# collinlongoria/blok

Hardware: AMD Instinct MI355X
Metric: Mrays/sec, primary first-hit rays at 4K over a 1024^3 SVO (higher is better)
Workload: dtype f32; 1 GPU; 1024^3 synthetic SVO (G(N,seed) terrain shell + 64 spheres, 2829976 voxels, 9299813 reference SvoNodes, 15132 sub-chunks), 3840x2160 primary rays, camera pose A, first-hit records 16 B/ray; hits_per_frame=2276630, framebuffer_pixels_hit=2276630, outputs=16-B first-hit records (kept on the tracing GPU) + RGBA8 framebuffer on rank 0, frames_in_flight=3, settle_frames=32, walk_waves_that_gave_up_waiting=0, beam_tile=32, full=False

## Files before the change

blok_amd/_ffi.py:

```python
from __future__ import annotations

import ctypes as C
import os
from pathlib import Path

import numpy as np

PKG_DIR = Path(__file__).resolve().parent
HOST_LIB = PKG_DIR / "libblok_host.so"
HIP_LIB = Path(os.environ.get("BLOK_HIP_LIB", PKG_DIR / "libblok_hip.so"))


class BlokLibraryError(RuntimeError):
    pass


class BlokError(RuntimeError):
    def __init__(self, status: int, message: str):
        super().__init__(f"blok status {status}: {message}")
        self.status = status


SVO_NODE = np.dtype([("child_mask", "<u4"), ("first_child", "<u4"), ("material_id", "<u4"),
                     ("occupancy", "<f4")])
# ... 237 lines not shown
    "blok_shapes_voxels": (C.c_int, [C.c_void_p, C.c_void_p, C.POINTER(C.c_int32), C.c_uint32, C.c_uint32, C.c_uint32, C.c_void_p, C.c_uint32, C.POINTER(C.c_uint64)]),
    "blok_lod_reduce": (C.c_int, [C.c_void_p, C.c_void_p, C.POINTER(C.c_int32), C.c_uint32, C.c_uint32, C.c_uint32, C.POINTER(C.c_int32), C.POINTER(C.c_int32),
                                  C.c_uint32, C.c_uint32, C.c_void_p, C.c_uint64, C.c_void_p]),
    "blok_terrain_reduce": (C.c_int, [C.c_void_p, C.POINTER(C.c_int32), C.POINTER(C.c_int32), C.c_uint32, C.c_uint32, C.c_void_p, C.c_uint64, C.c_void_p]),
    "blok_automaton_check": (C.c_int, [C.c_void_p, C.c_char_p, C.c_size_t]),
    "blok_automaton_voxels": (C.c_int, [C.c_void_p, C.c_void_p, C.POINTER(C.c_int32), C.c_uint32, C.c_uint32, C.c_uint32, C.POINTER(C.c_int32), C.POINTER(C.c_int32),
                                        C.c_void_p, C.c_void_p, C.c_void_p]),
    "blok_affine_from_instance": (C.c_int, [C.c_void_p, C.c_uint32, C.c_void_p]),
    "blok_affine_from_matrix": (C.c_int, [C.POINTER(C.c_double), C.c_void_p]),
    "blok_pose_from_instance": (C.c_int, [C.c_void_p, C.c_float, C.c_void_p]),
    "blok_pose_from_matrix": (C.c_int, [C.POINTER(C.c_double), C.POINTER(C.c_double), C.c_uint32, C.c_void_p]),
    "blok_affine_from_pose": (C.c_int, [C.c_void_p, C.c_float, C.c_uint32, C.c_void_p]),
    "blok_pose_motion_record": (C.c_int, [C.c_void_p, C.c_void_p, C.c_int, C.c_void_p]),
    "blok_affine_stamp_voxels": (C.c_int, [C.c_void_p, C.c_void_p, C.POINTER(C.c_int32), C.c_uint32, C.c_uint32, C.c_uint32, C.c_void_p, C.c_void_p, C.c_size_t,
                                           C.c_void_p, C.POINTER(C.c_int32), C.POINTER(C.c_int32), C.c_int, C.c_float, C.POINTER(C.c_uint64)]),
    "blok_scene_generate": (C.c_int, [C.c_void_p, C.c_uint32, C.c_uint32, C.POINTER(C.c_uint64)]),
    "blok_scene_generate_dense": (C.c_int, [C.c_uint32, C.c_uint32, C.c_void_p, C.POINTER(C.c_uint64)]),
    "blok_scene_materials": (C.c_int, [C.c_uint32, C.c_void_p]),
    "blok_scene_camera": (C.c_int, [C.c_uint32, C.c_uint32, C.c_int, C.c_uint32, C.c_uint32, C.c_void_p]),
}

HIP_SYMBOLS = {
    "blok_hip_create": (C.c_int, [C.POINTER(C.c_void_p), C.c_int, C.c_uint32, C.c_uint32]),
    "blok_hip_resize": (C.c_int, [C.c_void_p, C.c_uint32, C.c_uint32]),
    "blok_hip_destroy": (None, [C.c_void_p]),
    "blok_hip_last_error": (C.c_char_p, [C.c_void_p]),
    "blok_hip_release_stream": (C.c_int, [C.c_void_p, C.c_void_p]),
    "blok_hip_upload_world": (C.c_int, [C.c_void_p, C.c_void_p, C.c_size_t, C.c_void_p, C.c_size_t,
                                        C.c_void_p, C.c_size_t]),
    "blok_hip_upload_dense": (C.c_int, [C.c_void_p, C.c_void_p, C.c_uint32, C.c_uint32, C.c_uint32,
                                        C.POINTER(C.c_int32), C.c_void_p, C.c_size_t]),
    "blok_hip_set_host_build": (C.c_int, [C.c_void_p, C.c_int]),
    "blok_hip_world_built_on_device": (C.c_int, [C.c_void_p]),
    "blok_hip_download_tree": (C.c_int, [C.c_void_p, C.c_void_p, C.c_size_t, C.c_void_p, C.c_size_t]),
    "blok_hip_world_stats": (C.c_int, [C.c_void_p, C.POINTER(WorldStats)]),
    "blok_hip_trace_primary": (C.c_int, [C.c_void_p, C.c_void_p, C.c_uint32, C.c_uint32, C.c_uint32,
                                         C.c_uint32, C.c_void_p]),
    "blok_hip_trace_primary_device": (C.c_int, [C.c_void_p, C.c_void_p, C.c_uint32, C.c_uint32,
                                                C.c_uint32, C.c_uint32, C.c_void_p, C.c_void_p, C.c_void_p]),
    "blok_hip_tiles_for_rank": (C.c_uint32, [C.c_uint32, C.c_uint32, C.c_uint32, C.c_uint32, C.c_uint32]),
    "blok_hip_trace_tiles_device": (C.c_int, [C.c_void_p, C.c_void_p, C.c_uint32, C.c_uint32, C.c_uint32,
                                              C.c_void_p, C.c_void_p, C.c_void_p]),
    "blok_hip_untile_device": (C.c_int, [C.c_void_p, C.c_void_p, C.c_uint32, C.c_uint32, C.c_uint32, C.c_uint32,
                                         C.c_void_p, C.c_void_p]),
    "blok_hip_trace_paths_device": (C.c_int, [C.c_void_p, C.c_void_p] + [C.c_uint32] * 7 + [C.POINTER(GBuffer), C.c_void_p]),
    "blok_hip_trace_paths": (C.c_int, [C.c_void_p, C.c_void_p] + [C.c_uint32] * 7 + [C.POINTER(GBuffer)]),
    "blok_hip_trace_paths_ref_device": (C.c_int, [C.c_void_p, C.c_void_p] + [C.c_uint32] * 7 + [C.POINTER(C.c_float), C.POINTER(GBufferRef), C.c_void_p]),
    "blok_hip_denoise_ref_device": (C.c_int, [C.c_void_p, C.POINTER(GBufferRef), C.POINTER(C.c_float), C.c_uint32, C.c_void_p, C.c_void_p, C.c_void_p]),
    "blok_hip_tonemap_device": (C.c_int, [C.c_void_p, C.c_void_p, C.c_uint32, C.c_float, C.c_float, C.c_int, C.c_void_p, C.c_void_p]),
    "blok_hip_tonemap": (C.c_int, [C.c_void_p, C.c_void_p, C.c_uint32, C.c_float, C.c_float, C.c_int, C.c_void_p]),
    "blok_hip_trace_rays": (C.c_int, [C.c_void_p, C.c_void_p, C.c_size_t, C.c_void_p]),
    "blok_hip_shade_rgba8": (C.c_int, [C.c_void_p, C.c_void_p, C.c_uint32, C.c_uint32, C.c_uint32,
                                       C.c_uint32, C.c_void_p]),
    "blok_hip_draw_frame_accumulate": (C.c_int, [C.c_void_p, C.c_void_p, C.c_uint32, C.c_uint32, C.c_void_p, C.POINTER(C.c_uint32)]),
    "blok_hip_accum_download": (C.c_int, [C.c_void_p, C.c_void_p]),
    "blok_hip_reset_accum": (C.c_int, [C.c_void_p]),
    "blok_hip_set_beam": (C.c_int, [C.c_void_p, C.c_uint32]),
    "blok_hip_set_fused": (C.c_int, [C.c_void_p, C.c_int]),
    "blok_hip_set_dense_dda": (C.c_int, [C.c_void_p, C.c_int]),
    "blok_hip_set_voxel_size": (C.c_int, [C.c_void_p, C.c_float]),
    "blok_hip_multi_create": (C.c_int, [C.POINTER(C.c_void_p), C.POINTER(C.c_int), C.c_uint32, C.c_uint32, C.c_uint32, C.c_uint32, C.c_int]),
    "blok_hip_multi_destroy": (None, [C.c_void_p]),
    "blok_hip_multi_last_error": (C.c_char_p, [C.c_void_p]),
    "blok_hip_multi_device_count": (C.c_uint32, [C.c_void_p]),
    "blok_hip_multi_transport": (C.c_char_p, [C.c_void_p]),
    "blok_hip_multi_context": (C.c_void_p, [C.c_void_p, C.c_uint32]),
    "blok_hip_multi_upload_world": (C.c_int, [C.c_void_p, C.c_void_p, C.c_size_t, C.c_void_p, C.c_size_t, C.c_void_p, C.c_size_t]),
    "blok_hip_multi_draw_frame_device": (C.c_int, [C.c_void_p, C.c_void_p, C.POINTER(C.c_void_p)]),
    "blok_hip_multi_synchronize": (C.c_int, [C.c_void_p]),
    "blok_hip_multi_draw_frame": (C.c_int, [C.c_void_p, C.c_void_p, C.c_void_p]),
    "blok_hip_multi_set_exchange": (C.c_int, [C.c_void_p, C.c_int]),
    "blok_hip_multi_exchange": (C.c_char_p, [C.c_void_p]),
    "blok_hip_multi_debug_deny_peer_access": (C.c_int, [C.c_void_p, C.c_int]),
    "blok_hip_multi_draw_frames_device": (C.c_int, [C.c_void_p, C.c_void_p, C.c_uint32, C.POINTER(C.c_void_p)]),
    "blok_hip_multi_draw_frames": (C.c_int, [C.c_void_p, C.c_void_p, C.c_uint32, C.c_void_p]),
    "blok_hip_multi_download_hits": (C.c_int, [C.c_void_p, C.c_uint32, C.c_void_p, C.c_size_t]),
    "blok_hip_set_beam_budget": (C.c_int, [C.c_void_p, C.c_uint32]),
    "blok_hip_beam_cache_download": (C.c_int, [C.c_void_p, C.c_void_p, C.c_void_p, C.c_void_p, C.c_size_t]),
    "blok_hip_set_miss_writer": (C.c_int, [C.c_void_p, C.c_int]),
    "blok_hip_set_beam_cache": (C.c_int, [C.c_void_p, C.c_int]),
    "blok_hip_beam_cache_counters": (C.c_int, [C.c_void_p, C.POINTER(C.c_uint64), C.POINTER(C.c_uint64)]),
    "blok_hip_beam_cache_download_starts": (C.c_int, [C.c_void_p, C.c_void_p, C.c_void_p, C.c_size_t, C.c_void_p, C.c_size_t]),
    "blok_hip_beam_cache_start_counters": (C.c_int, [C.c_void_p, C.POINTER(C.c_uint64), C.POINTER(C.c_uint64)]),
    "blok_hip_set_packed_fill": (C.c_int, [C.c_void_p, C.c_uint32]),
    "blok_hip_packed_fill_counters": (C.c_int, [C.c_void_p, C.POINTER(C.c_uint64), C.POINTER(C.c_uint64)]),
    "blok_hip_beam_cache_refines": (C.c_int, [C.c_void_p, C.POINTER(C.c_uint64)]),
    "blok_hip_set_beam_refine_after": (C.c_int, [C.c_void_p, C.c_uint32]),
    "blok_hip_beam_cache_download_fine": (C.c_int, [C.c_void_p, C.c_void_p, C.c_void_p, C.c_void_p, C.c_size_t]),
    "blok_hip_pack_area": (C.c_uint32, []),
    "blok_hip_set_beam_list_after": (C.c_int, [C.c_void_p, C.c_uint32]),
    "blok_hip_beam_cache_list_builds": (C.c_int, [C.c_void_p, C.POINTER(C.c_uint64)]),
    "blok_hip_beam_cache_download_list": (C.c_int, [C.c_void_p, C.c_void_p, C.c_void_p, C.c_void_p, C.c_void_p, C.c_size_t, C.c_void_p, C.c_size_t, C.c_void_p, C.c_size_t]),
    "blok_hip_last_launch_kind": (C.c_int, [C.c_void_p]),
    "blok_hip_set_volume_layout": (C.c_int, [C.c_void_p, C.c_int]),
    "blok_hip_set_list_classes": (C.c_int, [C.c_void_p, C.c_int]),
    "blok_hip_set_joint_prefix_limit": (C.c_int, [C.c_void_p, C.c_uint32]),
    "blok_hip_set_tile_ordering": (C.c_int, [C.c_void_p, C.c_int]),
    "blok_hip_set_rank_tile_ordering": (C.c_int, [C.c_void_p, C.c_int]),
    "blok_hip_set_moving_order": (C.c_int, [C.c_void_p, C.c_int]),
    "blok_hip_last_fallback_tiles": (C.c_int64, [C.c_void_p]),
    "blok_hip_debug_force_order_shift": (C.c_int, [C.c_void_p, C.c_int, C.c_uint32, C.c_uint32]),
    "blok_hip_debug_class_order": (C.c_int, [C.c_void_p, C.c_void_p, C.c_uint32, C.c_uint32, C.c_uint32, C.c_void_p, C.c_uint32, C.c_void_p, C.c_void_p, C.POINTER(C.c_uint32), C.c_void_p]),
    "blok_hip_last_order_use": (C.c_int, [C.c_void_p, C.POINTER(C.c_int32), C.POINTER(C.c_int32)]),
    "blok_hip_beam_prepass": (C.c_int, [C.c_void_p, C.c_void_p] + [C.c_uint32] * 4 + [C.c_void_p, C.c_void_p, C.c_size_t]),
    "blok_hip_trace_wave_tiles_device": (C.c_int, [C.c_void_p, C.c_void_p] + [C.c_uint32] * 4 + [C.c_void_p, C.c_void_p, C.c_size_t, C.c_void_p, C.c_void_p, C.c_void_p]),
    "blok_hip_set_debug_wave_clocks": (C.c_int, [C.c_void_p, C.c_void_p]),
    "blok_hip_set_taa_jitter": (C.c_int, [C.c_void_p, C.POINTER(C.c_float)]),
    "blok_hip_set_rt_taa_jitter": (C.c_int, [C.c_void_p, C.c_int]),
    "blok_hip_compact_words": (C.c_size_t, [C.c_uint32, C.c_uint32]),
    "blok_hip_trace_tile_frames_device": (C.c_int, [C.c_void_p, C.c_void_p, C.c_uint32, C.c_uint32, C.c_uint32, C.c_uint32, C.c_uint32,
                                                    C.c_void_p, C.c_void_p, C.c_void_p]),
    "blok_hip_untile_frames_device": (C.c_int, [C.c_void_p, C.c_void_p, C.c_uint32, C.c_uint32, C.c_uint32, C.c_uint32, C.c_uint32, C.c_uint32,
                                                C.c_void_p, C.c_void_p]),
    "blok_hip_compact_tile_frames_device": (C.c_int, [C.c_void_p, C.c_void_p, C.c_uint32, C.c_uint32, C.c_uint32, C.c_uint32, C.c_void_p,
                                                      C.c_void_p]),
    "blok_hip_scatter_tile_frames_device": (C.c_int, [C.c_void_p, C.c_void_p, C.c_uint32, C.c_size_t, C.c_uint32, C.c_uint32, C.c_uint32,
                                                      C.c_void_p, C.c_void_p, C.c_void_p]),
    "blok_hip_exchange_code_bits": (C.c_uint32, [C.c_void_p]),
    "blok_hip_compact_code_words": (C.c_size_t, [C.c_uint32, C.c_uint32]),
    "blok_hip_compact_hit_tile_frames_device": (C.c_int, [C.c_void_p, C.c_void_p, C.c_uint32, C.c_uint32, C.c_uint32, C.c_uint32, C.c_void_p,
                                                          C.c_void_p]),
    "blok_hip_scatter_code_tile_frames_device": (C.c_int, [C.c_void_p, C.c_void_p, C.c_uint32, C.c_size_t, C.c_uint32, C.c_uint32, C.c_uint32,
                                                           C.c_void_p, C.c_void_p, C.c_void_p]),
    "blok_hip_compact_tiles_device": (C.c_int, [C.c_void_p, C.c_void_p, C.c_uint32, C.c_uint32, C.c_void_p, C.c_void_p]),
    "blok_hip_scatter_tiles_device": (C.c_int, [C.c_void_p, C.c_void_p, C.c_uint32, C.c_size_t, C.c_uint32, C.c_uint32, C.c_void_p, C.c_void_p]),
    "blok_hip_frame_queue_stalls": (C.c_int, [C.c_void_p, C.POINTER(C.c_uint32)]),
    "blok_hip_set_sun_map": (C.c_int, [C.c_void_p, C.c_int]),
    "blok_hip_sun_map_download": (C.c_int, [C.c_void_p, C.c_void_p, C.c_void_p, C.c_size_t]),
    "blok_hip_set_ray_batching": (C.c_int, [C.c_void_p, C.c_int]),
    "blok_hip_set_path_start": (C.c_int, [C.c_void_p, C.c_int, C.c_int]),
    "blok_denoise_settings_default": (None, [C.c_void_p]),
    "blok_hip_denoise_device": (C.c_int, [C.c_void_p, C.c_void_p, C.c_void_p, C.POINTER(C.c_float), C.c_uint32, C.c_void_p,
                                          C.c_void_p, C.c_void_p]),
    "blok_hip_denoise_state": (C.c_int, [C.c_void_p] * 6),
    "blok_hip_taa_device": (C.c_int, [C.c_void_p, C.c_void_p, C.c_void_p, C.c_float, C.c_float, C.c_uint32, C.c_void_p, C.c_void_p]),
    "blok_hip_sharpen_device": (C.c_int, [C.c_void_p, C.c_void_p, C.c_float, C.c_void_p, C.c_void_p]),
    "blok_hip_post_reset": (C.c_int, [C.c_void_p]),
    "blok_camera_view_proj": (None, [C.c_void_p, C.POINTER(C.c_float)]),
    "blok_hip_draw_frame_rt": (C.c_int, [C.c_void_p, C.c_void_p, C.c_uint32, C.c_uint32, C.c_void_p, C.c_void_p, C.POINTER(C.c_uint32)]),
    "blok_hip_volume_create": (C.c_int, [C.c_void_p, C.POINTER(C.c_int32), C.c_uint32, C.c_uint32, C.c_uint32, C.c_uint32, C.c_float]),
    "blok_hip_volume_destroy": (C.c_int, [C.c_void_p]),
    "blok_hip_volume_upload": (C.c_int, [C.c_void_p, C.c_void_p, C.c_void_p]),
    "blok_hip_volume_download": (C.c_int, [C.c_void_p, C.c_void_p, C.c_void_p]),
    "blok_hip_volume_set_voxels": (C.c_int, [C.c_void_p, C.c_void_p, C.c_void_p, C.c_void_p, C.c_size_t]),
    "blok_hip_volume_apply_brush": (C.c_int, [C.c_void_p, C.POINTER(C.c_float), C.c_float, C.c_float, C.c_int]),
    "blok_hip_volume_rebuild": (C.c_int, [C.c_void_p, C.c_void_p, C.c_size_t]),
    "blok_hip_volume_voxelize_mesh": (C.c_int, [C.c_void_p, C.c_void_p, C.c_size_t, C.c_void_p, C.c_size_t, C.c_void_p, C.c_uint32, C.c_float,
                                               C.c_int, C.POINTER(C.c_uint64)]),
    "blok_hip_volume_generate_terrain": (C.c_int, [C.c_void_p, C.c_void_p, C.POINTER(C.c_int32), C.POINTER(C.c_int32), C.POINTER(C.c_uint64)]),
    "blok_hip_volume_extract_quads": (C.c_int, [C.c_void_p, C.POINTER(C.c_int32), C.POINTER(C.c_int32), C.c_uint32, C.POINTER(C.c_uint64),
                                                C.POINTER(C.c_uint64)]),
    "blok_hip_volume_quads_download": (C.c_int, [C.c_void_p, C.c_void_p, C.c_uint64, C.c_uint64]),
    "blok_hip_lights_from_quads": (C.c_int, [C.c_void_p, C.c_uint32, C.c_void_p]),
    "blok_hip_set_lights": (C.c_int, [C.c_void_p, C.c_void_p, C.c_uint32, C.c_void_p]),
    "blok_hip_lights_info": (C.c_int, [C.c_void_p, C.c_void_p]),
    "blok_hip_lights_download": (C.c_int, [C.c_void_p, C.c_void_p, C.c_uint64, C.c_uint64]),
    "blok_hip_volume_stamp_models": (C.c_int, [C.c_void_p, C.c_void_p, C.c_uint32, C.c_int, C.c_float, C.POINTER(C.c_uint64)]),
    "blok_hip_volume_stamp_affine": (C.c_int, [C.c_void_p, C.c_void_p, C.c_uint32, C.POINTER(C.c_int32), C.POINTER(C.c_int32), C.c_int, C.c_float,
                                               C.POINTER(C.c_uint64)]),
    "blok_hip_volume_capture_model": (C.c_int, [C.c_void_p, C.POINTER(C.c_int32), C.POINTER(C.c_int32), C.c_uint32, C.POINTER(C.c_uint32),
                                                C.POINTER(C.c_uint64)]),
    "blok_hip_volume_label_components": (C.c_int, [C.c_void_p, C.POINTER(C.c_int32), C.POINTER(C.c_int32), C.c_uint32, C.POINTER(C.c_uint64),
                                                   C.POINTER(C.c_uint64)]),
    "blok_hip_volume_components_download": (C.c_int, [C.c_void_p, C.c_void_p, C.c_uint64, C.c_uint64]),
    "blok_hip_volume_labels_download": (C.c_int, [C.c_void_p, C.c_void_p, C.c_uint64, C.c_uint64]),
    "blok_hip_volume_capture_component": (C.c_int, [C.c_void_p, C.c_uint32, C.c_uint32, C.POINTER(C.c_uint32), C.POINTER(C.c_int32),
# ... 141 lines not shown
```

blok_amd/csrc/hip/api.hip:

```cpp
#include "api_internal.h"
#include "../common/lights_core.h"
#include <cstdlib>

namespace blok_api {


thread_local std::string g_create_error;

int set_error(blok_hip_ctx* ctx, int status, const std::string& msg) {
    if (ctx) ctx->error = msg; else g_create_error = msg;
    return status;
}


void free_world(blok_hip_ctx* ctx) {
    ctx->own_nodes.reset(); ctx->own_tree_materials.reset();
    ctx->d_nodes = nullptr; ctx->d_tree_materials = nullptr; ctx->tree_owned_by_volume = false;
    ctx->d_materials.reset(); ctx->d_sun_map.reset(); ctx->d_dense_tiled.reset(); ctx->d_dense_bits.reset();
    ctx->has_sun_map = false; ctx->has_dense = false;
    ctx->n_materials = 0; ctx->has_world = false; ctx->built_on_device = false; ctx->stats = blok_world_stats{};
    ctx->world_voxel_size = 1.0f;
    clear_lights(ctx);
}

// ... 155 lines not shown
    a.levels = ctx->stats.levels;
    a.voxel_size = ctx->world_voxel_size; a.inv_voxel_size = 1.0f / ctx->world_voxel_size;
    if (cam) a.cam = *cam;
    a.frame_w = ctx->width; a.frame_h = ctx->height;
    a.jitter_clip[0] = (2.0f * ctx->jitter_px[0]) / static_cast<float>(ctx->width);
    a.jitter_clip[1] = (2.0f * ctx->jitter_px[1]) / static_cast<float>(ctx->height);
    a.mat_table = ctx->d_materials;
    a.n_materials = static_cast<uint32_t>(ctx->n_materials);
    a.tmin = BLOK_RAY_TMIN; a.tmax = BLOK_RAY_TMAX;
    a.beam_budget = ctx->beam_budget;
    a.debug_clocks = ctx->debug_clocks;
    return a;
}

int beam_buffer(blok_hip_ctx* ctx, hipStream_t stream, size_t n, float** out) {
    auto& slot = ctx->beam_buffers[stream];
    BLOK_HIP_TRY(ctx, slot.beam.reserve(n, blok::FreeAfter::work_on(stream)));
    *out = slot.beam;
    return BLOK_OK;
}

int prepare_queue(blok_hip_ctx* ctx, blok::RayMode mode, const blok::TraceArgs& args, hipStream_t stream, uint32_t n_beams,
                  blok::FrameQueue* queue, uint32_t* n_blocks) {
    const size_t per_beam = static_cast<size_t>(args.beam_tile / blok::kWaveW) * (args.beam_tile / blok::kWaveH);
    const uint32_t parts = ctx->frame_parts;
    const size_t part_capacity = static_cast<size_t>((n_beams + parts - 1u) / parts) * per_beam;
    const size_t need = part_capacity * parts;
    auto& slot = ctx->beam_buffers[stream];
    bool fresh = false;
    BLOK_HIP_TRY(ctx, slot.ctl.reserve(blok::kFrameCtlWords, blok::FreeAfter::nothing(), &fresh));
    if (fresh) BLOK_HIP_TRY_FILL(ctx, slot.ctl, hipMemsetAsync(slot.ctl, 0, blok::kFrameCtlWords * sizeof(uint32_t), stream));
    BLOK_HIP_TRY(ctx, slot.entries.reserve(need, blok::FreeAfter::work_on(stream), &fresh));
    if (fresh) BLOK_HIP_TRY_FILL(ctx, slot.entries, hipMemsetAsync(slot.entries, 0xFF, need * sizeof(unsigned long long), stream));
    queue->ctl = slot.ctl; queue->entries = slot.entries; queue->n_beam = n_beams; queue->part_capacity = static_cast<uint32_t>(part_capacity);
    queue->n_parts = parts; queue->chunk = ctx->frame_chunk;
    const int m = mode == blok::RayMode::Rect ? 0 : 1;
    const uint32_t lv = args.levels < 16u ? args.levels : 15u;
    if (!ctx->frame_blocks_per_cu[m][lv]) {
        const int n = blok::frame_blocks_per_cu(mode, args);
        if (n <= 0) return set_error(ctx, BLOK_ERR_HIP, "frame kernel does not fit a compute unit");
        ctx->frame_blocks_per_cu[m][lv] = n;
    }
    const size_t resident = static_cast<size_t>(ctx->cu_count) * ctx->frame_blocks_per_cu[m][lv];
    const size_t waves = std::min(resident, std::max<size_t>(static_cast<size_t>(n_beams) * per_beam, n_beams));
    *n_blocks = static_cast<uint32_t>((waves + parts - 1u) / parts * parts);
    return BLOK_OK;
}

int prepare_beam(blok_hip_ctx* ctx, blok::RayMode mode, blok::TraceArgs& args, hipStream_t stream, uint32_t tiles_of_rank, uint32_t* n_beams) {
    *n_beams = 0;
    if (mode == blok::RayMode::Rays || !ctx->beam_tile) return BLOK_OK;
    args.beam_tile = ctx->beam_tile;
    if (mode == blok::RayMode::Tiles && args.tile % args.beam_tile) args.beam_tile = 16;
    if (args.beam_tile % blok::kWaveW || args.beam_tile % blok::kWaveH) { args.beam_tile = 0; return BLOK_OK; }
    args.beam_bx = (args.w + args.beam_tile - 1u) / args.beam_tile;
    *n_beams = blok::beam_tiles(mode, args, tiles_of_rank);
    return beam_buffer(ctx, stream, *n_beams, &args.beam);
}

bool rect_inside(const blok_hip_ctx* ctx, uint32_t x0, uint32_t y0, uint32_t w, uint32_t h) {
    return w && h && x0 < ctx->width && y0 < ctx->height && w <= ctx->width - x0 && h <= ctx->height - y0;
}

int check_trace(blok_hip_ctx* ctx, const blok_camera* cam) {
    if (!ctx) return BLOK_ERR_INVALID_ARG;
    if (!cam) return set_error(ctx, BLOK_ERR_INVALID_ARG, "camera is null");
    {
        const float* f = reinterpret_cast<const float*>(cam);
        for (size_t i = 0; i < sizeof(blok_camera) / sizeof(float); ++i)
            if (!std::isfinite(f[i])) return set_error(ctx, BLOK_ERR_INVALID_ARG, "camera has a non-finite component");
        if (!(cam->tan_half_fov > 0.0f) || !(cam->aspect > 0.0f)) return set_error(ctx, BLOK_ERR_INVALID_ARG, "camera needs tan_half_fov > 0 and aspect > 0");
    }
    if (!ctx->has_world) return set_error(ctx, BLOK_ERR_NO_WORLD, "no world uploaded");
    BLOK_HIP_TRY(ctx, hipSetDevice(ctx->device));
    return BLOK_OK;
}

}

using namespace blok_api;

extern "C" {

uint32_t blok_hip_abi_version(void) { return (1u << 16) | 26u; }

const char* blok_hip_last_error(const blok_hip_ctx* ctx) { return ctx ? ctx->error.c_str() : g_create_error.c_str(); }

int blok_hip_create(blok_hip_ctx** out_ctx, int device_ordinal, uint32_t width, uint32_t height) {
    if (!out_ctx) return BLOK_ERR_INVALID_ARG;
    *out_ctx = nullptr;
    if (!width || !height) return set_error(nullptr, BLOK_ERR_INVALID_ARG, "zero-sized frame");
    int count = 0;
    hipError_t e = hipGetDeviceCount(&count);
    if (e != hipSuccess || count <= 0)
        return set_error(nullptr, BLOK_ERR_NO_DEVICE, std::string("no HIP device: ") + hipGetErrorString(e));
    if (device_ordinal < 0 || device_ordinal >= count)
        return set_error(nullptr, BLOK_ERR_INVALID_ARG, "device ordinal out of range");
    hipDeviceProp_t prop{};
    e = hipGetDeviceProperties(&prop, device_ordinal);
    if (e != hipSuccess) return set_error(nullptr, BLOK_ERR_NO_DEVICE, std::string("hipGetDeviceProperties: ") + hipGetErrorString(e));
    if (std::strncmp(prop.gcnArchName, "gfx950", 6) != 0)
        return set_error(nullptr, BLOK_ERR_NO_DEVICE, std::string("device is ") + prop.gcnArchName + ", this backend is built for gfx950 only");
    e = hipSetDevice(device_ordinal);
    if (e != hipSuccess) return set_error(nullptr, BLOK_ERR_NO_DEVICE, std::string("hipSetDevice: ") + hipGetErrorString(e));
    auto* ctx = new (std::nothrow) blok_hip_ctx();
    if (!ctx) return set_error(nullptr, BLOK_ERR_OOM, "host allocation failed");
    ctx->device = device_ordinal; ctx->width = width; ctx->height = height;
    ctx->cu_count = prop.multiProcessorCount;
    if (const char* e = std::getenv("BLOK_FRAME_PARTS")) { const long v = std::atol(e); if (v >= 1 && v <= long(blok::kFrameParts)) ctx->frame_parts = uint32_t(v); }
    if (const char* e = std::getenv("BLOK_FRAME_CHUNK")) { const long v = std::atol(e); if (v >= 1 && v <= 64) ctx->frame_chunk = uint32_t(v); }    if (ctx->ev_begin.create(hipEventDefault) != hipSuccess || ctx->ev_end.create(hipEventDefault) != hipSuccess) {
        delete ctx;
        return set_error(nullptr, BLOK_ERR_HIP, "hipEventCreate failed");
    }
    if (order_buffers(ctx, 0u, nullptr) != BLOK_OK || beam_cache_buffers(ctx) != BLOK_OK || hipDeviceSynchronize() != hipSuccess) {
        const std::string why = ctx->error;
        blok_hip_destroy(ctx);
        return set_error(nullptr, BLOK_ERR_OOM, "scheduling buffers: " + why);
    }
    *out_ctx = ctx;
    return BLOK_OK;
}

int blok_hip_resize(blok_hip_ctx* ctx, uint32_t width, uint32_t height) {
    if (!ctx) return BLOK_ERR_INVALID_ARG;
    if (!width || !height) return set_error(ctx, BLOK_ERR_INVALID_ARG, "zero-sized frame");
    ctx->width = width; ctx->height = height;
    BLOK_HIP_TRY(ctx, hipSetDevice(ctx->device));
    const int rc = order_buffers(ctx, 0u, nullptr);
    if (rc != BLOK_OK) return rc;
    const int rc_cache = beam_cache_buffers(ctx);
    if (rc_cache != BLOK_OK) return rc_cache;
    BLOK_HIP_TRY(ctx, hipDeviceSynchronize());
    return BLOK_OK;
}

int blok_hip_release_stream(blok_hip_ctx* ctx, void* hip_stream) {
    if (!ctx) return BLOK_ERR_INVALID_ARG;
    hipStream_t stream = static_cast<hipStream_t>(hip_stream);
    BLOK_HIP_TRY(ctx, hipSetDevice(ctx->device));
    BLOK_HIP_TRY(ctx, hipDeviceSynchronize());
    auto it = ctx->beam_buffers.find(stream);
    if (it != ctx->beam_buffers.end()) ctx->beam_buffers.erase(it);
    forget_device_activity(ctx, true, stream);
    settle_beam_cache(ctx);
    return BLOK_OK;
}

void blok_hip_destroy(blok_hip_ctx* ctx) {
    if (!ctx) return;
    (void)hipSetDevice(ctx->device);
    if (ctx->has_volume) blok::gpu_volume_destroy(&ctx->volume);
    free_volume_snapshots(ctx);
    forget_device_activity(ctx);
    delete ctx;
}

int blok_hip_upload_world(blok_hip_ctx* ctx, const blok_svo_node* nodes, size_t n_nodes,
                          const blok_sub_chunk* sub_chunks, size_t n_sub_chunks,
                          const blok_material* materials, size_t n_materials) {
    if (!ctx) return BLOK_ERR_INVALID_ARG;
    if ((n_nodes && !nodes) || (n_sub_chunks && !sub_chunks) || (n_materials && !materials))
        return set_error(ctx, BLOK_ERR_INVALID_ARG, "null array with non-zero count");
    BLOK_HIP_TRY(ctx, hipSetDevice(ctx->device));
    const float vs = ctx->voxel_size;
    std::vector<blok_sub_chunk> scaled;
    if (vs != 1.0f) {
        scaled.assign(sub_chunks, sub_chunks + n_sub_chunks);
// ... 639 lines not shown
```

blok_amd/csrc/hip/api_debug.hip:

```cpp
#include "api_internal.h"
#include <cstdlib>
#include <cstdio>

using namespace blok_api;

extern "C" {

int blok_hip_set_host_build(blok_hip_ctx* ctx, int enabled) {
    if (!ctx) return BLOK_ERR_INVALID_ARG;
    ctx->force_host_build = enabled != 0;
    return BLOK_OK;
}

int blok_hip_world_built_on_device(const blok_hip_ctx* ctx) { return ctx && ctx->has_world && ctx->built_on_device ? 1 : 0; }

int blok_hip_download_tree(const blok_hip_ctx* ctx, void* nodes_out, size_t node_capacity, uint32_t* materials_out,
                           size_t material_capacity) {
    if (!ctx || !ctx->has_world) return BLOK_ERR_NO_WORLD;
    if ((nodes_out && node_capacity < ctx->stats.n_tree_nodes) || (materials_out && material_capacity < ctx->stats.n_voxels))
        return BLOK_ERR_INVALID_ARG;
    if (nodes_out && hipMemcpy(nodes_out, ctx->d_nodes, ctx->stats.n_tree_nodes * sizeof(blok::TreeNode), hipMemcpyDeviceToHost) != hipSuccess)
        return BLOK_ERR_HIP;
    if (materials_out && ctx->stats.n_voxels &&
        hipMemcpy(materials_out, ctx->d_tree_materials, ctx->stats.n_voxels * sizeof(uint32_t), hipMemcpyDeviceToHost) != hipSuccess)
// ... 209 lines not shown
    *out_stalled_waves = 0;
    BLOK_HIP_TRY(ctx, hipSetDevice(ctx->device));
    BLOK_HIP_TRY(ctx, hipDeviceSynchronize());
    for (auto& kv : ctx->beam_buffers) {
        if (kv.second.gave_up) {
            uint32_t n = 0;
            BLOK_HIP_TRY(ctx, hipMemcpy(&n, kv.second.gave_up, sizeof(n), hipMemcpyDeviceToHost));
            *out_stalled_waves += n;
        }
        if (!kv.second.ctl) continue;
        for (uint32_t part = 0; part < blok::kFrameParts; ++part) {
            uint32_t n = 0;
            BLOK_HIP_TRY(ctx, hipMemcpy(&n, kv.second.ctl + part * blok::kFramePartWords + blok::kFrameStalledWord, sizeof(n), hipMemcpyDeviceToHost));
            *out_stalled_waves += n;
        }
    }
    return BLOK_OK;
}

int blok_hip_last_launch_kind(const blok_hip_ctx* ctx) { return ctx ? ctx->last_launch_kind : -1; }

int blok_hip_set_tile_ordering(blok_hip_ctx* ctx, int resort_every_n_frames) {
    if (!ctx) return BLOK_ERR_INVALID_ARG;
    if (resort_every_n_frames < 0) return set_error(ctx, BLOK_ERR_INVALID_ARG, "tile ordering: interval must be >= 0");
    ctx->order.enabled = resort_every_n_frames != 0;
    if (resort_every_n_frames) ctx->order.interval = ctx->order.interval_now = static_cast<uint32_t>(resort_every_n_frames);
    return BLOK_OK;
}

int blok_hip_set_rank_tile_ordering(blok_hip_ctx* ctx, int enabled) {
    if (!ctx) return BLOK_ERR_INVALID_ARG;
    ctx->order.rank_tiles = enabled != 0;
    return BLOK_OK;
}

int blok_hip_debug_force_order_shift(blok_hip_ctx* ctx, int enabled, uint32_t shift_x, uint32_t shift_y) {
    if (!ctx) return BLOK_ERR_INVALID_ARG;
    ctx->order.debug_shift = enabled != 0; ctx->order.debug_sx = shift_x; ctx->order.debug_sy = shift_y;
    return BLOK_OK;
}

int64_t blok_hip_last_fallback_tiles(const blok_hip_ctx* ctx) {
    if (!ctx || !ctx->order.h_fallback) return -1;
    return static_cast<int64_t>(*static_cast<volatile uint32_t*>(ctx->order.h_fallback));
}

int blok_hip_set_moving_order(blok_hip_ctx* ctx, int enabled) {
    if (!ctx) return BLOK_ERR_INVALID_ARG;
    ctx->order.moving = enabled != 0;
    return BLOK_OK;
}

int blok_hip_last_order_use(const blok_hip_ctx* ctx, int32_t* out_shift_x, int32_t* out_shift_y) {
    if (!ctx) return -1;
    if (out_shift_x) *out_shift_x = static_cast<int32_t>(ctx->order.last_sx);
    if (out_shift_y) *out_shift_y = static_cast<int32_t>(ctx->order.last_sy);
    return ctx->order.last_use;
}

int blok_hip_set_joint_prefix_limit(blok_hip_ctx* ctx, uint32_t max_walk_waves) {
    if (!ctx) return BLOK_ERR_INVALID_ARG;
    ctx->order.prefix_limit = max_walk_waves;
    return BLOK_OK;
}

int blok_hip_set_list_classes(blok_hip_ctx* ctx, int enabled) {
    if (!ctx) return BLOK_ERR_INVALID_ARG;
    ctx->list_classes = enabled != 0;
    return BLOK_OK;
}

int blok_hip_set_miss_writer(blok_hip_ctx* ctx, int in_walk) {
    if (!ctx) return BLOK_ERR_INVALID_ARG;
    ctx->miss_in_walk = in_walk != 0;
    return BLOK_OK;
}

int blok_hip_set_beam_cache(blok_hip_ctx* ctx, int mode) {
    if (!ctx) return BLOK_ERR_INVALID_ARG;
    ctx->beam_cache.enabled = mode != 0;
    ctx->beam_cache.refine = mode >= 2;
    ctx->beam_cache.packed = mode >= 3;
    ctx->beam_cache.policy.own_starts = mode >= 4;
    blok::beam_cache_clear(ctx->beam_cache.policy);
    if (!ctx->beam_cache.packed) return BLOK_OK;
    BLOK_HIP_TRY(ctx, hipSetDevice(ctx->device));
    return beam_list_buffers(ctx);
}

int blok_hip_set_beam_list_after(blok_hip_ctx* ctx, uint32_t hits) {
    if (!ctx) return BLOK_ERR_INVALID_ARG;
    ctx->beam_cache.policy.list_after = hits ? hits : blok::kBeamListAfter;
    return BLOK_OK;
}

uint32_t blok_hip_pack_area(void) { return blok::kPackArea; }

int blok_hip_beam_cache_list_builds(const blok_hip_ctx* ctx, uint64_t* out_builds) {
    if (!ctx) return BLOK_ERR_INVALID_ARG;
    if (out_builds) *out_builds = ctx->beam_cache.list_builds;
    return BLOK_OK;
}

int blok_hip_beam_cache_download_list(blok_hip_ctx* ctx, int* out_state, uint32_t* out_n_areas, uint32_t* out_n_groups, uint32_t* out_list_host, size_t list_capacity,
                                      uint32_t* out_table_host, size_t table_capacity, uint8_t* out_trips_host, size_t trips_capacity) {
    if (!ctx) return BLOK_ERR_INVALID_ARG;
    const auto& B = ctx->beam_cache;
    if (out_state) *out_state = B.last_list;
    if (out_n_areas) *out_n_areas = 0u;
    if (out_n_groups) *out_n_groups = 0u;
    if (!B.last_list) return BLOK_OK;
    if (B.last_slot < 0 || static_cast<uint32_t>(B.last_slot) >= blok::kBeamCacheSlots || !B.slots[B.last_slot].d_list)
        return set_error(ctx, BLOK_ERR_INVALID_ARG, "beam cache: the latest launch's slot is gone (a resize)");
    const auto& sl = B.slots[B.last_slot];
    const uint32_t n_areas = sl.n_words / blok::kPackGroups;
    const size_t entries = static_cast<size_t>(n_areas) * blok::kPackStretch, pixels = static_cast<size_t>(B.last_w) * B.last_h;
    if (entries > B.list_capacity || sl.n_words > B.words_capacity || pixels > B.d_trips.capacity()) return set_error(ctx, BLOK_ERR_INVALID_ARG, "beam cache: the list's buffers are gone (a resize)");
    if ((out_list_host && list_capacity < entries) || (out_table_host && table_capacity < sl.n_words) || (out_trips_host && trips_capacity < pixels))
        return set_error(ctx, BLOK_ERR_INVALID_ARG, "beam cache: output smaller than the list, the table or the rectangle");
    if (out_n_areas) *out_n_areas = n_areas;
    if (!out_n_groups && !out_list_host && !out_table_host && !out_trips_host) return BLOK_OK;
    BLOK_HIP_TRY(ctx, hipSetDevice(ctx->device));
    BLOK_HIP_TRY(ctx, hipDeviceSynchronize());
    if (out_n_groups) *out_n_groups = B.last_list == 2 ? sl.n_groups : std::min(B.h_groups[B.last_slot], sl.n_words);
    if (out_list_host) BLOK_HIP_TRY(ctx, hipMemcpy(out_list_host, sl.d_list, entries * sizeof(uint32_t), hipMemcpyDeviceToHost));
    if (out_table_host) BLOK_HIP_TRY(ctx, hipMemcpy(out_table_host, sl.d_table, sl.n_words * sizeof(uint32_t), hipMemcpyDeviceToHost));
    if (out_trips_host) BLOK_HIP_TRY(ctx, hipMemcpy(out_trips_host, B.d_trips, pixels, hipMemcpyDeviceToHost));
    return BLOK_OK;
}

int blok_hip_beam_cache_download_starts(blok_hip_ctx* ctx, int* out_state, float* out_starts_host, size_t starts_capacity, uint8_t* out_restarts_host, size_t restarts_capacity) {
    if (!ctx) return BLOK_ERR_INVALID_ARG;
    const auto& B = ctx->beam_cache;
    if (out_state) *out_state = B.last_starts;
    if (!out_starts_host && !out_restarts_host) return BLOK_OK;
    if (!B.last_list || B.last_slot < 0 || static_cast<uint32_t>(B.last_slot) >= blok::kBeamCacheSlots || !B.policy.starts[B.last_slot] || !B.slots[B.last_slot].d_start)
        return set_error(ctx, BLOK_ERR_INVALID_ARG, "beam cache: the latest launch's slot has no list with starts");
    const auto& sl = B.slots[B.last_slot];
    const size_t entries = static_cast<size_t>(sl.n_words / blok::kPackGroups) * blok::kPackStretch, pixels = static_cast<size_t>(B.last_w) * B.last_h;
    if (entries > sl.d_start.capacity() || pixels > B.d_restarts.capacity()) return set_error(ctx, BLOK_ERR_INVALID_ARG, "beam cache: the starts' buffers are gone (a resize)");
    if ((out_starts_host && starts_capacity < entries) || (out_restarts_host && restarts_capacity < pixels))
        return set_error(ctx, BLOK_ERR_INVALID_ARG, "beam cache: output smaller than the list or the rectangle");
    BLOK_HIP_TRY(ctx, hipSetDevice(ctx->device));
    BLOK_HIP_TRY(ctx, hipDeviceSynchronize());
    if (out_starts_host) BLOK_HIP_TRY(ctx, hipMemcpy(out_starts_host, sl.d_start, entries * sizeof(float), hipMemcpyDeviceToHost));
    if (out_restarts_host) BLOK_HIP_TRY(ctx, hipMemcpy(out_restarts_host, B.d_restarts, pixels, hipMemcpyDeviceToHost));
    return BLOK_OK;
}

int blok_hip_beam_cache_start_counters(const blok_hip_ctx* ctx, uint64_t* out_from_starts, uint64_t* out_other_key) {
    if (!ctx) return BLOK_ERR_INVALID_ARG;
    if (out_from_starts) *out_from_starts = ctx->beam_cache.start_hits;
    if (out_other_key) *out_other_key = ctx->beam_cache.start_other_key;
    return BLOK_OK;
}

int blok_hip_set_packed_fill(blok_hip_ctx* ctx, uint32_t units_per_wave) {
    if (!ctx) return BLOK_ERR_INVALID_ARG;
    ctx->beam_cache.packed_fill = units_per_wave;
    return BLOK_OK;
}

int blok_hip_packed_fill_counters(const blok_hip_ctx* ctx, uint64_t* out_one_launch_frames, uint64_t* out_fill_only_workgroups) {
    if (!ctx) return BLOK_ERR_INVALID_ARG;
    if (out_one_launch_frames) *out_one_launch_frames = ctx->beam_cache.one_launch_frames;
    if (out_fill_only_workgroups) *out_fill_only_workgroups = ctx->beam_cache.fill_only_workgroups;
    return BLOK_OK;
}

int blok_hip_beam_cache_counters(const blok_hip_ctx* ctx, uint64_t* out_hits, uint64_t* out_fills) {
    if (!ctx) return BLOK_ERR_INVALID_ARG;
    if (out_hits) *out_hits = ctx->beam_cache.hits;
    if (out_fills) *out_fills = ctx->beam_cache.fills;
    return BLOK_OK;
}

int blok_hip_set_beam_refine_after(blok_hip_ctx* ctx, uint32_t hits) {
    if (!ctx) return BLOK_ERR_INVALID_ARG;
    ctx->beam_cache.policy.refine_after = hits ? hits : blok::kBeamRefineAfter;
    return BLOK_OK;
}

int blok_hip_beam_cache_refines(const blok_hip_ctx* ctx, uint64_t* out_refines) {
    if (!ctx) return BLOK_ERR_INVALID_ARG;
    if (out_refines) *out_refines = ctx->beam_cache.refines;
    return BLOK_OK;
}

int blok_hip_beam_cache_download(blok_hip_ctx* ctx, int* out_action, uint32_t* out_n_beams, float* out_t0_host, size_t capacity) {
    if (!ctx) return BLOK_ERR_INVALID_ARG;
    const auto& B = ctx->beam_cache;
    if (out_action) *out_action = B.last_action;
    if (out_n_beams) *out_n_beams = B.last_action ? B.last_n_beams : 0u;
    if (!out_t0_host || !B.last_action) return BLOK_OK;
    if (B.last_slot < 0 || static_cast<uint32_t>(B.last_slot) >= blok::kBeamCacheSlots || !B.slots[B.last_slot].d_beam || B.last_n_beams > B.capacity)
        return set_error(ctx, BLOK_ERR_INVALID_ARG, "beam cache: the latest launch's slot is gone (a resize)");
    if (capacity < B.last_n_beams) return set_error(ctx, BLOK_ERR_INVALID_ARG, "beam cache: output smaller than the launch's beam tiles");
    BLOK_HIP_TRY(ctx, hipSetDevice(ctx->device));
    BLOK_HIP_TRY(ctx, hipDeviceSynchronize());
    BLOK_HIP_TRY(ctx, hipMemcpy(out_t0_host, B.slots[B.last_slot].d_beam, B.last_n_beams * sizeof(float), hipMemcpyDeviceToHost));
    return BLOK_OK;
}

int blok_hip_beam_cache_download_fine(blok_hip_ctx* ctx, int* out_state, uint32_t* out_n_tiles, float* out_t0_host, size_t capacity) {
    if (!ctx) return BLOK_ERR_INVALID_ARG;
    const auto& B = ctx->beam_cache;
    if (out_state) *out_state = B.last_fine;
    if (out_n_tiles) *out_n_tiles = B.last_n_fine;
    if (!out_t0_host || !B.last_fine) return BLOK_OK;
    if (B.last_slot < 0 || static_cast<uint32_t>(B.last_slot) >= blok::kBeamCacheSlots || !B.slots[B.last_slot].d_fine || B.last_n_fine > B.capacity)
        return set_error(ctx, BLOK_ERR_INVALID_ARG, "beam cache: the latest launch's slot is gone (a resize)");
    if (capacity < B.last_n_fine) return set_error(ctx, BLOK_ERR_INVALID_ARG, "beam cache: output smaller than the launch's wave tiles");
    BLOK_HIP_TRY(ctx, hipSetDevice(ctx->device));
    BLOK_HIP_TRY(ctx, hipDeviceSynchronize());
    BLOK_HIP_TRY(ctx, hipMemcpy(out_t0_host, B.slots[B.last_slot].d_fine, B.last_n_fine * sizeof(float), hipMemcpyDeviceToHost));
    return BLOK_OK;
}

int blok_hip_set_beam_budget(blok_hip_ctx* ctx, uint32_t max_node_visits) {
    if (!ctx) return BLOK_ERR_INVALID_ARG;
    ctx->beam_budget = max_node_visits;
    return BLOK_OK;
}

}
```

blok_amd/csrc/hip/api_internal.h:

```cpp
#ifndef BLOK_API_INTERNAL_H
#define BLOK_API_INTERNAL_H
#include <hip/hip_runtime.h>

#include <cmath>
#include <map>
#include <mutex>
#include <unordered_map>
#include <utility>
#include <cstdio>
#include <cstring>
#include <new>
#include <string>
#include <vector>

#include "blok_hip.h"
#include "blok_hip_debug.h"
#include "device_buffer.h"
#include "gpu_build.h"
#include <hip/hip_fp16.h>
#include "post_kernels.h"
#include "post_core.h"
#include "reference_world.h"
#include "trace_kernels.h"
#include "dense_kernels.h"
// ... 46 lines not shown
        bool has_motion = false;
        blok::DeviceArray<float> rt_planes[2], rt_denoised, rt_resolved;
        blok::DeviceArray<uint16_t> rt_normal_roughness_h, rt_motion_h;
        blok::DeviceArray<uint32_t> rt_albedo_metallic_u8;
        blok::DeviceArray<uint32_t> rt_ldr, rt_final;
        uint32_t rt_frame = 0;
        blok_camera rt_prev_cam{};
        blok::DeviceArray<uint32_t> rt_ids;
        uint32_t rt_prev_n = 0;
        uint32_t rt_prev_n_poses = 0;
    } post;
    blok::DeviceArray<blok_instance> rt_instances, rt_prev_instances;
    blok::DeviceArray<blok_pose> rt_poses;
    blok::DeviceArray<blok_pose> rt_prev_poses;
    blok::GpuVolume volume;
    bool has_volume = false;
    bool volume_keyed_layout = true;
    blok::GpuQuads quads;
    blok::GpuComponents components;
    blok::GpuBricks bricks;
    blok::GpuDistance distance;
    blok::GpuFlood flood;
    blok::GpuColumns columns;
    blok::GpuScatter scatter;
    blok::GpuLod lod;
    struct Lights {
        blok::DeviceArray<blok_light> table;
        blok::DeviceArray<uint32_t> owned;
        uint32_t n = 0, n_owned = 0;
        uint64_t n_faces = 0;
        float area_world = 0.0f;
    } lights;
    std::vector<uint32_t> material_glows;
    std::vector<unsigned char> volume_materials;
    blok::DeviceArray<float> d_sun_map;
    bool sun_map_enabled = true, has_sun_map = false;
    uint32_t sun_loose_edits = 0; int32_t sun_loose_lo[3] = {0, 0, 0}, sun_loose_hi[3] = {0, 0, 0};
    bool sun_tighten_pending = false; uint32_t sun_tighten_u0 = 0, sun_tighten_u1 = 0, sun_tighten_v0 = 0, sun_tighten_v1 = 0;
    blok::Event sun_event; bool sun_event_pending = false;
    uint32_t ray_batching = 3;
    uint32_t tail_cap = 24, tail_cap_parked = 32;
    bool pose_tlas = true;
    bool path_resume = false, path_fine_beam = true;
    blok::SunMapArgs sun{};
    uint32_t beam_tile = 32;
    uint32_t beam_budget = 0;
    bool miss_in_walk = true;
    struct StreamScratch {
        blok::DeviceArray<float> beam;
        blok::DeviceArray<uint32_t> ctl; blok::DeviceArray<unsigned long long> entries;
        blok::DeviceArray<unsigned long long> slots; uint32_t serial = 0;
        blok::DeviceArray<uint32_t> gave_up;
        blok::DeviceArray<unsigned long long> list_entries; size_t list_capacity = 0;
        blok::DeviceArray<unsigned long long> list_ctl;
        uint32_t list_serial = 0;
        blok::PinnedArray<uint32_t> list_hint; bool list_hint_valid = false; uint32_t list_hint_key = 0;
        blok::DeviceArray<uint32_t> tile_map;
        blok::DeviceBytes tail_pool;
        blok::DeviceArray<uint32_t> inst_bins;
        blok::DeviceArray<blok_hit> inst_hits;
        blok::DeviceArray<uint32_t> pose_bins;
        blok::DeviceBytes pose_tlas;
        blok::DeviceArray<blok_pose_motion> pose_motion;
        blok::DeviceBytes tlas;
    };
    std::unordered_map<hipStream_t, StreamScratch> beam_buffers;
    struct BeamCache {
        bool enabled = true;
        bool refine = true;
        blok::BeamCachePolicy policy{};
        struct Produced {
            blok::Event done;
            hipStream_t producer = nullptr;
            bool settled = true;
            static constexpr uint32_t kWaited = 8;
            hipStream_t waited[kWaited] = {}; uint32_t n_waited = 0;
        };
        struct Slot {
            blok::DeviceArray<float> d_beam, d_fine;
            Produced filled, refined;
            bool used = false;
            blok::DeviceArray<uint32_t> d_list, d_table;
            blok::DeviceArray<float> d_start;
            uint32_t n_words = 0, n_groups = 0;
        } slots[blok::kBeamCacheSlots];
        bool packed = true;
        blok::DeviceArray<uint8_t> d_trips;
        blok::DeviceArray<float> d_ray_start;
        blok::DeviceArray<uint8_t> d_restarts;
        blok::DeviceArray<uint32_t> d_words;
        blok::DeviceBytes d_sort_temp; size_t sort_temp_bytes = 0;
        blok::PinnedArray<uint32_t> h_groups;
        blok::Event list_done;
        size_t list_capacity = 0, words_capacity = 0;
        uint64_t list_builds = 0;
        uint64_t start_hits = 0, start_other_key = 0;
        uint32_t packed_fill = BLOK_PACKED_FILL;
        uint64_t one_launch_frames = 0, fill_only_workgroups = 0;
        int last_starts = 0;
        int last_list = 0;
        uint32_t last_w = 0, last_h = 0;
        size_t capacity = 0;
        uint64_t hits = 0, fills = 0, refines = 0;
        int last_action = 0, last_slot = -1; uint32_t last_n_beams = 0;
        int last_fine = 0; uint32_t last_n_fine = 0;
    } beam_cache;
    struct TileOrder {
        bool enabled = true;
        bool rank_tiles = true;
        uint32_t interval = 8, interval_now = 8;
        blok::DeviceArray<uint32_t> d_cost, d_iota;
        blok::DeviceArray<uint32_t> d_keys_in, d_keys;
        blok::DeviceBytes d_temp;
        size_t temp_bytes = 0, capacity = 0;
        static constexpr int kSlots = 4;
        struct Slot {
            blok::DeviceArray<uint32_t> d_order, d_rank_of;
            bool valid = false, dilated = false;
            uint32_t live = 0, radius = 0;
            blok_camera cam{};
            float inv_depth[2] = {};
            uint32_t frames_since_sort = 0, interval_now = 8;
            uint64_t last_use = 0;
        } slots[kSlots];
        blok::PinnedArray<uint32_t> h_live;
        blok::PinnedArray<float> h_depth;
        uint32_t key[7] = {};
        int current = -1, target = 0;
        bool pending = false;
        bool orphan = false;
        uint32_t still_frames = 0, prefix_limit = 0;
        uint64_t launch_serial = 0, hold_serial = 0;
        blok_camera last_cam{};
        blok_camera recent[4] = {}; uint32_t n_recent = 0, revisit_streak = 0;
        blok_camera pending_cam{}; bool pending_dilated = false; uint32_t pending_radius = 0, pending_interval = 8;
        blok::Event done;
        bool moving = true;
        blok::DeviceBytes d_class_scratch;
        bool have_residual = false; float last_residual = 0.0f;
        bool debug_shift = false; uint32_t debug_sx = 0, debug_sy = 0;
        blok::DeviceArray<uint32_t> d_fallback;
        blok::PinnedArray<uint32_t> h_fallback;
        uint32_t last_fallback = 0;
        bool alone_before = false;
        int last_use = 0; uint32_t last_sx = 0, last_sy = 0;
        int chosen = -1;
    } order;
    blok::DeviceArray<uint32_t> d_list_cost; uint32_t list_cost_key[6] = {};
    blok_camera list_prev_cam{}; bool list_has_prev_cam = false;
    bool list_classes = true;
    uint32_t* debug_clocks = nullptr;
    int launch_form = blok::kFormAuto;
    int last_launch_kind = -1;
    uint32_t frame_parts = 32, frame_chunk = 1;
    int cu_count = 0;
    int frame_blocks_per_cu[2][16] = {};
    float jitter_px[2] = {0.0f, 0.0f};
    bool rt_taa_jitter = true;
    struct Models {
        struct Arrays {
            blok::DeviceArray<uint4> nodes; blok::DeviceArray<uint32_t> materials;
            uint32_t n_nodes = 0, n_materials = 0;
            int32_t box_lo[3] = {0, 0, 0}, box_hi[3] = {0, 0, 0};
        };
        std::vector<blok::ModelDesc> desc;
        std::vector<Arrays> own;
        blok::DeviceArray<blok::ModelDesc> d_desc;
        float uploaded_voxel_size = 1.0f;
        uint32_t stack_levels = 1;
    } models;
    blok::Event ev_begin, ev_end;
    bool timing = false, timed = false;
// ... 112 lines not shown
```

blok_amd/csrc/hip/api_launch.hip:

```cpp
#include "api_internal.h"
#include "beam.h"
#include <cstdlib>

namespace blok_api {

namespace {
struct StreamMarks { blok::Event last, held; bool fresh = false; };
struct DeviceActivity {
    std::mutex lock;
    std::map<std::pair<const blok_hip_ctx*, hipStream_t>, StreamMarks> marks;
};
DeviceActivity& device_activity(int device) {
    static std::mutex table_lock;
    static auto& table = *new std::map<int, DeviceActivity>;
    std::lock_guard<std::mutex> g(table_lock);
    return table[device];
}
}

static bool device_busy_elsewhere(const blok_hip_ctx* ctx, hipStream_t stream) {
    DeviceActivity& act = device_activity(ctx->device);
    std::lock_guard<std::mutex> g(act.lock);
    bool busy = false;
    for (auto& kv : act.marks) {
// ... 227 lines not shown
}

int live_list(blok_hip_ctx* ctx, blok::TraceArgs& args, hipStream_t stream, uint32_t n_searches, uint32_t per_search) {
    auto& slot = ctx->beam_buffers[stream];
    const size_t seg_capacity = static_cast<size_t>((n_searches + blok::kListSegments - 1u) / blok::kListSegments) * per_search;
    bool fresh = false;
    BLOK_HIP_TRY(ctx, slot.list_ctl.reserve(blok::kListSegments * blok::kListCtlWords, blok::FreeAfter::nothing(), &fresh));
    if (fresh) {
        BLOK_HIP_TRY_FILL(ctx, slot.list_ctl, hipMemsetAsync(slot.list_ctl, 0, blok::kListSegments * blok::kListCtlWords * sizeof(unsigned long long), stream));
        BLOK_HIP_TRY_FILL(ctx, slot.list_ctl, slot.list_hint.reserve(blok::kListSegments * blok::kListClasses, blok::FreeAfter::nothing()));
        std::memset(slot.list_hint, 0, blok::kListSegments * blok::kListClasses * sizeof(uint32_t));
        slot.list_hint_valid = false;
    }
    const bool wrapped = slot.list_serial + 1u >= (1u << blok::kListSerialBits);
    if (slot.list_capacity < seg_capacity || wrapped) {
        bool grown = false;
        if (slot.list_capacity < seg_capacity) {
            slot.list_capacity = 0;
            BLOK_HIP_TRY(ctx, slot.list_entries.reserve(seg_capacity * blok::kListSegments * blok::kListClasses, blok::FreeAfter::work_on(stream), &grown));
            slot.list_capacity = seg_capacity;
        }
        const hipError_t emptied = hipMemsetAsync(slot.list_entries, 0, slot.list_capacity * blok::kListSegments * blok::kListClasses * sizeof(unsigned long long), stream);
        if (emptied != hipSuccess && grown) { slot.list_entries.reset(); slot.list_capacity = 0; }
        BLOK_HIP_TRY(ctx, emptied);
        if (wrapped) slot.list_serial = 0;
    }
    slot.list_serial += 1u;
    args.list.entries = slot.list_entries; args.list.ctl = slot.list_ctl; args.list.hint = slot.list_hint;
    args.list.seg_capacity = static_cast<uint32_t>(slot.list_capacity);
    args.list.serial = slot.list_serial; args.list.n_searches = n_searches;
    return gave_up_counter(ctx, stream, &args.joint_gave_up);
}

static bool list_hint(const blok_hip_ctx* ctx, hipStream_t stream, uint32_t geometry_key, uint32_t per_class[blok::kListClasses]) {
    auto it = ctx->beam_buffers.find(stream);
    if (it == ctx->beam_buffers.end() || !it->second.list_hint || !it->second.list_hint_valid || it->second.list_hint_key != geometry_key) return false;
    for (uint32_t c = 0; c < blok::kListClasses; ++c) {
        per_class[c] = 0;
        for (uint32_t k = 0; k < blok::kListSegments; ++k) per_class[c] = std::max(per_class[c], it->second.list_hint[k * blok::kListClasses + c]);
    }
    return true;
}

static int list_costs(blok_hip_ctx* ctx, blok::TraceArgs& args, uint32_t wave_tiles, hipStream_t stream) {
    const uint32_t key[6] = {args.x0, args.y0, args.w, args.h, ctx->width, ctx->height};
    bool fresh = false;
    BLOK_HIP_TRY(ctx, ctx->d_list_cost.reserve(wave_tiles, blok::FreeAfter::device(), &fresh));
    if (fresh || std::memcmp(key, ctx->list_cost_key, sizeof(key)) != 0) {
        BLOK_HIP_TRY(ctx, hipMemsetAsync(ctx->d_list_cost, 0, ctx->d_list_cost.capacity() * sizeof(uint32_t), stream));
        std::memcpy(ctx->list_cost_key, key, sizeof(key));
        ctx->list_has_prev_cam = false;
    }
    args.list.cost = ctx->d_list_cost;
    args.list.has_prev = ctx->list_has_prev_cam ? 1u : 0u;
    args.list.prev_cam = ctx->list_prev_cam;
    ctx->list_prev_cam = args.cam; ctx->list_has_prev_cam = true;
    return BLOK_OK;
}

int beam_cache_buffers(blok_hip_ctx* ctx) {
    auto& B = ctx->beam_cache;
    const size_t want = static_cast<size_t>((ctx->width + 7u) / 8u) * ((ctx->height + 7u) / 8u);
    if (B.capacity >= want) return beam_list_buffers(ctx);
    BLOK_HIP_TRY(ctx, hipDeviceSynchronize());
    B.capacity = 0;
    blok::beam_cache_clear(B.policy);
    for (auto& sl : B.slots) {
        sl = blok_hip_ctx::BeamCache::Slot{};
        BLOK_HIP_TRY(ctx, sl.d_beam.reserve(want, blok::FreeAfter::nothing()));
        BLOK_HIP_TRY(ctx, sl.d_fine.reserve(want, blok::FreeAfter::nothing()));
        BLOK_HIP_TRY(ctx, sl.filled.done.create());
        BLOK_HIP_TRY(ctx, sl.refined.done.create());
    }
    B.capacity = want;
    B.list_capacity = 0;
    return beam_list_buffers(ctx);
}

int beam_list_buffers(blok_hip_ctx* ctx) {
    auto& B = ctx->beam_cache;
    if (!B.packed) return BLOK_OK;
    const size_t areas = static_cast<size_t>((ctx->width + blok::kPackArea - 1u) / blok::kPackArea) * ((ctx->height + blok::kPackArea - 1u) / blok::kPackArea);
    const size_t entries = areas * blok::kPackStretch, words = areas * blok::kPackGroups, pixels = static_cast<size_t>(ctx->width) * ctx->height;
    const bool own = B.policy.own_starts;
    if (B.list_capacity >= entries && B.words_capacity >= words && B.d_trips.capacity() >= pixels &&
        (!own || (B.d_ray_start.capacity() >= pixels && B.d_restarts.capacity() >= pixels && B.slots[0].d_start.capacity() >= entries))) return BLOK_OK;
    BLOK_HIP_TRY(ctx, hipDeviceSynchronize());
    B.list_capacity = 0; B.words_capacity = 0;
    blok::beam_cache_clear(B.policy);
    blok::beam_list_settle(B.policy);
    const blok::FreeAfter waited = blok::FreeAfter::nothing();
    for (auto& sl : B.slots) {
        BLOK_HIP_TRY(ctx, sl.d_list.reserve(entries, waited));
        BLOK_HIP_TRY(ctx, sl.d_table.reserve(words, waited));
        if (own) BLOK_HIP_TRY(ctx, sl.d_start.reserve(entries, waited));
        sl.n_groups = 0;
    }
    BLOK_HIP_TRY(ctx, B.d_trips.reserve(pixels, waited));
    if (own) { BLOK_HIP_TRY(ctx, B.d_ray_start.reserve(pixels, waited)); BLOK_HIP_TRY(ctx, B.d_restarts.reserve(pixels, waited)); }
    BLOK_HIP_TRY(ctx, B.d_words.reserve(words, waited));
    B.sort_temp_bytes = blok::pack_table_temp_bytes(static_cast<uint32_t>(words));
    BLOK_HIP_TRY(ctx, B.d_sort_temp.reserve(B.sort_temp_bytes ? B.sort_temp_bytes : 16, waited));
    BLOK_HIP_TRY(ctx, B.h_groups.reserve(blok::kBeamCacheSlots, waited));
    BLOK_HIP_TRY(ctx, B.list_done.create());
    B.list_capacity = entries; B.words_capacity = words;
    return BLOK_OK;
}

void settle_beam_cache(blok_hip_ctx* ctx) {
    for (auto& sl : ctx->beam_cache.slots)
        for (auto* p : {&sl.filled, &sl.refined}) { p->settled = true; p->n_waited = 0; }
}

static blok::BeamKey beam_key(const blok_hip_ctx* ctx, blok::RayMode mode, const blok::TraceArgs& args) {
    blok::BeamKey k{};
    static_assert(sizeof(k.cam) == sizeof(blok_camera), "beam_cache.h: BeamKey::cam is blok_camera, byte for byte");
    std::memcpy(k.cam, &args.cam, sizeof(blok_camera));
    k.x0 = args.x0; k.y0 = args.y0; k.w = args.w; k.h = args.h;
    k.frame_w = args.frame_w; k.frame_h = args.frame_h;
    k.beam_tile = args.beam_tile; k.beam_budget = args.beam_budget;
    k.tuning = blok::kBeamCoarsen1 | (blok::kBeamCoarsen2 << 8) | (static_cast<uint32_t>(BLOK_BEAM_STOP_LEVEL) << 16);
    k.ray_mode = static_cast<uint32_t>(mode);
    k.levels = args.levels;
    for (int a = 0; a < 3; ++a) k.origin[a] = args.origin[a];
    std::memcpy(&k.voxel_bits, &args.voxel_size, sizeof(uint32_t));
    const uint64_t nodes = reinterpret_cast<uintptr_t>(args.nodes);
    k.nodes_lo = static_cast<uint32_t>(nodes); k.nodes_hi = static_cast<uint32_t>(nodes >> 32);
    k.world_version = ctx->world_version; k.tree_version = ctx->tree_version;
    return k;
}

static int wait_for_producer(blok_hip_ctx* ctx, blok_hip_ctx::BeamCache::Produced& p, hipStream_t stream) {
    if (p.settled || stream == p.producer) return BLOK_OK;
    for (uint32_t k = 0; k < p.n_waited; ++k) if (p.waited[k] == stream) return BLOK_OK;
    if (hipEventQuery(p.done) == hipSuccess) { p.settled = true; p.n_waited = 0; return BLOK_OK; }
    (void)hipGetLastError();
    BLOK_HIP_TRY(ctx, hipStreamWaitEvent(stream, p.done, 0));
    if (p.n_waited < blok_hip_ctx::BeamCache::Produced::kWaited) p.waited[p.n_waited++] = stream;
    return BLOK_OK;
}

static int beam_cache_before_launch(blok_hip_ctx* ctx, blok::RayMode mode, blok::TraceArgs& args, hipStream_t stream, blok::BeamCachePlan* plan, blok::BeamRefinePlan* fine,
                                    blok::BeamListPlan* listed, blok::BeamStartsPlan* starts) {
    auto& B = ctx->beam_cache;
    *plan = blok::plan_beam_cache(B.policy, beam_key(ctx, mode, args));
    *fine = blok::plan_beam_refine(B.policy, *plan, B.refine && blok::beam_refine_applies(args) && blok::beam_refine_tiles(args) <= B.capacity);
    bool build_finished = false;
    if (B.policy.building >= 0) { build_finished = hipEventQuery(B.list_done) == hipSuccess; (void)hipGetLastError(); }
    *listed = blok::plan_beam_list(B.policy, *plan, *fine, B.packed && blok::pack_applies(args) && static_cast<size_t>(blok::pack_areas(args)) * blok::kPackStretch <= B.list_capacity &&
                                   static_cast<size_t>(args.w) * args.h <= B.d_trips.capacity(), build_finished);
    if (listed->adopted >= 0) { auto& got = B.slots[listed->adopted]; got.n_groups = std::min(B.h_groups[listed->adopted], got.n_words); }
    blok::BeamStartKey start_key;
    static_assert(sizeof(args.jitter_clip) == sizeof(start_key.jitter_clip), "beam_cache.h: BeamStartKey::jitter_clip is TraceArgs::jitter_clip, bit for bit");
    std::memcpy(start_key.jitter_clip, args.jitter_clip, sizeof(start_key.jitter_clip));
    std::memcpy(&start_key.tmin, &args.tmin, sizeof(uint32_t)); std::memcpy(&start_key.tmax, &args.tmax, sizeof(uint32_t));
    *starts = blok::plan_beam_starts(B.policy, *plan, *listed, start_key);
    if (plan->action == blok::BeamAction::Search) return BLOK_OK;
    auto& sl = B.slots[plan->slot];
    if (plan->action == blok::BeamAction::Hit) {
        { const int rc = wait_for_producer(ctx, sl.filled, stream); if (rc != BLOK_OK) return rc; }
        if (fine->use_fine) { const int rc = wait_for_producer(ctx, sl.refined, stream); if (rc != BLOK_OK) return rc; }
        B.hits += 1u;
    } else {
        if (sl.used) {
            hold_markers(ctx);
            const int rc = wait_for_held_markers(ctx, stream);
            if (rc != BLOK_OK) return rc;
        }
        sl.used = true;
        sl.filled.settled = false; sl.filled.producer = stream; sl.filled.n_waited = 0;
        B.fills += 1u;
    }
    args.beam = sl.d_beam; args.beam_slots = nullptr; args.beam_serial = 0u;
    return BLOK_OK;
}

int launch_timed(blok_hip_ctx* ctx, blok::RayMode mode, blok::TraceArgs args, uint32_t blocks, hipStream_t stream,
                 uint32_t tiles_of_rank, const blok::TileFrames* frames) {
    uint32_t n_beams = 0;
    if (blocks) { const int rc = prepare_beam(ctx, mode, args, stream, tiles_of_rank, &n_beams); if (rc != BLOK_OK) return rc; }
    const uint32_t n_frames = frames ? frames->n_frames : 1u;
    if (frames && n_beams) { const int rc = beam_buffer(ctx, stream, static_cast<size_t>(n_beams) * n_frames, &args.beam); if (rc != BLOK_OK) return rc; }
    blok::LaunchFacts facts{};
    facts.form = ctx->launch_form;
    facts.has_beam = n_beams != 0;
    facts.one_wave_blocks = blok::kBlock == 64;
    facts.wave_tiles = blocks * n_frames;
    const uint32_t geometry_key = blocks * 31u + n_beams * n_frames;
    facts.have_hint = list_hint(ctx, stream, geometry_key, facts.hint);
    bool busy = false;
    bool capturing = false;
    if (stream) {
        hipStreamCaptureStatus status = hipStreamCaptureStatusNone;
        if (hipStreamIsCapturing(stream, &status) == hipSuccess) capturing = status != hipStreamCaptureStatusNone;
        else (void)hipGetLastError();
    }
    if (capturing) facts.form = blok::kFormTwoLaunches;
    else busy = facts.has_beam && (ctx->launch_form == blok::kFormAuto || (ctx->order.enabled && ctx->order.moving)) && device_busy_elsewhere(ctx, stream);
    facts.device_busy = busy && ctx->launch_form == blok::kFormAuto;
    blok::LaunchPlan plan = blok::plan_launch(facts);
    if (frames && (plan.kind == blok::LaunchKind::Queues || plan.kind == blok::LaunchKind::Joint)) plan.kind = blok::LaunchKind::TwoLaunches;
    ctx->last_launch_kind = static_cast<int>(plan.kind);

    blok::FrameQueue queue{};
    uint32_t frame_blocks = 0;
    blok::TileFrames fr{};
    if (frames) { fr = *frames; fr.blocks_per_frame = blocks; fr.beams_per_frame = n_beams; }
    if (plan.kind == blok::LaunchKind::Joint) { const int rc = joint_slots(ctx, args, stream, n_beams); if (rc != BLOK_OK) return rc; }
    if (plan.kind == blok::LaunchKind::Queues) { const int rc = prepare_queue(ctx, mode, args, stream, n_beams, &queue, &frame_blocks); if (rc != BLOK_OK) return rc; }
    if (plan.kind == blok::LaunchKind::ListJoint || plan.kind == blok::LaunchKind::ListTwoLaunches) {
        const uint32_t per_search = (args.beam_tile / blok::kWaveW) * (args.beam_tile / blok::kWaveH);
        const int rc = live_list(ctx, args, stream, n_beams * n_frames, per_search);
        if (rc != BLOK_OK) return rc;
        for (uint32_t c = 0; c < blok::kListClasses; ++c) args.list.walkers[c] = plan.walkers_per_class[c];
        if (mode == blok::RayMode::Rect && ctx->list_classes) { const int rc2 = list_costs(ctx, args, blocks, stream); if (rc2 != BLOK_OK) return rc2; }
        auto& slot = ctx->beam_buffers[stream];
        slot.list_hint_valid = true; slot.list_hint_key = geometry_key;
    }
    const bool static_form = plan.kind == blok::LaunchKind::TwoLaunches || plan.kind == blok::LaunchKind::Joint;
    const bool rect = mode == blok::RayMode::Rect;
    const bool orderable = !capturing && ctx->order.enabled && static_form && ((rect && !frames) || (mode == blok::RayMode::Tiles && ctx->order.rank_tiles)) && n_beams &&
                           blocks >= blok::kOrderMinTiles && BLOK_XCD_MAP == 0 && blok::kBlock == 64;
    bool uniform_view = true;
    if (frames) for (uint32_t f = 1; f < frames->n_frames; ++f) uniform_view = uniform_view && camera_near(ctx, frames->cam[0], frames->cam[f]);
    blok::OrderPlan order_plan{};
    if (orderable) { const int rc = order_before_launch(ctx, args, blocks, stream, !busy, rect, uniform_view, &order_plan); if (rc != BLOK_OK) return rc; }
    else ctx->order.last_use = 0;
    uint32_t walk_blocks = blocks;
    if (args.order && args.rank_of && plan.may_use_prefix && args.launched <= blocks) {
        if (ctx->order.prefix_limit && args.launched > ctx->order.prefix_limit) args.launched = ctx->order.prefix_limit;
        walk_blocks = args.launched;
        if (ctx->timing) {
            ctx->order.last_fallback = *static_cast<volatile uint32_t*>(ctx->order.h_fallback.get());
            BLOK_HIP_TRY(ctx, hipMemsetAsync(ctx->order.d_fallback, 0, sizeof(uint32_t), stream));
            args.fallback_tiles = ctx->order.d_fallback;
        }
        if (args.order_sx || args.order_sy) {
            const uint32_t tiles_x = (args.w + blok::kTileW - 1u) / blok::kTileW, tiles_y = (args.h + blok::kTileH - 1u) / blok::kTileH;
            const bool left = args.order_sx * 2u <= tiles_x, top = args.order_sy * 2u <= tiles_y;
            const float res = ctx->order.have_residual && ctx->order.last_residual >= 0.0f ? std::min(ctx->order.last_residual, 8.0f) : 0.0f;
            const uint32_t extra = static_cast<uint32_t>(std::ceil(res));
            args.strip_nx = left ? args.order_sx : tiles_x - args.order_sx; if (args.strip_nx) args.strip_nx = std::min(args.strip_nx + extra, tiles_x);
            args.strip_ny = top ? args.order_sy : tiles_y - args.order_sy; if (args.strip_ny) args.strip_ny = std::min(args.strip_ny + extra, tiles_y);
            args.strip_x0 = left ? 0u : tiles_x - args.strip_nx;
            args.strip_y0 = top ? 0u : tiles_y - args.strip_ny;
            args.n_strip = args.strip_nx * tiles_y + (tiles_x - args.strip_nx) * args.strip_ny;
            walk_blocks += args.n_strip;
        }
    } else { args.rank_of = nullptr; args.launched = 0u; }
    if (ctx->timing && !capturing) BLOK_HIP_TRY(ctx, hipEventRecord(ctx->ev_begin, stream));
    args.miss_in_walk = static_form && !args.rank_of && ctx->miss_in_walk ? 1u : 0u;
    blok::BeamCachePlan cached{blok::BeamAction::Search, -1};
    blok::BeamRefinePlan finer{false, false};
    blok::BeamListPlan listed{false, false, -1};
    blok::BeamStartsPlan starts{false, blok::BeamStarts::None};
    if (ctx->beam_cache.enabled && rect && !frames && !capturing && static_form && ctx->launch_form == blok::kFormAuto && n_beams && n_beams <= ctx->beam_cache.capacity) {
        const int rc = beam_cache_before_launch(ctx, mode, args, stream, &cached, &finer, &listed, &starts);
        if (rc != BLOK_OK) {
            if (finer.refine_now) blok::beam_refine_commit(ctx->beam_cache.policy, cached.slot, false);
            if (listed.count_now) blok::beam_list_commit(ctx->beam_cache.policy, cached.slot, false);
            return rc;
        }
        if (cached.action == blok::BeamAction::Fill && plan.kind == blok::LaunchKind::Joint) { plan.kind = blok::LaunchKind::TwoLaunches; ctx->last_launch_kind = static_cast<int>(plan.kind); }
    }
    ctx->beam_cache.last_action = cached.action == blok::BeamAction::Hit ? 2 : cached.action == blok::BeamAction::Fill ? 1 : 0;
    ctx->beam_cache.last_slot = cached.slot; ctx->beam_cache.last_n_beams = n_beams;
    ctx->beam_cache.last_fine = finer.use_fine ? 2 : finer.refine_now ? 1 : 0;
    ctx->beam_cache.last_n_fine = ctx->beam_cache.last_fine ? blok::beam_refine_tiles(args) : 0u;
    ctx->beam_cache.last_list = listed.use_list ? 2 : listed.count_now ? 1 : 0;
    ctx->beam_cache.last_starts = starts.use == blok::BeamStarts::OtherKey ? 2 : (starts.use == blok::BeamStarts::Use || starts.count_own) ? 1 : 0;
    if (starts.use == blok::BeamStarts::Use) ctx->beam_cache.start_hits += 1u;
    if (starts.use == blok::BeamStarts::OtherKey) ctx->beam_cache.start_other_key += 1u;
    ctx->beam_cache.last_w = args.w; ctx->beam_cache.last_h = args.h;
    if (cached.action == blok::BeamAction::Hit && (listed.use_list || listed.count_now)) {
        auto& B = ctx->beam_cache;
        auto& sl = B.slots[cached.slot];
        blok::TraceArgs fill = args;
        fill.order = nullptr; fill.rank_of = nullptr; fill.launched = 0u; fill.order_sx = fill.order_sy = 0u; fill.n_strip = 0u; fill.fallback_tiles = nullptr;
        fill.miss_in_walk = 0u;
        const bool one_launch = listed.use_list && sl.n_groups > 0u && B.packed_fill > 0u;
        if (!one_launch) blok::launch_beam_fill(mode, fill, n_beams, sl.d_fine, stream);
        if (one_launch) {
            const uint32_t tail = starts.use == blok::BeamStarts::Use ? blok::launch_packed_frame_own(fill, sl.d_start, sl.d_fine, sl.d_list, sl.d_table, sl.n_groups, B.packed_fill, stream)
                                                                      : blok::launch_packed_frame(fill, sl.d_fine, sl.d_list, sl.d_table, sl.n_groups, B.packed_fill, stream);
            B.one_launch_frames += 1u; B.fill_only_workgroups += tail;
        } else if (listed.use_list && starts.use == blok::BeamStarts::Use) blok::launch_packed_walk_own(fill, sl.d_start, sl.d_list, sl.d_table, sl.n_groups, stream);
        else if (listed.use_list) blok::launch_packed_walk(fill, sl.d_fine, sl.d_list, sl.d_table, sl.n_groups, stream);
        else if (starts.count_own) {
            blok::TraceArgs walk = fill;
            walk.beam = sl.d_fine; walk.beam_tile = blok::kWaveW; walk.beam_bx = (args.w + blok::kWaveW - 1u) / blok::kWaveW;
            blok::launch_trace_count_own(walk, blocks, B.d_trips, B.d_ray_start, B.d_restarts, stream);
            sl.n_words = blok::pack_areas(args) * blok::kPackGroups; sl.n_groups = 0u;
            blok::launch_pack_build_own(fill, sl.d_fine, B.d_restarts, B.d_ray_start, sl.d_list, B.d_words, sl.d_start, stream);
        } else {
            blok::TraceArgs walk = fill;
            walk.beam = sl.d_fine; walk.beam_tile = blok::kWaveW; walk.beam_bx = (args.w + blok::kWaveW - 1u) / blok::kWaveW;
            blok::launch_trace_count(walk, blocks, B.d_trips, stream);
            sl.n_words = blok::pack_areas(args) * blok::kPackGroups; sl.n_groups = 0u;
            blok::launch_pack_build(fill, sl.d_fine, B.d_trips, sl.d_list, B.d_words, stream);
        }
    } else if (cached.action == blok::BeamAction::Hit) {
        float* const d_fine = ctx->beam_cache.slots[cached.slot].d_fine;
        if (!args.miss_in_walk) blok::launch_beam_fill(mode, args, n_beams, finer.use_fine ? d_fine : nullptr, stream);
        if (finer.use_fine) {
            blok::TraceArgs walk = args;
            walk.beam = d_fine; walk.beam_tile = blok::kWaveW; walk.beam_bx = (args.w + blok::kWaveW - 1u) / blok::kWaveW;
            blok::launch_trace(mode, walk, walk_blocks, stream);
        } else blok::launch_trace(mode, args, walk_blocks, stream);
        if (finer.refine_now) blok::launch_beam_refine(args, d_fine, stream);
    } else
    switch (plan.kind) {
        case blok::LaunchKind::Walk:
            if (frames) blok::launch_tile_frames(args, fr, stream); else blok::launch_trace(mode, args, blocks, stream);
            break;
        case blok::LaunchKind::TwoLaunches:
            if (frames) blok::launch_tile_frames(args, fr, stream, walk_blocks);
            else { blok::launch_beam(mode, args, n_beams, stream); blok::launch_trace(mode, args, walk_blocks, stream); }
            break;
        case blok::LaunchKind::Queues: blok::launch_frame(mode, args, queue, frame_blocks, stream); break;
        case blok::LaunchKind::Joint: blok::launch_joint(mode, args, n_beams, walk_blocks, stream); break;
        case blok::LaunchKind::ListJoint: blok::launch_list_joint(mode, args, frames ? &fr : nullptr, n_beams * n_frames, plan.walkers, stream); break;
        case blok::LaunchKind::ListTwoLaunches:
            if (frames) blok::launch_beam_frames(args, fr, stream); else blok::launch_beam(mode, args, n_beams, stream);
            blok::launch_list_walk(mode, args, frames ? &fr : nullptr, plan.walkers, stream);
            break;
    }
    const hipError_t launch_error = hipGetLastError();
    if (launch_error != hipSuccess && cached.action == blok::BeamAction::Fill) ctx->beam_cache.policy.valid[cached.slot] = false;
    if (finer.refine_now) {
        auto& made = ctx->beam_cache.slots[cached.slot].refined;
        const hipError_t marked = launch_error == hipSuccess ? hipEventRecord(made.done, stream) : launch_error;
        blok::beam_refine_commit(ctx->beam_cache.policy, cached.slot, marked == hipSuccess);
        if (marked == hipSuccess) { made.settled = false; made.producer = stream; made.n_waited = 0; ctx->beam_cache.refines += 1u; }
        else if (launch_error == hipSuccess) BLOK_HIP_TRY(ctx, marked);
    }
    if (listed.count_now) {
        auto& B = ctx->beam_cache;
        auto& sl = B.slots[cached.slot];
        hipError_t built = launch_error;
        if (built == hipSuccess) built = blok::launch_pack_table_sort(B.d_words, sl.d_table, B.d_sort_temp, B.sort_temp_bytes, sl.n_words, B.h_groups + cached.slot, stream);
        if (built == hipSuccess) built = hipEventRecord(B.list_done, stream);
        blok::beam_list_commit(B.policy, cached.slot, built == hipSuccess);
        if (built == hipSuccess) B.list_builds += 1u;
        else if (launch_error == hipSuccess) BLOK_HIP_TRY(ctx, built);
    }
    BLOK_HIP_TRY(ctx, launch_error);
    if (cached.action == blok::BeamAction::Fill) BLOK_HIP_TRY(ctx, hipEventRecord(ctx->beam_cache.slots[cached.slot].filled.done, stream));
    if (ctx->timing && !capturing) { BLOK_HIP_TRY(ctx, hipEventRecord(ctx->ev_end, stream)); ctx->timed = true; }
    if (args.fallback_tiles) BLOK_HIP_TRY(ctx, hipMemcpyAsync(ctx->order.h_fallback, ctx->order.d_fallback, sizeof(uint32_t), hipMemcpyDeviceToHost, stream));
    if (listed.use_list) order_plan.start_sort = false;
    if (orderable) { const int rc = order_after_launch(ctx, args, blocks, n_beams, stream, order_plan); if (rc != BLOK_OK) return rc; }
    if (facts.has_beam && !capturing) return note_frame_launch(ctx, stream);
    return BLOK_OK;
}

}
```

blok_amd/csrc/hip/beam_cache.h:

```cpp
#ifndef BLOK_BEAM_CACHE_H
#define BLOK_BEAM_CACHE_H
#include <stdint.h>
#include <string.h>

namespace blok {

struct BeamKey {
    uint32_t cam[14];
    uint32_t x0, y0, w, h;
    uint32_t frame_w, frame_h;
    uint32_t beam_tile, beam_budget, tuning;
    uint32_t ray_mode;
    uint32_t levels;
    int32_t origin[3];
    uint32_t voxel_bits;
    uint32_t nodes_lo, nodes_hi;
    uint32_t world_version, tree_version;
};
static_assert(sizeof(BeamKey) == 33 * sizeof(uint32_t), "BeamKey is compared with memcmp: no padding");

inline bool beam_key_equal(const BeamKey& a, const BeamKey& b) { return memcmp(&a, &b, sizeof(BeamKey)) == 0; }

constexpr int kBeamCacheSlots = 4;

enum class BeamAction : int {
    Search = 0,
    Fill = 1,
    Hit = 2,
};
struct BeamCachePlan { BeamAction action; int slot; };

enum class BeamRefine : uint8_t {
    None = 0,
    Now = 1,
    Done = 2,
};
constexpr uint32_t kBeamRefineAfter = 16;
struct BeamRefinePlan { bool refine_now, use_fine; };

enum class BeamList : uint8_t {
    None = 0,
    Now = 1,
    Building = 2,
    Ready = 3,
};
constexpr uint32_t kBeamListAfter = 16;
struct BeamListPlan { bool count_now, use_list; int adopted; };

struct BeamStartKey { uint32_t jitter_clip[2], tmin, tmax; };
static_assert(sizeof(BeamStartKey) == 4 * sizeof(uint32_t), "BeamStartKey is compared with memcmp: no padding");
inline bool beam_start_key_equal(const BeamStartKey& a, const BeamStartKey& b) { return memcmp(&a, &b, sizeof(BeamStartKey)) == 0; }
enum class BeamStarts : int {
    None = 0,
    Use = 1,
    OtherKey = 2,
};
struct BeamStartsPlan { bool count_own; BeamStarts use; };

struct BeamCachePolicy {
    BeamKey key[kBeamCacheSlots];
    bool valid[kBeamCacheSlots];
    uint64_t last_use[kBeamCacheSlots];
    BeamKey last;
    bool have_last;
    uint64_t serial;
    BeamRefine refine[kBeamCacheSlots];
    uint32_t hits_since_fill[kBeamCacheSlots];
    uint32_t refine_after = kBeamRefineAfter;
    BeamList list[kBeamCacheSlots];
    uint32_t fine_hits[kBeamCacheSlots];
    uint32_t list_after = kBeamListAfter;
    bool own_starts = true;
    bool starts[kBeamCacheSlots];
    BeamStartKey start_key[kBeamCacheSlots];
    int building = -1;
    bool building_stale = false;
};

inline void beam_list_drop(BeamCachePolicy& s, int slot) {
    s.list[slot] = BeamList::None; s.fine_hits[slot] = 0u; s.starts[slot] = false;
    if (s.building == slot) s.building_stale = true;
}

inline void beam_cache_clear(BeamCachePolicy& s) {
    for (int k = 0; k < kBeamCacheSlots; ++k) { s.valid[k] = false; s.last_use[k] = 0u; s.refine[k] = BeamRefine::None; s.hits_since_fill[k] = 0u; beam_list_drop(s, k); }
    s.have_last = false;
}

inline void beam_list_settle(BeamCachePolicy& s) {
    if (s.building >= 0 && s.building < kBeamCacheSlots && s.list[s.building] == BeamList::Building) s.list[s.building] = BeamList::None;
    s.building = -1; s.building_stale = false;
}

inline BeamCachePlan plan_beam_cache(BeamCachePolicy& s, const BeamKey& k) {
    s.serial += 1u;
    const bool again = s.have_last && beam_key_equal(s.last, k);
    s.last = k; s.have_last = true;
    for (int i = 0; i < kBeamCacheSlots; ++i)
        if (s.valid[i] && beam_key_equal(s.key[i], k)) {
            s.last_use[i] = s.serial;
            if (s.hits_since_fill[i] != UINT32_MAX) s.hits_since_fill[i] += 1u;
            return {BeamAction::Hit, i};
        }
    if (!again) return {BeamAction::Search, -1};
    int target = -1;
    for (int i = 0; i < kBeamCacheSlots && target < 0; ++i) if (!s.valid[i]) target = i;
    if (target < 0) { target = 0; for (int i = 1; i < kBeamCacheSlots; ++i) if (s.last_use[i] < s.last_use[target]) target = i; }
    s.key[target] = k; s.valid[target] = true; s.last_use[target] = s.serial;
    s.refine[target] = BeamRefine::None; s.hits_since_fill[target] = 0u;
    beam_list_drop(s, target);
    return {BeamAction::Fill, target};
}

inline BeamRefinePlan plan_beam_refine(BeamCachePolicy& s, const BeamCachePlan& p, bool eligible) {
    if (p.action != BeamAction::Hit || p.slot < 0 || p.slot >= kBeamCacheSlots || !eligible) return {false, false};
    if (s.refine[p.slot] == BeamRefine::Done) return {false, true};
    if (s.refine[p.slot] == BeamRefine::None && s.hits_since_fill[p.slot] >= (s.refine_after ? s.refine_after : 1u)) {
        s.refine[p.slot] = BeamRefine::Now;
        return {true, false};
    }
    return {false, false};
}

inline void beam_refine_commit(BeamCachePolicy& s, int slot, bool issued) {
    if (slot < 0 || slot >= kBeamCacheSlots || s.refine[slot] != BeamRefine::Now) return;
    s.refine[slot] = issued ? BeamRefine::Done : BeamRefine::None;
    if (!issued) s.hits_since_fill[slot] = 0u;
}

inline BeamListPlan plan_beam_list(BeamCachePolicy& s, const BeamCachePlan& p, const BeamRefinePlan& f, bool eligible, bool build_finished) {
    BeamListPlan out{false, false, -1};
    if (s.building >= 0 && build_finished) {
        if (!s.building_stale && s.building < kBeamCacheSlots && s.list[s.building] == BeamList::Building) { s.list[s.building] = BeamList::Ready; out.adopted = s.building; }
        s.building = -1; s.building_stale = false;
    }
    if (p.action != BeamAction::Hit || p.slot < 0 || p.slot >= kBeamCacheSlots || !f.use_fine || !eligible) return out;
    if (s.list[p.slot] == BeamList::Ready) { out.use_list = true; return out; }
    if (s.list[p.slot] != BeamList::None) return out;
    if (s.fine_hits[p.slot] != UINT32_MAX) s.fine_hits[p.slot] += 1u;
    if (s.building < 0 && s.fine_hits[p.slot] >= (s.list_after ? s.list_after : 1u)) { s.list[p.slot] = BeamList::Now; out.count_now = true; }
    return out;
}

inline BeamStartsPlan plan_beam_starts(BeamCachePolicy& s, const BeamCachePlan& p, const BeamListPlan& l, const BeamStartKey& k) {
    if (p.action != BeamAction::Hit || p.slot < 0 || p.slot >= kBeamCacheSlots) return {false, BeamStarts::None};
    if (l.count_now) {
        s.starts[p.slot] = s.own_starts;
        if (s.own_starts) s.start_key[p.slot] = k;
        return {s.own_starts, BeamStarts::None};
    }
    if (!l.use_list || !s.starts[p.slot]) return {false, BeamStarts::None};
    return {false, beam_start_key_equal(s.start_key[p.slot], k) ? BeamStarts::Use : BeamStarts::OtherKey};
}

inline void beam_list_commit(BeamCachePolicy& s, int slot, bool issued) {
    if (slot < 0 || slot >= kBeamCacheSlots || s.list[slot] != BeamList::Now) return;
    s.list[slot] = issued ? BeamList::Building : BeamList::None;
    if (issued) { s.building = slot; s.building_stale = false; }
    else { s.fine_hits[slot] = 0u; s.starts[slot] = false; }
}

}
#endif
```

blok_amd/csrc/hip/trace_core.h:

```cpp
#ifndef BLOK_TRACE_CORE_H
#define BLOK_TRACE_CORE_H

#include "trace_kernels.h"

#ifdef BLOK_TRACE_HOST_HARNESS
#define BLOK_DEV inline
#else
#define BLOK_DEV __device__ __forceinline__
#endif

#ifndef BLOK_STAT
#define BLOK_STAT(event, level)
#endif

#if defined(__clang__)
#pragma clang fp contract(off)
#endif

namespace blok {

BLOK_DEV float rn_add(float a, float b) { return a + b; }
BLOK_DEV float rn_sub(float a, float b) { return a - b; }
BLOK_DEV float rn_mul(float a, float b) { return a * b; }
BLOK_DEV float rn_div(float a, float b) { return a / b; }
// ... 313 lines not shown
        s.fx = __uint_as_float(__float_as_uint(fx) & keep); s.fy = __uint_as_float(__float_as_uint(fy) & keep); s.fz = __uint_as_float(__float_as_uint(fz) & keep);
        s.tFx = plane_t(R.ax, s.fx + s.size); s.tFy = plane_t(R.ay, s.fy + s.size); s.tFz = plane_t(R.az, s.fz + s.size);
    }
    if (climbed) {
        BLOK_STAT(2, lvl);
        const float tExit = fminf(fminf(s.tFx, s.tFy), s.tFz);
        s.tCur = tExit;
        if (!(tExit < r.tmax)) { s.walking = false; return true; }
        const bool sx = s.tFx == tExit;
        const bool sy = !sx && s.tFy == tExit;
        const float stepped = as_written((sx ? s.fx : (sy ? s.fy : s.fz)) + s.size);
        s.fx = sx ? stepped : s.fx; s.fy = sy ? stepped : s.fy; s.fz = (sx || sy) ? s.fz : stepped;
        const uint32_t up = static_cast<uint32_t>(__builtin_ctz(__float_as_uint(stepped))) >> 1;
        if (up != lvl) {
            BLOK_STAT(3, lvl);
            if (up >= L) { s.walking = false; return true; }
            lvl = up;
            s.size = cell_size(lvl);
            const uint32_t keep = ~((1u << (2 * up)) - 1u);
            s.fx = __uint_as_float(__float_as_uint(s.fx) & keep); s.fy = __uint_as_float(__float_as_uint(s.fy) & keep); s.fz = __uint_as_float(__float_as_uint(s.fz) & keep);
            const uint4 c = stk[(lvl - 1) * kBlock];
            node.lo = c.x; node.hi = c.y; node.base = c.z;
        }
        s.tFx = plane_t(R.ax, s.fx + s.size); s.tFy = plane_t(R.ay, s.fy + s.size); s.tFz = plane_t(R.az, s.fz + s.size);
    }
    s.lvl = lvl; s.node = node;
    return true;
}

#ifndef BLOK_TRACE_HOST_HARNESS
BLOK_DEV bool walk_enter_wave(const TraceArgs& A, const RayIn& r, const WalkRay& R, uint4* stk, WalkState& s) {
    const uint32_t L = A.levels;
    const int W = 1 << (2 * L);
    const float tS = r.tmin;
    const bool negx = !(R.ax.inv > 0.0f), negy = !(R.ay.inv > 0.0f), negz = !(R.az.inv > 0.0f);
    float fx, fy, fz, tFx, tFy, tFz;
    bool ok = resume_axis(R.ax, negx, __builtin_fmaf(r.dx, tS, r.ox), A.inv_voxel_size, A.origin[0], W, tS, fx, tFx);
    ok = resume_axis(R.ay, negy, __builtin_fmaf(r.dy, tS, r.oy), A.inv_voxel_size, A.origin[1], W, tS, fy, tFy) && ok;
    ok = resume_axis(R.az, negz, __builtin_fmaf(r.dz, tS, r.oz), A.inv_voxel_size, A.origin[2], W, tS, fz, tFz) && ok;
    ok = ok && tS < r.tmax;
    if (__ballot(!ok) != 0ull) return false;
    const uint32_t qx = __float_as_uint(fx) & 0x7FFFFFu, qy = __float_as_uint(fy) & 0x7FFFFFu, qz = __float_as_uint(fz) & 0x7FFFFFu;
    const uint32_t ux = negx ? static_cast<uint32_t>(W - 1) - qx : qx, uy = negy ? static_cast<uint32_t>(W - 1) - qy : qy, uz = negz ? static_cast<uint32_t>(W - 1) - qz : qz;
    const uint32_t ux0 = __builtin_amdgcn_readfirstlane(ux), uy0 = __builtin_amdgcn_readfirstlane(uy), uz0 = __builtin_amdgcn_readfirstlane(uz);
    const uint32_t diff = (ux ^ ux0) | (uy ^ uy0) | (uz ^ uz0);
    const uint32_t mine = diff ? (static_cast<uint32_t>(31 - __clz(static_cast<int>(diff))) >> 1) + 1u : 0u;
    uint32_t m = 0u;
    for (uint32_t k = 0; k < L; ++k) if (__ballot(mine > k) != 0ull) m = k + 1u;
    if (m >= L) return false;
    typedef uint32_t Words4 __attribute__((ext_vector_type(4)));
    auto uniform_node = [&](uint32_t index, uint32_t& lo, uint32_t& hi, uint32_t& base) {
        const Words4 v = reinterpret_cast<const __attribute__((address_space(4))) Words4*>(reinterpret_cast<uintptr_t>(A.nodes))[__builtin_amdgcn_readfirstlane(index)];
        lo = v.x; hi = v.y; base = v.z;
    };
    uint32_t n_lo, n_hi, n_base;
    uniform_node(0u, n_lo, n_hi, n_base);
    uint32_t lvl = L - 1u;
    for (;;) {
        if (lvl < m) break;
        const uint32_t shift = 2u * lvl;
        const uint32_t bit = ((ux0 >> shift) & 3u) | (((uy0 >> shift) & 3u) << 2) | (((uz0 >> shift) & 3u) << 4);
        const uint32_t word = bit < 32u ? n_lo : n_hi;
        if (!((word >> (bit & 31u)) & 1u) || lvl == 0u) break;
        BLOK_STAT(1, lvl);
        stk[(lvl - 1u) * kBlock] = make_uint4(n_lo, n_hi, n_base, 0u);
        const uint32_t below_lo = bit < 32u ? (n_lo & ((1u << bit) - 1u)) : n_lo;
        const uint32_t below_hi = bit < 32u ? 0u : (n_hi & ((1u << (bit & 31u)) - 1u));
        const uint32_t child = n_base + static_cast<uint32_t>(__builtin_popcount(below_lo)) + static_cast<uint32_t>(__builtin_popcount(below_hi));
        uniform_node(child, n_lo, n_hi, n_base);
        lvl -= 1u;
    }
    s.found = false; s.bit = 0u; s.tCur = tS; s.walking = true;
    s.lvl = lvl; s.size = cell_size(lvl);
    s.node.lo = n_lo; s.node.hi = n_hi; s.node.base = n_base;
    if (lvl != 0u) {
        const uint32_t keep = ~((1u << (2 * lvl)) - 1u);
        s.fx = __uint_as_float(__float_as_uint(fx) & keep); s.fy = __uint_as_float(__float_as_uint(fy) & keep); s.fz = __uint_as_float(__float_as_uint(fz) & keep);
        s.tFx = plane_t(R.ax, s.fx + s.size); s.tFy = plane_t(R.ay, s.fy + s.size); s.tFz = plane_t(R.az, s.fz + s.size);
    } else { s.fx = fx; s.fy = fy; s.fz = fz; s.tFx = tFx; s.tFy = tFy; s.tFz = tFz; }
    return true;
}
#endif

BLOK_DEV HitInfo walk(const TraceArgs& A, const RayIn& r, uint4* stk) {
    BLOK_STAT(4, 0);
    HitInfo out;
    out.found = false; out.t = -1.0f; out.material = 0u; out.face = 0xFFu; out.vx = out.vy = out.vz = 0;
    out.brick.lo = out.brick.hi = out.brick.base = 0u;
    const WalkRay R = walk_ray(A, r.ox, r.oy, r.oz, safe_inv(r.dx), safe_inv(r.dy), safe_inv(r.dz));
    WalkState s;
    walk_enter(A, R, r.tmin, r.tmax, s);
    walk_loop(A, R, r.tmax, s, stk);
    if (s.found) out = walk_hit(A, r, R, s);
    return out;
}

template <bool kCount = false, bool kOwn = false>
BLOK_DEV HitInfo walk_wave(const TraceArgs& A, const RayIn& r, uint4* stk, [[maybe_unused]] uint32_t* n_trips = nullptr, [[maybe_unused]] float* own_start = nullptr,
                           [[maybe_unused]] uint32_t* own_trips = nullptr) {
#ifdef BLOK_TRACE_HOST_HARNESS
    return walk(A, r, stk);
#else
    HitInfo out;
    out.found = false; out.t = -1.0f; out.material = 0u; out.face = 0xFFu; out.vx = out.vy = out.vz = 0;
    out.brick.lo = out.brick.hi = out.brick.base = 0u;
    const WalkRay R = walk_ray(A, r.ox, r.oy, r.oz, safe_inv(r.dx), safe_inv(r.dy), safe_inv(r.dz));
    WalkState s;
    if (!walk_enter_wave(A, r, R, stk, s)) walk_enter(A, R, r.tmin, r.tmax, s);
    if constexpr (kCount) {
        const uint32_t shared = A.levels - 1u - s.lvl;
        if constexpr (kOwn) { *own_start = r.tmin; *own_trips = 0u; walk_loop<false, true, true>(A, R, r.tmax, s, stk, 0u, n_trips, own_start, own_trips); }
        else walk_loop<false, true>(A, R, r.tmax, s, stk, 0u, n_trips);
        *n_trips += shared;
    } else walk_loop(A, R, r.tmax, s, stk);
    if (s.found) out = walk_hit(A, r, R, s);
    return out;
#endif
}

template <bool kWave = false, bool kCount = false, bool kOwn = false>
BLOK_DEV void trace_one(const TraceArgs& A, const RayIn& r, uint4* stk, const Sink& dst, [[maybe_unused]] uint8_t* trips_out = nullptr, [[maybe_unused]] float* start_out = nullptr,
                        [[maybe_unused]] uint8_t* restart_out = nullptr) {
    [[maybe_unused]] uint32_t n_trips = 0u, own_trips = 0u;
    [[maybe_unused]] float own_start = 0.0f;
    static_assert(kWave || !kCount, "trips are counted for the primary rays of a wave tile");
    static_assert(kCount || !kOwn, "the restart parameters are left by the count launch");
    const HitInfo h = kOwn ? walk_wave<kCount, kOwn>(A, r, stk, &n_trips, &own_start, &own_trips) : kCount ? walk_wave<kCount>(A, r, stk, &n_trips) : (kWave ? walk_wave(A, r, stk) : walk(A, r, stk));
    if constexpr (kCount) *trips_out = static_cast<uint8_t>(n_trips < 255u ? n_trips : 255u);
    if constexpr (kOwn) { *start_out = own_start; *restart_out = static_cast<uint8_t>(own_trips); }
    if (!h.found) { write_miss(dst); return; }
    uint4 rec;
    rec.x = __float_as_uint(h.t);
    rec.y = h.material;
    rec.z = (static_cast<uint32_t>(h.vx) & 0xFFFFu) | (static_cast<uint32_t>(h.vy) << 16);
    rec.w = (static_cast<uint32_t>(h.vz) & 0xFFFFu) | (h.face << 16) | (1u << 24);
    if (dst.hit) *reinterpret_cast<uint4*>(dst.hit) = rec;
    if (dst.rgba) *dst.rgba = shade_rgba(A.mat_table, A.n_materials, h.material, h.face);
}

BLOK_DEV void camera_plane_uv(const TraceArgs& A, float pcx, float pcy, float& u, float& v) {
    const blok_camera& c = A.cam;
    const float qx = rn_div(pcx, static_cast<float>(A.frame_w));
    const float qy = rn_div(pcy, static_cast<float>(A.frame_h));
    u = rn_mul(rn_mul(rn_add(rn_sub(rn_mul(2.0f, qx), 1.0f), A.jitter_clip[0]), c.tan_half_fov), c.aspect);
    v = rn_mul(rn_sub(rn_sub(1.0f, rn_mul(2.0f, qy)), A.jitter_clip[1]), c.tan_half_fov);
}

BLOK_DEV RayIn primary_ray(const TraceArgs& A, uint32_t x, uint32_t y) {
    const blok_camera& c = A.cam;
    float u, v;
    camera_plane_uv(A, rn_add(static_cast<float>(x), 0.5f), rn_add(static_cast<float>(y), 0.5f), u, v);
    const float dx = rn_add(rn_add(c.fwd[0], rn_mul(c.right[0], u)), rn_mul(c.up[0], v));
    const float dy = rn_add(rn_add(c.fwd[1], rn_mul(c.right[1], u)), rn_mul(c.up[1], v));
    const float dz = rn_add(rn_add(c.fwd[2], rn_mul(c.right[2], u)), rn_mul(c.up[2], v));
    const float len = rn_sqrt(rn_add(rn_add(rn_mul(dx, dx), rn_mul(dy, dy)), rn_mul(dz, dz)));
    RayIn r;
    r.ox = c.pos[0]; r.oy = c.pos[1]; r.oz = c.pos[2];
    r.dx = rn_div(dx, len); r.dy = rn_div(dy, len); r.dz = rn_div(dz, len);
    r.tmin = A.tmin; r.tmax = A.tmax;
    return r;
}

}
#endif
```

blok_amd/csrc/hip/trace_kernels.h:

```cpp
#ifndef BLOK_TRACE_KERNELS_H
#define BLOK_TRACE_KERNELS_H

#ifdef BLOK_TRACE_HOST_HARNESS
#include "host_harness_shims.h"
#else
#include <hip/hip_runtime.h>
#endif
#include <stdint.h>

#include "blok_hip.h"
#include "tree.h"

namespace blok {

#ifndef BLOK_BLOCK_THREADS
#define BLOK_BLOCK_THREADS 64
#endif
constexpr int kBlock = BLOK_BLOCK_THREADS;
#ifndef BLOK_WAVE_W
#define BLOK_WAVE_W 8
#endif
constexpr uint32_t kWaveW = BLOK_WAVE_W, kWaveH = 64u / kWaveW;
constexpr uint32_t kTileW = kBlock >= 128 ? 2u * kWaveW : kWaveW;
constexpr uint32_t kTileH = kBlock >= 256 ? 2u * kWaveH : kWaveH;
// ... 101 lines not shown

struct UntileArgs {
    const void* gathered;
    void* frame;
    uint32_t frame_w, frame_h, tile, n_ranks, tiles_per_rank_max, tiles_x, elem_bytes;
    size_t gathered_frame_stride;
};

struct CompactArgs {
    const uint32_t* tiles;
    uint32_t* out;
    uint32_t tile, n_tiles, n_frames;
    size_t tiles_frame_stride;
};
struct CompactHitArgs {
    const blok_hit* hits;
    uint32_t* out;
    uint32_t tile, n_tiles, n_frames, n_materials;
    size_t hits_frame_stride;
};
struct ScatterArgs {
    const uint32_t* gathered;
    const uint32_t* const* rank_ptrs;
    uint32_t* frame;
    uint32_t* tile_map;
    uint8_t* tile_state;
    uint32_t frame_w, frame_h, tile, n_ranks, tiles_x, tiles_total, max_records, n_frames;
    size_t rank_stride;
    uint32_t record_words;
    const blok_material* mat_table;
    uint32_t n_materials;
};
void launch_compact_hit_tiles(const CompactHitArgs& args, hipStream_t stream);
void launch_compact_tiles(const CompactArgs& args, hipStream_t stream);
void launch_scatter_tiles(const ScatterArgs& args, bool codes, hipStream_t stream);
uint32_t sky_rgba();

struct SunMapArgs {
    TraceArgs trace;
    float u[3], v[3], s[3];
    float u0, v0, texel;
    uint32_t nu, nv;
    float* map;
    uint32_t iu0, iv0, sub_nu, sub_nv;
};
void launch_sun_map(const SunMapArgs& args, hipStream_t stream);
void launch_sun_map_raise(const SunMapArgs& args, float far_depth, hipStream_t stream);

struct PathArgs;
struct TonemapArgs;
struct AccumArgs;
void launch_accumulate(const AccumArgs& args, hipStream_t stream);
void launch_tonemap(const TonemapArgs& args, hipStream_t stream);
void launch_paths(const PathArgs& args, uint32_t n_blocks, hipStream_t stream);
struct TlasScene;
void launch_paths_instanced(const PathArgs& args, const TlasScene& scene, uint32_t stack_slots, uint32_t n_blocks, hipStream_t stream);
struct PoseScene;
struct LightScene;
void launch_paths_posed(const PathArgs& args, const TlasScene& scene, const PoseScene& poses, uint32_t stack_slots, uint32_t n_blocks, hipStream_t stream);
void launch_paths_lit(const PathArgs& args, const TlasScene& scene, const PoseScene& poses, const LightScene& lit, uint32_t stack_slots, uint32_t n_blocks,
                      hipStream_t stream);
void launch_trace(RayMode mode, const TraceArgs& args, uint32_t n_blocks, hipStream_t stream);
void launch_joint(RayMode mode, const TraceArgs& args, uint32_t n_beam_tiles, uint32_t n_blocks, hipStream_t stream);
constexpr uint32_t kJointPollBudget = 512u;
void launch_list_joint(RayMode mode, const TraceArgs& args, const TileFrames* frames, uint32_t n_beam_tiles, uint32_t n_walkers, hipStream_t stream);
void launch_list_walk(RayMode mode, const TraceArgs& args, const TileFrames* frames, uint32_t n_walkers, hipStream_t stream);
uint32_t beam_tiles(RayMode mode, const TraceArgs& args, uint32_t tiles_of_rank);
void launch_beam(RayMode mode, const TraceArgs& args, uint32_t n_beam_tiles, hipStream_t stream);
void launch_beam_fill(RayMode mode, const TraceArgs& args, uint32_t n_beam_tiles, const float* fine, hipStream_t stream);
uint32_t beam_refine_tiles(const TraceArgs& args);
bool beam_refine_applies(const TraceArgs& args);
void launch_beam_refine(const TraceArgs& args, float* fine, hipStream_t stream);
#ifndef BLOK_PACK_AREA
#define BLOK_PACK_AREA 32
#endif
static_assert(BLOK_PACK_AREA == 16 || BLOK_PACK_AREA == 32 || BLOK_PACK_AREA == 64, "whole wave tiles, and a stretch a workgroup can sort");
constexpr uint32_t kPackArea = BLOK_PACK_AREA, kPackStretch = kPackArea * kPackArea, kPackGroups = kPackStretch / 64u, kPackPad = 0xFFFFFFFFu;
constexpr uint32_t kPackKeyShift = 20u;
uint32_t pack_areas(const TraceArgs& args);
bool pack_applies(const TraceArgs& args);
void launch_trace_count(const TraceArgs& args, uint32_t n_blocks, uint8_t* trips, hipStream_t stream);
void launch_pack_build(const TraceArgs& args, const float* fine, const uint8_t* trips, uint32_t* list, uint32_t* words, hipStream_t stream);
void launch_packed_walk(const TraceArgs& args, const float* fine, const uint32_t* list, const uint32_t* table, uint32_t n_groups, hipStream_t stream);
void launch_trace_count_own(const TraceArgs& args, uint32_t n_blocks, uint8_t* trips, float* starts, uint8_t* restarts, hipStream_t stream);
void launch_pack_build_own(const TraceArgs& args, const float* fine, const uint8_t* restarts, const float* starts, uint32_t* list, uint32_t* words, float* slot_start, hipStream_t stream);
void launch_packed_walk_own(const TraceArgs& args, const float* slot_start, const uint32_t* list, const uint32_t* table, uint32_t n_groups, hipStream_t stream);
#ifndef BLOK_PACKED_FILL
#define BLOK_PACKED_FILL 4
#endif
uint32_t launch_packed_frame(const TraceArgs& args, const float* fine, const uint32_t* list, const uint32_t* table, uint32_t n_groups, uint32_t units_per_wave, hipStream_t stream);
uint32_t launch_packed_frame_own(const TraceArgs& args, const float* slot_start, const float* fine, const uint32_t* list, const uint32_t* table, uint32_t n_groups, uint32_t units_per_wave,
                                 hipStream_t stream);
void launch_untile(const UntileArgs& args, uint32_t n_frames, hipStream_t stream);
void launch_tile_frames(const TraceArgs& args, const TileFrames& frames, hipStream_t stream, uint32_t walk_blocks_per_frame = 0);
void launch_beam_frames(const TraceArgs& args, const TileFrames& frames, hipStream_t stream);
void launch_frame(RayMode mode, const TraceArgs& args, const FrameQueue& queue, uint32_t n_blocks, hipStream_t stream);
int frame_blocks_per_cu(RayMode mode, const TraceArgs& args);

}
#endif
```

blok_amd/csrc/hip/trace_kernels.hip:

```cpp
#include "trace_kernels.h"
#include "trace_core.h"
#include "path_core.h"
#include "beam.h"
#include "fill_units.h"

namespace blok {

namespace {

__device__ __forceinline__ bool block_to_tile(uint32_t b, uint32_t grid, uint32_t bx_count, uint32_t by_count,
                                              uint32_t& bx, uint32_t& by) {
#if BLOK_XCD_MAP == 0
    (void)grid;
    bx = b % bx_count; by = b / bx_count;
    return by < by_count;
#else
    const uint32_t vb = (b & 7u) * (grid >> 3) + (b >> 3);
#if BLOK_XCD_MAP == 1
    bx = vb % bx_count; by = vb / bx_count;
    return by < by_count;
#else
    const uint32_t super_x = (bx_count + kSuper - 1u) / kSuper;
    const uint32_t st = vb / (kSuper * kSuper), in = vb % (kSuper * kSuper);
    uint32_t mx = in & 0x55u, my = (in >> 1) & 0x55u;
// ... 60 lines not shown
        const float px = (u + 1.0f) * 0.5f * static_cast<float>(A.frame_w) - static_cast<float>(A.x0), py = (1.0f - v) * 0.5f * static_cast<float>(A.frame_h) - static_cast<float>(A.y0);
        if (!(px >= 0.0f && py >= 0.0f && px < static_cast<float>(A.w) && py < static_cast<float>(A.h))) return kListUnknownClass;
        was = min(static_cast<uint32_t>(py) / kTileH, by_count - 1u) * bx_count + min(static_cast<uint32_t>(px) / kTileW, bx_count - 1u);
    }
    const uint32_t c = Q.cost[was];
    if (c == 0u) return kListUnknownClass;
    return c >= kListCostClass3 ? 3u : (c >= kListCostClass2 ? 2u : (c >= kListCostClass1 ? 1u : 0u));
}

template <RayMode MODE>
__device__ __forceinline__ void list_publish(const TraceArgs& A, const uint32_t search, const uint32_t task_base, const uint32_t b, const float t0, const uint32_t lane) {
    const LiveList& Q = A.list;
    const uint32_t seg = search & (kListSegments - 1u);
    const uint32_t subs_x = A.beam_tile / kWaveW, subs_y = A.beam_tile / kWaveH;
    bool valid = false;
    uint32_t task = 0, cls = kListUnknownClass;
    if (t0 < kBeamNone && lane < subs_x * subs_y) {
        const uint32_t sx = lane % subs_x, sy = lane / subs_x;
        if constexpr (MODE == RayMode::Rect) {
            const uint32_t bx_count = (A.w + kTileW - 1u) / kTileW, by_count = (A.h + kTileH - 1u) / kTileH;
            const uint32_t bx = (b % A.beam_bx) * subs_x + sx, by = (b / A.beam_bx) * subs_y + sy;
            valid = bx < bx_count && by < by_count;
            task = by * bx_count + bx;
            if (valid) cls = list_class_rect(A, bx, by, bx_count, by_count, t0);
        } else {
            const uint32_t per_side = A.tile / kTileW, bps = A.tile / A.beam_tile;
            const uint32_t local_tile = b / (bps * bps), rem = b % (bps * bps);
            task = local_tile * per_side * (A.tile / kTileH) + ((rem / bps) * subs_y + sy) * per_side + (rem % bps) * subs_x + sx;
            valid = true;
        }
    }
    unsigned long long* const ctl = Q.ctl + seg * kListCtlWords;
    for (uint32_t c = 0; c < kListClasses; ++c) {
        const unsigned long long m = __ballot(valid && cls == c);
        if (m == 0ull) continue;
        const uint32_t n = static_cast<uint32_t>(__builtin_popcountll(m));
        const uint32_t pos = static_cast<uint32_t>(wave_fetch_add64(ctl + kListTally + c, n));
        if (valid && cls == c) {
            const uint32_t slot = pos + __builtin_amdgcn_mbcnt_hi(static_cast<uint32_t>(m >> 32), __builtin_amdgcn_mbcnt_lo(static_cast<uint32_t>(m), 0u));
            if (slot < Q.seg_capacity) list_st(Q.entries + (static_cast<size_t>(seg) * kListClasses + c) * Q.seg_capacity + slot, list_entry(Q.serial, task_base + task, t0));
        }
    }
    const uint32_t done = static_cast<uint32_t>(wave_fetch_add64(ctl + kListDone, 1ull));
    const uint32_t in_seg = (Q.n_searches + kListSegments - 1u - seg) / kListSegments;
    if (done + 1u == in_seg && lane < kListClasses) {
        const uint32_t total = min(static_cast<uint32_t>(list_ld(ctl + kListTally + lane)), Q.seg_capacity);
        list_st(ctl + kListFinal + lane, (static_cast<unsigned long long>(Q.serial) << 32) | total);
        list_st(ctl + kListTally + lane, 0ull);
        if (lane == 0) list_st(ctl + kListDone, 0ull);
        if (Q.hint) Q.hint[seg * kListClasses + lane] = total;
    }
}

__device__ __forceinline__ bool list_await(unsigned long long* slot, unsigned long long* final_word, unsigned long long* gave_up_word, const uint32_t serial, const uint32_t k,
                                           uint32_t* gave_up, uint32_t& task, float& t0) {
    for (uint32_t polls = 0; polls < kListPollBudget; ++polls) {
        const unsigned long long v = list_ld(slot);
        const uint32_t lo = __builtin_amdgcn_readfirstlane(static_cast<uint32_t>(v)), hi = __builtin_amdgcn_readfirstlane(static_cast<uint32_t>(v >> 32));
        if ((hi >> 12) == serial) {
            task = ((hi & 0xFFFu) << 9) | (lo >> 23);
            t0 = __uint_as_float((lo & 0x7FFFFFu) << 8);
            return true;
        }
#ifndef BLOK_LIST_FINAL_EVERY
#define BLOK_LIST_FINAL_EVERY 8
#endif
#ifndef BLOK_LIST_SLEEP
#define BLOK_LIST_SLEEP 32
#endif
        if ((polls & (BLOK_LIST_FINAL_EVERY - 1u)) == 0u) {
            const unsigned long long f = list_ld(final_word);
            const uint32_t flo = __builtin_amdgcn_readfirstlane(static_cast<uint32_t>(f)), fhi = __builtin_amdgcn_readfirstlane(static_cast<uint32_t>(f >> 32));
            if (fhi == serial && k >= flo) return false;
        }
        __builtin_amdgcn_s_sleep(BLOK_LIST_SLEEP);
    }
    list_st(gave_up_word, serial);
    if (gave_up && threadIdx.x == 0) (void)__hip_atomic_fetch_add(gave_up, 1u, __ATOMIC_RELAXED, __HIP_MEMORY_SCOPE_AGENT);
    return false;
}

template <RayMode MODE, bool kListed = false, bool kCount = false, bool kOwn = false>
__device__ __forceinline__ void trace_block(const TraceArgs& A, const uint32_t block, const uint32_t grid, uint4* lds_stack, const float listed_t0 = 0.0f,
                                            [[maybe_unused]] uint8_t* trips = nullptr, [[maybe_unused]] float* starts = nullptr, [[maybe_unused]] uint8_t* restarts = nullptr) {
    const uint32_t tid = threadIdx.x;
    uint4* stk = lds_stack + tid;

    if constexpr (MODE == RayMode::Rays) {
        const uint32_t i = block * kBlock + tid;
        if (i >= A.n_rays) return;
        const blok_ray ray = A.rays[i];
        RayIn r{ray.org[0], ray.org[1], ray.org[2], ray.dir[0], ray.dir[1], ray.dir[2], ray.tmin, ray.tmax};
        trace_one(A, r, stk, Sink{A.out ? A.out + i : nullptr, A.out_rgba ? A.out_rgba + i : nullptr});
        return;
    } else {
        const uint32_t wave = tid >> 6, lane = tid & 63u;
        const uint32_t lx = (wave & 1u) * kWaveW + (lane % kWaveW);
        const uint32_t ly = (wave >> 1) * kWaveH + (lane / kWaveW);
        const uint32_t wave_x = __builtin_amdgcn_readfirstlane((wave & 1u) * kWaveW), wave_y = __builtin_amdgcn_readfirstlane((wave >> 1) * kWaveH);
        uint32_t x, y;
        [[maybe_unused]] uint64_t clock0 = 0;
        [[maybe_unused]] uint32_t* cost_slot = nullptr;
        float t0 = 0.0f;
        size_t out_index;
        bool inside;
        if constexpr (MODE == RayMode::Rect) {
            const uint32_t bx_count = (A.w + kTileW - 1u) / kTileW, by_count = (A.h + kTileH - 1u) / kTileH;
            uint32_t bx, by;
            if constexpr (kListed) { bx = block % bx_count; by = block / bx_count; if (by >= by_count) return; }
            else {
                if (A.n_strip && block < A.n_strip) {
                    const uint32_t in_columns = A.strip_nx * by_count;
                    if (block < in_columns) { bx = A.strip_x0 + block % A.strip_nx; by = block / A.strip_nx; }
                    else { const uint32_t k = block - in_columns, w = bx_count - A.strip_nx; bx = k % w; if (bx >= A.strip_x0) bx += A.strip_nx; by = A.strip_y0 + k / w; }
                    if (bx >= bx_count || by >= by_count) return;
                } else {
                    const uint32_t entry = block - A.n_strip;
                    const uint32_t tile = A.order ? A.order[entry] : entry;
                    if (!block_to_tile(tile, grid, bx_count, by_count, bx, by)) return;
                    if (A.order) {
                        bx += A.order_sx; if (bx >= bx_count) bx -= bx_count;
                        by += A.order_sy; if (by >= by_count) by -= by_count;
                        if (A.n_strip && (bx - A.strip_x0 < A.strip_nx || by - A.strip_y0 < A.strip_ny)) return;
                    }
                }
                cost_slot = A.cost_out ? A.cost_out + (by * bx_count + bx) : nullptr;
            }
            if constexpr (kListed) t0 = listed_t0;
            else if (A.beam) {
                const uint32_t beam_index = ((by * kTileH + wave_y) / A.beam_tile) * A.beam_bx + (bx * kTileW + wave_x) / A.beam_tile;
                t0 = A.beam_slots ? await_beam(A.beam_slots + beam_index, A.beam_serial, A.joint_gave_up) : A.beam[beam_index];
                if (t0 >= kBeamNone) {
                    if (cost_slot && tid == 0) *cost_slot = 0u;
                    if (A.miss_in_walk) {
                        const uint32_t mx = bx * kTileW + lx, my = by * kTileH + ly;
                        const size_t at = static_cast<size_t>(my) * A.w + mx;
                        if (mx < A.w && my < A.h) write_miss(Sink{A.out ? A.out + at : nullptr, A.out_rgba ? A.out_rgba + at : nullptr});
                    }
                    return;
                }
            }
            const uint32_t rx = bx * kTileW + lx, ry = by * kTileH + ly;
            inside = rx < A.w && ry < A.h;
            x = A.x0 + rx; y = A.y0 + ry;
            out_index = static_cast<size_t>(ry) * A.w + rx;
        } else {
            const uint32_t per_side = A.tile / kTileW;
            const uint32_t per_tile = per_side * (A.tile / kTileH);
            const uint32_t wave_tile = (!kListed && A.order) ? A.order[block] : block;
            if constexpr (!kListed) cost_slot = A.cost_out ? A.cost_out + wave_tile : nullptr;
            const uint32_t local_tile = wave_tile / per_tile, sub = wave_tile % per_tile;
            const uint32_t global_tile = A.rank + local_tile * A.n_ranks;
            const uint32_t tx = global_tile % A.tiles_x, ty = global_tile / A.tiles_x;
            const uint32_t ix = (sub % per_side) * kTileW + lx, iy = (sub / per_side) * kTileH + ly;
            x = tx * A.tile + ix; y = ty * A.tile + iy;
            out_index = static_cast<size_t>(local_tile) * A.tile * A.tile + static_cast<size_t>(iy) * A.tile + ix;
            inside = x < A.frame_w && y < A.frame_h;
            if (global_tile >= A.tiles_total) {
                write_miss(Sink{A.out ? A.out + out_index : nullptr, A.out_rgba ? A.out_rgba + out_index : nullptr});
                if (cost_slot && tid == 0) *cost_slot = 0u;
                return;
            }
            if constexpr (kListed) t0 = listed_t0;
            else if (A.beam) {
                const uint32_t beams_per_side = A.tile / A.beam_tile;
                const uint32_t beam_index = (local_tile * beams_per_side + ((sub / per_side) * kTileH + wave_y) / A.beam_tile) * beams_per_side +
                                            ((sub % per_side) * kTileW + wave_x) / A.beam_tile;
                t0 = A.beam_slots ? await_beam(A.beam_slots + beam_index, A.beam_serial, A.joint_gave_up) : A.beam[beam_index];
                if (t0 >= kBeamNone) {
                    if (cost_slot && tid == 0) *cost_slot = 0u;
                    if (A.miss_in_walk) write_miss(Sink{A.out ? A.out + out_index : nullptr, A.out_rgba ? A.out_rgba + out_index : nullptr});
                    return;
                }
            }
        }
        const Sink sink{A.out ? A.out + out_index : nullptr, A.out_rgba ? A.out_rgba + out_index : nullptr};
        if (!inside) {
            if constexpr (MODE == RayMode::Tiles) {
                write_miss(sink);
                if (cost_slot && tid == 0) *cost_slot = 256u;
            }
            return;
        }
        if constexpr (MODE == RayMode::Rect) {
            if constexpr (kListed) cost_slot = A.debug_clocks ? A.debug_clocks + block : nullptr;
        }
        if (cost_slot && tid == 0) clock0 = __builtin_amdgcn_s_memtime();
        RayIn r = primary_ray(A, x, y);
        r.tmin = fmaxf(r.tmin, t0);
#ifndef BLOK_WAVE_START
#define BLOK_WAVE_START 1
#endif
        if constexpr (kOwn) trace_one<true, true, true>(A, r, stk, sink, trips + out_index, starts + out_index, restarts + out_index);
        else if constexpr (kCount) trace_one<true, true>(A, r, stk, sink, trips + out_index);
        else trace_one<BLOK_WAVE_START != 0>(A, r, stk, sink);
        if (cost_slot && tid == 0) *cost_slot = max(static_cast<uint32_t>(__builtin_amdgcn_s_memtime() - clock0), 256u);
    }
}

template <RayMode MODE>
__global__ __launch_bounds__(kBlock) void trace_kernel(const TraceArgs A) {
    extern __shared__ uint4 lds_stack[];
    trace_block<MODE>(A, blockIdx.x, gridDim.x, lds_stack);
}

__global__ __launch_bounds__(kBlock) void trace_count_kernel(const TraceArgs A, uint8_t* trips) {
    extern __shared__ uint4 lds_stack[];
    trace_block<RayMode::Rect, false, true>(A, blockIdx.x, gridDim.x, lds_stack, 0.0f, trips);
}

__global__ __launch_bounds__(kBlock) void trace_count_own_kernel(const TraceArgs A, uint8_t* trips, float* starts, uint8_t* restarts) {
    extern __shared__ uint4 lds_stack[];
    trace_block<RayMode::Rect, false, true, true>(A, blockIdx.x, gridDim.x, lds_stack, 0.0f, trips, starts, restarts);
}

__device__ __forceinline__ TraceArgs frame_args(const TraceArgs& A, const TileFrames& F, const uint32_t f) {
    TraceArgs L = A;
    L.cam = F.cam[f];
    if (L.out) L.out += f * F.frame_stride;
    if (L.out_rgba) L.out_rgba += f * F.frame_stride;
    if (L.beam) L.beam += static_cast<size_t>(f) * F.beams_per_frame;
    return L;
}

__global__ __launch_bounds__(kBlock) void trace_frames_kernel(const TraceArgs A, const TileFrames F) {
    extern __shared__ uint4 lds_stack[];
    const uint32_t f = blockIdx.x / F.blocks_per_frame;
    if (f >= F.n_frames) return;
    const TraceArgs L = frame_args(A, F, f);
    trace_block<RayMode::Tiles>(L, blockIdx.x - f * F.blocks_per_frame, F.blocks_per_frame, lds_stack);
}

__device__ __forceinline__ const TraceArgs& kernel_args() {
    return *(const TraceArgs*)__builtin_amdgcn_kernarg_segment_ptr();
}

template <RayMode MODE, bool kKept = false>
__device__ __forceinline__ void beam_block(const TraceArgs& A, const uint32_t b, const uint32_t n_beam_tiles, [[maybe_unused]] uint4* lds_stack = nullptr,
                                           const uint32_t list_search = 0u, const uint32_t list_task_base = 0u, [[maybe_unused]] const float* fine = nullptr) {
    const uint32_t lane = threadIdx.x;
    if (b >= n_beam_tiles) return;
    const uint32_t B = A.beam_tile;
    uint32_t px, py, px_end, py_end;
    [[maybe_unused]] uint32_t tile_x0 = 0, tile_y0 = 0;
    [[maybe_unused]] size_t tile_base = 0;
    bool padding = false;
    if constexpr (MODE == RayMode::Rect) {
        px = A.x0 + (b % A.beam_bx) * B; py = A.y0 + (b / A.beam_bx) * B;
        px_end = min(px + B, A.x0 + A.w); py_end = min(py + B, A.y0 + A.h);
    } else {
        const uint32_t per_side = A.tile / B, per_tile = per_side * per_side;
        const uint32_t local_tile = b / per_tile, sub = b % per_tile;
        const uint32_t global_tile = A.rank + local_tile * A.n_ranks;
        padding = global_tile >= A.tiles_total;
        if (padding && !A.list.entries && A.miss_in_walk) { if (lane == 0) { if (A.beam_slots) publish_beam(A.beam_slots + b, A.beam_serial, kBeamNone); else A.beam[b] = kBeamNone; } return; }
        tile_x0 = (global_tile % A.tiles_x) * A.tile; tile_y0 = (global_tile / A.tiles_x) * A.tile;
        tile_base = static_cast<size_t>(local_tile) * A.tile * A.tile;
        px = tile_x0 + (sub % per_side) * B; py = tile_y0 + (sub / per_side) * B;
        px_end = px + B; py_end = py + B;
    }
    float t0;
    if constexpr (kKept) t0 = __uint_as_float(__builtin_amdgcn_readfirstlane(__float_as_uint(A.beam[b])));
    else {
        uint32_t visits = 0;
        t0 = padding ? kBeamNone : beam_start(A, static_cast<float>(px), static_cast<float>(py), static_cast<float>(px_end), static_cast<float>(py_end), lane, kBeamNone,
                                              &visits);
        if (A.debug_visits && lane == 0) A.debug_visits[b] = visits;
        if (A.list.entries) list_publish<MODE>(A, list_search, list_task_base, b, t0, lane);
        else if (lane == 0) { if (A.beam_slots) publish_beam(A.beam_slots + b, A.beam_serial, t0); else A.beam[b] = t0; }
    }
    if (t0 >= kBeamNone && (A.list.entries || !A.miss_in_walk) && (A.out || A.out_rgba)) {
        const uint32_t tw = px_end - px, n = tw * (py_end - py);
        for (uint32_t i = lane; i < n; i += 64u) {
            const uint32_t x = px + i % tw, y = py + i / tw;
            size_t out_index;
            if constexpr (MODE == RayMode::Rect) out_index = static_cast<size_t>(y - A.y0) * A.w + (x - A.x0);
            else out_index = tile_base + static_cast<size_t>(y - tile_y0) * A.tile + (x - tile_x0);
            write_miss(Sink{A.out ? A.out + out_index : nullptr, A.out_rgba ? A.out_rgba + out_index : nullptr});
        }
    }
    if constexpr (MODE == RayMode::Rect && kBlock == 64 && kKept) {
        if (fine && t0 < kBeamNone) {
            const uint32_t bx_count = (A.w + kTileW - 1u) / kTileW, by_count = (A.h + kTileH - 1u) / kTileH;
            const uint32_t bx0 = (px - A.x0) / kTileW, bx1 = (px_end - A.x0 + kTileW - 1u) / kTileW;
            const uint32_t by0 = (py - A.y0) / kTileH, by1 = (py_end - A.y0 + kTileH - 1u) / kTileH;
            uint32_t walked = 0u;
            for (uint32_t by = by0; by < by1; ++by)
                for (uint32_t bx = bx0; bx < bx1; ++bx) {
                    const uint32_t tile = by * bx_count + bx;
                    const float f0 = __uint_as_float(__builtin_amdgcn_readfirstlane(__float_as_uint(fine[tile])));
                    const uint32_t rx = bx * kTileW + lane % kWaveW, ry = by * kTileH + lane / kWaveW;
                    const bool inside = rx < A.w && ry < A.h;
                    const size_t at = static_cast<size_t>(ry) * A.w + rx;
                    if (f0 >= kBeamNone) {
                        if (inside && !A.miss_in_walk) write_miss(Sink{A.out ? A.out + at : nullptr, A.out_rgba ? A.out_rgba + at : nullptr});
                        continue;
// ... 86 lines not shown
    float t0 = kBeamNone;
    if (coarse < kBeamNone) {
        const uint32_t px = A.x0 + bx * kWaveW, py = A.y0 + by * kWaveH;
        const float own = beam_start(A, static_cast<float>(px), static_cast<float>(py), static_cast<float>(min(px + kWaveW, A.x0 + A.w)), static_cast<float>(min(py + kWaveH, A.y0 + A.h)), lane);
        t0 = own >= kBeamNone ? kBeamNone : fmaxf(own, coarse);
    }
    if (lane == 0) fine[tile] = t0;
}

constexpr uint32_t kPackThreads = kPackStretch < 1024u ? kPackStretch : 1024u;
__global__ __launch_bounds__(kPackThreads) void pack_build_kernel(const uint8_t* trips, const float* fine, const uint32_t w, const uint32_t h, uint32_t* list, uint32_t* words) {
    constexpr uint32_t kChunks = kPackStretch / 64u, kWaves = kPackThreads / 64u, kRounds = kChunks / kWaves, kKeys = 256u, kTilesX = kPackArea / kWaveW;
    static_assert(kPackStretch % kPackThreads == 0u && kPackStretch <= 65535u && kPackGroups <= kPackThreads && kPackThreads >= kKeys, "the counts fit 16 bits; a thread per key and per group");
    __shared__ uint16_t in_chunk[kChunks][kKeys];
    __shared__ uint32_t key_base[kKeys + 1u];
    const uint32_t p = threadIdx.x, lane = p & 63u, wave = p >> 6;
    const uint32_t areas_x = (w + kPackArea - 1u) / kPackArea;
    uint32_t rx[kRounds], ry[kRounds], count[kRounds], rank[kRounds];
    bool valid[kRounds], any = false;
    for (uint32_t r = 0; r < kRounds; ++r) {
        const uint32_t chunk = r * kWaves + wave;
        rx[r] = (blockIdx.x % areas_x) * kPackArea + (chunk % kTilesX) * kWaveW + lane % kWaveW;
        ry[r] = (blockIdx.x / areas_x) * kPackArea + (chunk / kTilesX) * kWaveH + lane / kWaveW;
        valid[r] = rx[r] < w && ry[r] < h && fine[(ry[r] / kWaveH) * ((w + kWaveW - 1u) / kWaveW) + rx[r] / kWaveW] < kBeamNone;
        count[r] = valid[r] ? trips[static_cast<size_t>(ry[r]) * w + rx[r]] : 0u;
        rank[r] = 0u;
        any = any || valid[r];
    }
    for (uint32_t i = p; i < kChunks * kKeys; i += kPackThreads) (&in_chunk[0][0])[i] = 0u;
    if (!__syncthreads_or(any)) {
        if (p < kPackGroups) words[blockIdx.x * kPackGroups + p] = 0u;
        return;
    }
    for (uint32_t r = 0; r < kRounds; ++r) {
        const uint32_t key = 255u - count[r];
        unsigned long long remaining = __ballot(valid[r]);
        while (remaining) {
            const uint32_t k = __builtin_amdgcn_readlane(key, static_cast<int>(__builtin_ctzll(remaining)));
            const unsigned long long m = __ballot(valid[r] && key == k);
            if (valid[r] && key == k) rank[r] = __builtin_amdgcn_mbcnt_hi(static_cast<uint32_t>(m >> 32), __builtin_amdgcn_mbcnt_lo(static_cast<uint32_t>(m), 0u));
            if (lane == 0u) in_chunk[r * kWaves + wave][k] = static_cast<uint16_t>(__builtin_popcountll(m));
            remaining &= ~m;
        }
    }
    __syncthreads();
    if (p < kKeys) {
        uint32_t sum = 0u;
        for (uint32_t v = 0; v < kChunks; ++v) { const uint32_t c = in_chunk[v][p]; in_chunk[v][p] = static_cast<uint16_t>(sum); sum += c; }
        key_base[p] = sum;
    }
    __syncthreads();
    if (wave == 0u) {
        static_assert(kKeys == 4u * 64u, "four keys per lane");
        uint32_t c[4], mine = 0u;
        for (uint32_t j = 0; j < 4u; ++j) { c[j] = key_base[lane * 4u + j]; mine += c[j]; }
        uint32_t incl = mine;
        for (uint32_t off = 1u; off < 64u; off <<= 1) { const uint32_t u = __shfl_up(incl, off); if (lane >= off) incl += u; }
        uint32_t before = incl - mine;
        for (uint32_t j = 0; j < 4u; ++j) { key_base[lane * 4u + j] = before; before += c[j]; }
        if (lane == 63u) key_base[kKeys] = incl;
    }
    __syncthreads();
    const uint32_t n = key_base[kKeys], padded = (n + 63u) & ~63u;
    uint32_t* const stretch = list + static_cast<size_t>(blockIdx.x) * kPackStretch;
    for (uint32_t r = 0; r < kRounds; ++r)
        if (valid[r]) {
            const uint32_t key = 255u - count[r];
            const uint32_t at = key_base[key] + in_chunk[r * kWaves + wave][key] + rank[r];
            stretch[at] = rx[r] | (ry[r] << 16);
            if ((at & 63u) == 0u) words[blockIdx.x * kPackGroups + (at >> 6)] = ((count[r] + 1u) << kPackKeyShift) | (blockIdx.x * kPackGroups + (at >> 6));
        }
    if (n + p < padded) stretch[n + p] = kPackPad;
    if (p < kPackGroups && p * 64u >= n) words[blockIdx.x * kPackGroups + p] = 0u;
}

__global__ __launch_bounds__(256) void pack_starts_kernel(const uint32_t* list, const float* starts, const uint32_t w, const uint32_t h, const uint32_t n_entries, float* slot_start) {
    const uint32_t i = blockIdx.x * 256u + threadIdx.x;
    if (i >= n_entries) return;
    const uint32_t entry = list[i], rx = entry & 0xFFFFu, ry = entry >> 16;
    if (entry == kPackPad || rx >= w || ry >= h) return;
    slot_start[i] = starts[static_cast<size_t>(ry) * w + rx];
}

__global__ __launch_bounds__(kBlock) void packed_walk_kernel(const TraceArgs A, const float* fine, const uint32_t* list, const uint32_t* table) {
    static_assert(kBlock == 64, "one wave per group");
    extern __shared__ uint4 lds_stack[];
    const uint32_t lane = threadIdx.x;
    const uint32_t group = __builtin_amdgcn_readfirstlane(table[blockIdx.x]) & ((1u << kPackKeyShift) - 1u);
    const uint32_t entry = list[static_cast<size_t>(group) * 64u + lane];
    const uint32_t rx = entry & 0xFFFFu, ry = entry >> 16;
    if (entry == kPackPad || rx >= A.w || ry >= A.h) return;
    const float t0 = fine[(ry / kWaveH) * ((A.w + kWaveW - 1u) / kWaveW) + rx / kWaveW];
    const size_t at = static_cast<size_t>(ry) * A.w + rx;
    RayIn r = primary_ray(A, A.x0 + rx, A.y0 + ry);
    r.tmin = fmaxf(r.tmin, t0);
    trace_one<true>(A, r, lds_stack + lane, Sink{A.out ? A.out + at : nullptr, A.out_rgba ? A.out_rgba + at : nullptr});
}

__global__ __launch_bounds__(kBlock) void packed_walk_own_kernel(const TraceArgs A, const float* slot_start, const uint32_t* list, const uint32_t* table) {
    static_assert(kBlock == 64, "one wave per group");
    extern __shared__ uint4 lds_stack[];
    const uint32_t lane = threadIdx.x;
    const uint32_t group = __builtin_amdgcn_readfirstlane(table[blockIdx.x]) & ((1u << kPackKeyShift) - 1u);
    const uint32_t entry = list[static_cast<size_t>(group) * 64u + lane];
    const float t0 = slot_start[static_cast<size_t>(group) * 64u + lane];
    const uint32_t rx = entry & 0xFFFFu, ry = entry >> 16;
    if (entry == kPackPad || rx >= A.w || ry >= A.h) return;
    const size_t at = static_cast<size_t>(ry) * A.w + rx;
    RayIn r = primary_ray(A, A.x0 + rx, A.y0 + ry);
    r.tmin = fmaxf(r.tmin, t0);
    trace_one<true>(A, r, lds_stack + lane, Sink{A.out ? A.out + at : nullptr, A.out_rgba ? A.out_rgba + at : nullptr});
}

#ifndef BLOK_PACKED_FILL_FIRST
#define BLOK_PACKED_FILL_FIRST 0
#endif
#ifndef BLOK_PACKED_FILL_NT
#define BLOK_PACKED_FILL_NT 1
#endif
__device__ __forceinline__ void fill_units_of_workgroup(const TraceArgs& A, const float* fine, const uint32_t n_units, const uint32_t units_x) {
    if (!A.out && !A.out_rgba) return;
    const uint32_t lane = threadIdx.x, tiles_x = (A.w + kWaveW - 1u) / kWaveW;
    constexpr uint32_t kBatch = 4u;
    for (uint32_t i = 0u; fill_unit_of(blockIdx.x, i, gridDim.x) < n_units; i += kBatch) {
        float bound[kBatch];
        size_t at[kBatch];
#pragma unroll
        for (uint32_t j = 0; j < kBatch; ++j) {
            const uint32_t u = fill_unit_of(blockIdx.x, i + j, gridDim.x);
            const uint32_t ry = fill_unit_row(u, units_x), rx = fill_unit_x0(u, units_x) + lane;
            at[j] = static_cast<size_t>(ry) * A.w + rx;
            bound[j] = u < n_units && rx < A.w && ry < A.h ? fine[(ry / kWaveH) * tiles_x + rx / kWaveW] : 0.0f;
        }
#pragma unroll
        for (uint32_t j = 0; j < kBatch; ++j)
            if (bound[j] >= kBeamNone) {
#if BLOK_PACKED_FILL_NT
                typedef uint32_t u32x4 __attribute__((ext_vector_type(4)));
                if (A.out) __builtin_nontemporal_store(u32x4{0xBF800000u, 0u, 0u, 0x00FF0000u}, reinterpret_cast<u32x4*>(A.out + at[j]));
                if (A.out_rgba) __builtin_nontemporal_store(kSkyRgba, A.out_rgba + at[j]);
#else
                write_miss(Sink{A.out ? A.out + at[j] : nullptr, A.out_rgba ? A.out_rgba + at[j] : nullptr});
#endif
            }
    }
}

__global__ __launch_bounds__(kBlock) void packed_frame_kernel(const TraceArgs A, const float* fine, const uint32_t* list, const uint32_t* table, const uint32_t n_groups,
                                                              const uint32_t n_units, const uint32_t units_x) {
    static_assert(kBlock == 64, "one wave per group, one lane per pixel of a unit");
    extern __shared__ uint4 lds_stack[];
    const uint32_t lane = threadIdx.x;
    if constexpr (BLOK_PACKED_FILL_FIRST != 0) fill_units_of_workgroup(A, fine, n_units, units_x);
    if (blockIdx.x < n_groups) {
        const uint32_t group = __builtin_amdgcn_readfirstlane(table[blockIdx.x]) & ((1u << kPackKeyShift) - 1u);
        const uint32_t entry = list[static_cast<size_t>(group) * 64u + lane];
        const uint32_t rx = entry & 0xFFFFu, ry = entry >> 16;
        if (entry != kPackPad && rx < A.w && ry < A.h) {
            const float t0 = fine[(ry / kWaveH) * ((A.w + kWaveW - 1u) / kWaveW) + rx / kWaveW];
            const size_t at = static_cast<size_t>(ry) * A.w + rx;
            RayIn r = primary_ray(A, A.x0 + rx, A.y0 + ry);
            r.tmin = fmaxf(r.tmin, t0);
            trace_one<true>(A, r, lds_stack + lane, Sink{A.out ? A.out + at : nullptr, A.out_rgba ? A.out_rgba + at : nullptr});
        }
    }
    if constexpr (BLOK_PACKED_FILL_FIRST == 0) fill_units_of_workgroup(A, fine, n_units, units_x);
}

__global__ __launch_bounds__(kBlock) void packed_frame_own_kernel(const TraceArgs A, const float* slot_start, const float* fine, const uint32_t* list, const uint32_t* table,
                                                                  const uint32_t n_groups, const uint32_t n_units, const uint32_t units_x) {
    static_assert(kBlock == 64, "one wave per group, one lane per pixel of a unit");
    extern __shared__ uint4 lds_stack[];
    const uint32_t lane = threadIdx.x;
    if constexpr (BLOK_PACKED_FILL_FIRST != 0) fill_units_of_workgroup(A, fine, n_units, units_x);
    if (blockIdx.x < n_groups) {
        const uint32_t group = __builtin_amdgcn_readfirstlane(table[blockIdx.x]) & ((1u << kPackKeyShift) - 1u);
        const uint32_t entry = list[static_cast<size_t>(group) * 64u + lane];
        const float t0 = slot_start[static_cast<size_t>(group) * 64u + lane];
        const uint32_t rx = entry & 0xFFFFu, ry = entry >> 16;
        if (entry != kPackPad && rx < A.w && ry < A.h) {
            const size_t at = static_cast<size_t>(ry) * A.w + rx;
            RayIn r = primary_ray(A, A.x0 + rx, A.y0 + ry);
            r.tmin = fmaxf(r.tmin, t0);
            trace_one<true>(A, r, lds_stack + lane, Sink{A.out ? A.out + at : nullptr, A.out_rgba ? A.out_rgba + at : nullptr});
        }
    }
    if constexpr (BLOK_PACKED_FILL_FIRST == 0) fill_units_of_workgroup(A, fine, n_units, units_x);
}

template <RayMode MODE>
__global__ __launch_bounds__(kBlock) void joint_kernel(const TraceArgs A, const uint32_t n_beam_tiles) {
    extern __shared__ uint4 lds_stack[];
    if (blockIdx.x < n_beam_tiles) {
        if (threadIdx.x < 64u) beam_block<MODE>(kernel_args(), blockIdx.x, n_beam_tiles, lds_stack);
        return;
    }
    trace_block<MODE>(A, blockIdx.x - n_beam_tiles, gridDim.x - n_beam_tiles, lds_stack);
}

__global__ __launch_bounds__(64) void beam_frames_kernel(const TraceArgs A, const TileFrames F) {
    extern __shared__ uint4 lds_stack[];
    const uint32_t f = blockIdx.x / F.beams_per_frame;
    if (f >= F.n_frames) return;
    const TraceArgs L = frame_args(A, F, f);
    beam_block<RayMode::Tiles>(L, blockIdx.x - f * F.beams_per_frame, F.beams_per_frame, A.rank_of ? lds_stack : nullptr, blockIdx.x, f * F.blocks_per_frame);
}

template <RayMode MODE, bool kFrames>
__device__ __forceinline__ void list_task(const TraceArgs& A, const TileFrames& F, const uint32_t task, const float t0, uint4* lds_stack) {
    if constexpr (kFrames) {
        const uint32_t f = task / F.blocks_per_frame;
        if (f >= F.n_frames) return;
        const TraceArgs L = frame_args(A, F, f);
        trace_block<MODE, true>(L, task - f * F.blocks_per_frame, F.blocks_per_frame, lds_stack, t0);
    } else {
        [[maybe_unused]] uint64_t clock0 = 0;
        if constexpr (MODE == RayMode::Rect) { if (A.list.cost) clock0 = __builtin_amdgcn_s_memtime(); }
        trace_block<MODE, true>(A, task, 0u, lds_stack, t0);
        if constexpr (MODE == RayMode::Rect) {
            if (A.list.cost && threadIdx.x == 0) A.list.cost[task] = max(static_cast<uint32_t>(__builtin_amdgcn_s_memtime() - clock0), 1u);
        }
    }
}

template <RayMode MODE, bool kFrames>
__device__ __forceinline__ void list_walk(const TraceArgs& A, const TileFrames& F, const uint32_t walker, const uint32_t seg, uint4* lds_stack) {
    const LiveList& Q = A.list;
    if (seg >= Q.n_searches) return;
    uint32_t k = walker / kListSegments, cls = kListClasses - 1u;
    while (cls != 0u && k >= Q.walkers[cls]) { k -= Q.walkers[cls]; cls -= 1u; }
    const uint32_t stride = Q.walkers[cls];
    if (k >= stride) return;
    unsigned long long* const entries = Q.entries + (static_cast<size_t>(seg) * kListClasses + cls) * Q.seg_capacity;
    unsigned long long* const ctl = Q.ctl + seg * kListCtlWords;
    for (; k < Q.seg_capacity; k += stride) {
        uint32_t task; float t0;
        if (!list_await(entries + k, ctl + kListFinal + cls, ctl + kListGaveUp, Q.serial, k, A.joint_gave_up, task, t0)) return;
        __hip_atomic_store(entries + k, 0ull, __ATOMIC_RELAXED, __HIP_MEMORY_SCOPE_AGENT);
        list_task<MODE, kFrames>(A, F, task, t0, lds_stack);
    }
}

template <RayMode MODE, bool kFrames>
__device__ __forceinline__ void list_search(const TraceArgs& A, const TileFrames& F, const uint32_t search) {
    if constexpr (kFrames) {
        const uint32_t f = search / F.beams_per_frame;
        if (f >= F.n_frames) return;
        const TraceArgs L = frame_args(A, F, f);
        beam_block<MODE>(L, search - f * F.beams_per_frame, F.beams_per_frame, nullptr, search, f * F.blocks_per_frame);
    } else {
        beam_block<MODE>(A, search, A.list.n_searches, nullptr, search, 0u);
    }
}

template <RayMode MODE, bool kFrames>
__global__ __launch_bounds__(kBlock) void list_joint_kernel(const TraceArgs A, const TileFrames F) {
    static_assert(kBlock == 64, "one wave per workgroup");
    extern __shared__ uint4 lds_stack[];
    const uint32_t n = A.list.n_searches;
    if (blockIdx.x < n) { list_search<MODE, kFrames>(A, F, blockIdx.x); return; }
    list_walk<MODE, kFrames>(A, F, blockIdx.x - n, blockIdx.x & (kListSegments - 1u), lds_stack);
}

template <RayMode MODE, bool kFrames>
__global__ __launch_bounds__(kBlock) void list_walk_kernel(const TraceArgs A, const TileFrames F) {
    extern __shared__ uint4 lds_stack[];
    list_walk<MODE, kFrames>(A, F, blockIdx.x, blockIdx.x & (kListSegments - 1u), lds_stack);
// ... 545 lines not shown
    }
}

void launch_joint(RayMode mode, const TraceArgs& args, uint32_t n_beam_tiles, uint32_t n_blocks, hipStream_t stream) {
    if (n_beam_tiles + n_blocks == 0 || mode == RayMode::Rays) return;
    const size_t lds = static_cast<size_t>(args.levels > 1 ? args.levels - 1 : 1) * kBlock * sizeof(uint4);
    if (mode == RayMode::Rect) hipLaunchKernelGGL(joint_kernel<RayMode::Rect>, dim3(n_beam_tiles + n_blocks), dim3(kBlock), lds, stream, args, n_beam_tiles);
    else hipLaunchKernelGGL(joint_kernel<RayMode::Tiles>, dim3(n_beam_tiles + n_blocks), dim3(kBlock), lds, stream, args, n_beam_tiles);
}

void launch_list_joint(RayMode mode, const TraceArgs& args, const TileFrames* frames, uint32_t n_beam_tiles, uint32_t n_walkers, hipStream_t stream) {
    if (n_beam_tiles == 0 || mode == RayMode::Rays || !args.list.entries) return;
    const size_t lds = frame_lds_bytes(args);
    const dim3 grid(n_beam_tiles + n_walkers), clean(kListSegments * 8u);
    const TileFrames none{};
    if (mode == RayMode::Rect) {
        hipLaunchKernelGGL((list_joint_kernel<RayMode::Rect, false>), grid, dim3(kBlock), lds, stream, args, none);
        hipLaunchKernelGGL((list_cleanup_kernel<RayMode::Rect, false>), clean, dim3(kBlock), lds, stream, args, none);
    } else if (!frames) {
        hipLaunchKernelGGL((list_joint_kernel<RayMode::Tiles, false>), grid, dim3(kBlock), lds, stream, args, none);
        hipLaunchKernelGGL((list_cleanup_kernel<RayMode::Tiles, false>), clean, dim3(kBlock), lds, stream, args, none);
    } else {
        hipLaunchKernelGGL((list_joint_kernel<RayMode::Tiles, true>), grid, dim3(kBlock), lds, stream, args, *frames);
        hipLaunchKernelGGL((list_cleanup_kernel<RayMode::Tiles, true>), clean, dim3(kBlock), lds, stream, args, *frames);
    }
}

void launch_list_walk(RayMode mode, const TraceArgs& args, const TileFrames* frames, uint32_t n_walkers, hipStream_t stream) {
    if (n_walkers == 0 || mode == RayMode::Rays || !args.list.entries) return;
    const size_t lds = frame_lds_bytes(args);
    const TileFrames none{};
    if (mode == RayMode::Rect) hipLaunchKernelGGL((list_walk_kernel<RayMode::Rect, false>), dim3(n_walkers), dim3(kBlock), lds, stream, args, none);
    else if (!frames) hipLaunchKernelGGL((list_walk_kernel<RayMode::Tiles, false>), dim3(n_walkers), dim3(kBlock), lds, stream, args, none);
    else hipLaunchKernelGGL((list_walk_kernel<RayMode::Tiles, true>), dim3(n_walkers), dim3(kBlock), lds, stream, args, *frames);
}

uint32_t beam_tiles(RayMode mode, const TraceArgs& a, uint32_t tiles_of_rank) {
    if (mode == RayMode::Rect) return ((a.w + a.beam_tile - 1u) / a.beam_tile) * ((a.h + a.beam_tile - 1u) / a.beam_tile);
    return tiles_of_rank * (a.tile / a.beam_tile) * (a.tile / a.beam_tile);
}

void launch_beam(RayMode mode, const TraceArgs& args, uint32_t n_beam_tiles, hipStream_t stream) {
    if (n_beam_tiles == 0 || mode == RayMode::Rays) return;
    const size_t lds = args.rank_of ? frame_lds_bytes(args) : 0;
    if (mode == RayMode::Rect) hipLaunchKernelGGL(beam_kernel<RayMode::Rect>, dim3(n_beam_tiles), dim3(64), lds, stream, args, n_beam_tiles);
    else hipLaunchKernelGGL(beam_kernel<RayMode::Tiles>, dim3(n_beam_tiles), dim3(64), lds, stream, args, n_beam_tiles);
}

void launch_beam_fill(RayMode mode, const TraceArgs& args, uint32_t n_beam_tiles, const float* fine, hipStream_t stream) {
    if (n_beam_tiles == 0 || mode != RayMode::Rect || !args.beam || args.beam_slots || args.list.entries) return;
    const size_t lds = args.rank_of ? frame_lds_bytes(args) : 0;
    hipLaunchKernelGGL(beam_fill_kernel<RayMode::Rect>, dim3(n_beam_tiles), dim3(64), lds, stream, args, n_beam_tiles, fine);
}

uint32_t beam_refine_tiles(const TraceArgs& a) { return ((a.w + kWaveW - 1u) / kWaveW) * ((a.h + kWaveH - 1u) / kWaveH); }

bool beam_refine_applies(const TraceArgs& a) {
    return kBlock == 64 && kWaveW == kWaveH && a.beam_tile > kWaveW && a.beam_tile % kWaveW == 0u;
}

void launch_beam_refine(const TraceArgs& args, float* fine, hipStream_t stream) {
    const uint32_t n = beam_refine_tiles(args);
    if (n == 0 || !fine || !args.beam || args.beam_slots || !beam_refine_applies(args)) return;
    hipLaunchKernelGGL(beam_refine_kernel, dim3(n), dim3(64), 0, stream, args, fine);
}

uint32_t pack_areas(const TraceArgs& a) { return ((a.w + kPackArea - 1u) / kPackArea) * ((a.h + kPackArea - 1u) / kPackArea); }

bool pack_applies(const TraceArgs& a) {
    return kBlock == 64 && kWaveW == 8u && kWaveH == 8u && a.w && a.h && a.w < 0xFFFFu && a.h < 0xFFFFu &&
           static_cast<uint64_t>(pack_areas(a)) * kPackGroups <= (1u << kPackKeyShift);
}

void launch_trace_count(const TraceArgs& args, uint32_t n_blocks, uint8_t* trips, hipStream_t stream) {
    if (n_blocks == 0 || !trips) return;
    hipLaunchKernelGGL(trace_count_kernel, dim3(n_blocks), dim3(kBlock), frame_lds_bytes(args), stream, args, trips);
}

void launch_pack_build(const TraceArgs& args, const float* fine, const uint8_t* trips, uint32_t* list, uint32_t* words, hipStream_t stream) {
    if (!pack_applies(args) || !fine || !trips || !list || !words) return;
    hipLaunchKernelGGL(pack_build_kernel, dim3(pack_areas(args)), dim3(kPackThreads), 0, stream, trips, fine, args.w, args.h, list, words);
}

void launch_trace_count_own(const TraceArgs& args, uint32_t n_blocks, uint8_t* trips, float* starts, uint8_t* restarts, hipStream_t stream) {
    if (n_blocks == 0 || !trips || !starts || !restarts) return;
    hipLaunchKernelGGL(trace_count_own_kernel, dim3(n_blocks), dim3(kBlock), frame_lds_bytes(args), stream, args, trips, starts, restarts);
}

void launch_pack_build_own(const TraceArgs& args, const float* fine, const uint8_t* restarts, const float* starts, uint32_t* list, uint32_t* words, float* slot_start, hipStream_t stream) {
    if (!pack_applies(args) || !fine || !restarts || !starts || !list || !words || !slot_start) return;
    hipLaunchKernelGGL(pack_build_kernel, dim3(pack_areas(args)), dim3(kPackThreads), 0, stream, restarts, fine, args.w, args.h, list, words);
    const uint32_t n_entries = pack_areas(args) * kPackStretch;
    hipLaunchKernelGGL(pack_starts_kernel, dim3((n_entries + 255u) / 256u), dim3(256), 0, stream, list, starts, args.w, args.h, n_entries, slot_start);
}

void launch_packed_walk_own(const TraceArgs& args, const float* slot_start, const uint32_t* list, const uint32_t* table, uint32_t n_groups, hipStream_t stream) {
    if (n_groups == 0 || !pack_applies(args) || !slot_start || !list || !table) return;
    hipLaunchKernelGGL(packed_walk_own_kernel, dim3(n_groups), dim3(kBlock), frame_lds_bytes(args), stream, args, slot_start, list, table);
}

void launch_packed_walk(const TraceArgs& args, const float* fine, const uint32_t* list, const uint32_t* table, uint32_t n_groups, hipStream_t stream) {
    if (n_groups == 0 || !pack_applies(args) || !fine || !list || !table) return;
    hipLaunchKernelGGL(packed_walk_kernel, dim3(n_groups), dim3(kBlock), frame_lds_bytes(args), stream, args, fine, list, table);
}

uint32_t launch_packed_frame(const TraceArgs& args, const float* fine, const uint32_t* list, const uint32_t* table, uint32_t n_groups, uint32_t units_per_wave, hipStream_t stream) {
    if (n_groups == 0 || units_per_wave == 0 || !pack_applies(args) || !fine || !list || !table) return 0u;
    const FillGrid g = fill_grid(args.w, args.h, n_groups, units_per_wave);
    hipLaunchKernelGGL(packed_frame_kernel, dim3(g.grid), dim3(kBlock), frame_lds_bytes(args), stream, args, fine, list, table, n_groups, g.n_units, g.units_x);
    return g.grid - n_groups;
}

uint32_t launch_packed_frame_own(const TraceArgs& args, const float* slot_start, const float* fine, const uint32_t* list, const uint32_t* table, uint32_t n_groups, uint32_t units_per_wave,
                                 hipStream_t stream) {
    if (n_groups == 0 || units_per_wave == 0 || !pack_applies(args) || !slot_start || !fine || !list || !table) return 0u;
    const FillGrid g = fill_grid(args.w, args.h, n_groups, units_per_wave);
    hipLaunchKernelGGL(packed_frame_own_kernel, dim3(g.grid), dim3(kBlock), frame_lds_bytes(args), stream, args, slot_start, fine, list, table, n_groups, g.n_units, g.units_x);
    return g.grid - n_groups;
}

size_t frame_lds_bytes(const TraceArgs& args) { return static_cast<size_t>(args.levels > 1 ? args.levels - 1 : 1) * kBlock * sizeof(uint4); }

int frame_blocks_per_cu(RayMode mode, const TraceArgs& args) {
    int n = 0;
    const hipError_t e = mode == RayMode::Rect
        ? hipOccupancyMaxActiveBlocksPerMultiprocessor(&n, frame_kernel<RayMode::Rect>, kBlock, frame_lds_bytes(args))
        : hipOccupancyMaxActiveBlocksPerMultiprocessor(&n, frame_kernel<RayMode::Tiles>, kBlock, frame_lds_bytes(args));
    return e == hipSuccess ? n : 0;
}

void launch_frame(RayMode mode, const TraceArgs& args, const FrameQueue& queue, uint32_t n_blocks, hipStream_t stream) {
    if (n_blocks == 0 || mode == RayMode::Rays) return;
    const size_t lds = frame_lds_bytes(args);
    if (mode == RayMode::Rect) hipLaunchKernelGGL(frame_kernel<RayMode::Rect>, dim3(n_blocks), dim3(kBlock), lds, stream, args, queue);
    else hipLaunchKernelGGL(frame_kernel<RayMode::Tiles>, dim3(n_blocks), dim3(kBlock), lds, stream, args, queue);
}

void launch_sun_map(const SunMapArgs& args, hipStream_t stream) {
    const uint32_t n = args.sub_nu * args.sub_nv;
    if (n) hipLaunchKernelGGL(sun_map_kernel, dim3(n), dim3(64), 0, stream, args);
}

void launch_sun_map_raise(const SunMapArgs& args, float far_depth, hipStream_t stream) {
    const uint32_t n = args.sub_nu * args.sub_nv;
    if (n) hipLaunchKernelGGL(sun_map_raise_kernel, dim3((n + 63u) / 64u), dim3(64), 0, stream, args, far_depth);
}

void launch_paths(const PathArgs& args, uint32_t n_blocks, hipStream_t stream) {
    if (n_blocks == 0) return;
    const uint32_t levels = args.trace.levels;
    size_t lds = static_cast<size_t>(levels > 1 ? levels - 1 : 1) * kBlock * sizeof(uint4);
    const size_t tail_lds = args.tail_pool ? (kTailBatch + 1u) * sizeof(TailAnswer) : 0u;
    if (args.resume_secondary && levels >= 2) {
        lds += (static_cast<size_t>(levels - 2) * kBlock * (sizeof(uint2) + sizeof(uint32_t)) + 15u) / 16u * 16u;
        hipLaunchKernelGGL(path_kernel<true>, dim3(n_blocks), dim3(kBlock), lds + tail_lds, stream, args);
    } else hipLaunchKernelGGL(path_kernel<false>, dim3(n_blocks), dim3(kBlock), lds + tail_lds, stream, args);
}

void launch_paths_instanced(const PathArgs& args, const TlasScene& scene, uint32_t stack_slots, uint32_t n_blocks, hipStream_t stream) {
    if (n_blocks == 0) return;
    const uint32_t levels = args.trace.levels;
    uint32_t slots = levels > 1 ? levels - 1 : 1;
    if (stack_slots > slots) slots = stack_slots;
    hipLaunchKernelGGL(path_kernel_instanced, dim3(n_blocks), dim3(kBlock), static_cast<size_t>(slots) * kBlock * sizeof(uint4), stream, args, scene);
}

void launch_pose_tlas_build(const blok_pose* poses, uint32_t n, const ModelDesc* models, uint32_t n_models, float vs, const float cam[3], TlasNode* nodes,
                            hipStream_t stream) {
    if (n == 0u || n > kTlasMax) return;
    hipLaunchKernelGGL(pose_tlas_build_kernel, dim3(1), dim3(kTlasBuildThreads), 0, stream, poses, n, models, n_models, vs, cam[0], cam[1], cam[2], nodes);
}

void launch_paths_posed(const PathArgs& args, const TlasScene& scene, const PoseScene& poses, uint32_t stack_slots, uint32_t n_blocks, hipStream_t stream) {
    if (n_blocks == 0) return;
    uint32_t slots = args.trace.levels > 1u ? args.trace.levels - 1u : 1u;
    if (stack_slots > slots) slots = stack_slots;
    hipLaunchKernelGGL(path_kernel_posed, dim3(n_blocks), dim3(kBlock), static_cast<size_t>(slots) * kBlock * sizeof(uint4), stream, args, scene, poses);
}

void launch_paths_lit(const PathArgs& args, const TlasScene& scene, const PoseScene& poses, const LightScene& lit, uint32_t stack_slots, uint32_t n_blocks,
                      hipStream_t stream) {
    if (n_blocks == 0 || lit.n == 0u) return;
    uint32_t slots = args.trace.levels > 1u ? args.trace.levels - 1u : 1u;
    if (stack_slots > slots) slots = stack_slots;
    hipLaunchKernelGGL(path_kernel_lit, dim3(n_blocks), dim3(kBlock), static_cast<size_t>(slots) * kBlock * sizeof(uint4), stream, args, scene, poses, lit);
}

void launch_tlas_build(const blok_instance* instances, uint32_t n, const ModelDesc* models, uint32_t n_models, TlasNode* nodes, hipStream_t stream) {
    if (n == 0u || n > kTlasMax) return;
    hipLaunchKernelGGL(tlas_build_kernel, dim3(1), dim3(kTlasBuildThreads), 0, stream, instances, n, models, n_models, nodes);
}

void launch_tonemap(const TonemapArgs& args, hipStream_t stream) {
    if (args.n) hipLaunchKernelGGL(tonemap_kernel, dim3((args.n + 255u) / 256u), dim3(256), 0, stream, args);
}

void launch_accumulate(const AccumArgs& args, hipStream_t stream) {
    if (args.n) hipLaunchKernelGGL(accumulate_kernel, dim3((args.n + 255u) / 256u), dim3(256), 0, stream, args);
}

// ... 9 lines not shown
```

blok_amd/tracer.py:

```python
from __future__ import annotations

import ctypes as C

import numpy as np

from . import _ffi
from ._ffi import BlokError, CAMERA, GBuffer, HIT, INSTANCE, MATERIAL, POSE, RAY, SUB_CHUNK, SVO_NODE, WorldStats


def _vec3(v):
    return None if v is None else (C.c_int32 * 3)(*[int(c) for c in v])


class HipTracer:
    def __init__(self, width: int, height: int, device: int = 0):
        self.width, self.height, self.device = int(width), int(height), int(device)
        self._lib = None
        self._ctx = None
        self._beam_tile = 32

    def init(self) -> "HipTracer":
        self._lib = _ffi.hip_lib()
        ctx = C.c_void_p()
        rc = self._lib.blok_hip_create(C.byref(ctx), self.device, self.width, self.height)
# ... 399 lines not shown
        return info, texels

    def set_beam(self, beam_tile_pixels: int):
        self._check(self._lib.blok_hip_set_beam(self._ctx, beam_tile_pixels))
        self._beam_tile = int(beam_tile_pixels)

    def set_taa_jitter(self, jitter_px=None):
        if jitter_px is None:
            self._check(self._lib.blok_hip_set_taa_jitter(self._ctx, None))
        else:
            j = (C.c_float * 2)(float(jitter_px[0]), float(jitter_px[1]))
            self._check(self._lib.blok_hip_set_taa_jitter(self._ctx, j))

    def set_rt_taa_jitter(self, enabled: bool):
        self._check(self._lib.blok_hip_set_rt_taa_jitter(self._ctx, 1 if enabled else 0))

    def beam_prepass(self, cam, rect=None, want_visits=False):
        x0, y0, w, h = rect or (0, 0, self.width, self.height)
        tile = self._beam_tile
        n = ((w + tile - 1) // tile) * ((h + tile - 1) // tile)
        t0 = np.zeros(n, dtype=np.float32)
        visits = np.zeros(n, dtype=np.uint32) if want_visits else None
        cam = np.ascontiguousarray(cam)
        self._check(self._lib.blok_hip_beam_prepass(self._ctx, C.c_void_p(cam.ctypes.data), x0, y0, w, h, C.c_void_p(t0.ctypes.data),
                                                    C.c_void_p(visits.ctypes.data) if want_visits else None, n))
        return t0, visits

    def trace_wave_tiles_device(self, cam, tiles, t0, hits_ptr=0, rgba_ptr=0, rect=None, stream=0):
        x0, y0, w, h = rect or (0, 0, self.width, self.height)
        tiles = np.ascontiguousarray(tiles, dtype=np.uint32)
        t0 = None if t0 is None else np.ascontiguousarray(t0, dtype=np.float32)
        cam = np.ascontiguousarray(cam)
        self._check(self._lib.blok_hip_trace_wave_tiles_device(self._ctx, C.c_void_p(cam.ctypes.data), x0, y0, w, h, C.c_void_p(tiles.ctypes.data),
                                                               C.c_void_p(t0.ctypes.data) if t0 is not None else None, len(tiles),
                                                               C.c_void_p(hits_ptr) if hits_ptr else None, C.c_void_p(rgba_ptr) if rgba_ptr else None,
                                                               C.c_void_p(stream) if stream else None))

    def set_debug_wave_clocks(self, dev_ptr):
        self._check(self._lib.blok_hip_set_debug_wave_clocks(self._ctx, C.c_void_p(dev_ptr) if dev_ptr else None))

    def set_tile_ordering(self, resort_every_n_frames):
        n = 8 if resort_every_n_frames is True else int(resort_every_n_frames or 0)
        self._check(self._lib.blok_hip_set_tile_ordering(self._ctx, n))

    def set_rank_tile_ordering(self, enabled: bool):
        self._check(self._lib.blok_hip_set_rank_tile_ordering(self._ctx, int(bool(enabled))))

    def set_moving_order(self, enabled: bool):
        self._check(self._lib.blok_hip_set_moving_order(self._ctx, 1 if enabled else 0))

    def debug_class_order(self, cost, radius, beam=None):
        cost = np.ascontiguousarray(cost, dtype=np.uint32)
        ty, tx = cost.shape
        order = np.zeros(tx * ty, dtype=np.uint32); rank = np.zeros(tx * ty, dtype=np.uint32)
        live = C.c_uint32(0); sums = np.zeros(3, dtype=np.float32)
        b = None if beam is None else np.ascontiguousarray(beam, dtype=np.float32)
        self._check(self._lib.blok_hip_debug_class_order(self._ctx, C.c_void_p(cost.ctypes.data), tx, ty, int(radius), C.c_void_p(b.ctypes.data) if b is not None else None,
                                                         0 if b is None else len(b), C.c_void_p(order.ctypes.data), C.c_void_p(rank.ctypes.data), C.byref(live), C.c_void_p(sums.ctypes.data)))
        return order, rank, live.value, sums

    def debug_force_order_shift(self, shift=None):
        self._check(self._lib.blok_hip_debug_force_order_shift(self._ctx, 0 if shift is None else 1, *(shift or (0, 0))))

    def last_fallback_tiles(self) -> int:
        return int(self._lib.blok_hip_last_fallback_tiles(self._ctx))

    def last_order_use(self):
        sx, sy = C.c_int32(0), C.c_int32(0)
        return self._lib.blok_hip_last_order_use(self._ctx, C.byref(sx), C.byref(sy)), sx.value, sy.value

    def set_joint_prefix_limit(self, max_walk_waves: int):
        self._check(self._lib.blok_hip_set_joint_prefix_limit(self._ctx, max_walk_waves))

    def set_list_classes(self, enabled: bool):
        self._check(self._lib.blok_hip_set_list_classes(self._ctx, 1 if enabled else 0))

    def last_launch_kind(self) -> int:
        return int(self._lib.blok_hip_last_launch_kind(self._ctx))

    def set_miss_writer(self, in_walk: bool):
        self._check(self._lib.blok_hip_set_miss_writer(self._ctx, 1 if in_walk else 0))

    def set_beam_cache(self, mode):
        self._check(self._lib.blok_hip_set_beam_cache(self._ctx, (4 if mode else 0) if isinstance(mode, bool) else int(mode)))

    def set_beam_refine_after(self, hits: int):
        self._check(self._lib.blok_hip_set_beam_refine_after(self._ctx, hits))

    def set_beam_list_after(self, hits: int):
        self._check(self._lib.blok_hip_set_beam_list_after(self._ctx, hits))

    def beam_cache_list_builds(self) -> int:
        n = C.c_uint64(0)
        self._check(self._lib.blok_hip_beam_cache_list_builds(self._ctx, C.byref(n)))
        return int(n.value)

    def pack_area(self) -> int:
        return int(self._lib.blok_hip_pack_area())

    def beam_cache_list_state(self) -> int:
        state = C.c_int(0)
        self._check(self._lib.blok_hip_beam_cache_download_list(self._ctx, C.byref(state), None, None, None, 0, None, 0, None, 0))
        return int(state.value)

    def beam_cache_list(self, w: int, h: int):
        state, areas, groups = C.c_int(0), C.c_uint32(0), C.c_uint32(0)
        self._check(self._lib.blok_hip_beam_cache_download_list(self._ctx, C.byref(state), C.byref(areas), None, None, 0, None, 0, None, 0))
        if not state.value:
            return None
        stretch = self.pack_area() ** 2
        entries = np.zeros((int(areas.value), stretch), dtype=np.uint32)
        table = np.zeros(int(areas.value) * (stretch // 64), dtype=np.uint32)
        trips = np.zeros((h, w), dtype=np.uint8)
        self._check(self._lib.blok_hip_beam_cache_download_list(self._ctx, C.byref(state), C.byref(areas), C.byref(groups), _ffi.ptr(entries), entries.size,
                                                                 _ffi.ptr(table), table.size, _ffi.ptr(trips), trips.size))
        return int(state.value), int(groups.value), entries, table, trips

    def beam_cache_starts_state(self) -> int:
        state = C.c_int(0)
        self._check(self._lib.blok_hip_beam_cache_download_starts(self._ctx, C.byref(state), None, 0, None, 0))
        return int(state.value)

    def beam_cache_starts(self, w: int, h: int):
        state, areas = C.c_int(0), C.c_uint32(0)
        self._check(self._lib.blok_hip_beam_cache_download_list(self._ctx, C.byref(state), C.byref(areas), None, None, 0, None, 0, None, 0))
        starts = np.zeros((int(areas.value), self.pack_area() ** 2), dtype=np.float32)
        restarts = np.zeros((h, w), dtype=np.uint8)
        self._check(self._lib.blok_hip_beam_cache_download_starts(self._ctx, None, _ffi.ptr(starts), starts.size, _ffi.ptr(restarts), restarts.size))
        return starts, restarts

    def beam_cache_start_counters(self):
        used, other = C.c_uint64(0), C.c_uint64(0)
        self._check(self._lib.blok_hip_beam_cache_start_counters(self._ctx, C.byref(used), C.byref(other)))
        return int(used.value), int(other.value)

    def set_packed_fill(self, units_per_wave: int):
        self._check(self._lib.blok_hip_set_packed_fill(self._ctx, int(units_per_wave)))

    def packed_fill_counters(self):
        frames, tail = C.c_uint64(0), C.c_uint64(0)
        self._check(self._lib.blok_hip_packed_fill_counters(self._ctx, C.byref(frames), C.byref(tail)))
        return int(frames.value), int(tail.value)

    def beam_cache_refines(self) -> int:
        n = C.c_uint64(0)
        self._check(self._lib.blok_hip_beam_cache_refines(self._ctx, C.byref(n)))
        return int(n.value)

    def beam_cache_fine_state(self) -> int:
        state = C.c_int(0)
        self._check(self._lib.blok_hip_beam_cache_download_fine(self._ctx, C.byref(state), None, None, 0))
        return int(state.value)

    def beam_cache_fine(self):
        state, n = C.c_int(0), C.c_uint32(0)
        self._check(self._lib.blok_hip_beam_cache_download_fine(self._ctx, C.byref(state), C.byref(n), None, 0))
        if not state.value:
            return 0, None
        t0 = np.zeros(int(n.value), dtype=np.float32)
        self._check(self._lib.blok_hip_beam_cache_download_fine(self._ctx, C.byref(state), C.byref(n), _ffi.ptr(t0), len(t0)))
        return int(state.value), t0

    def beam_cache_counters(self):
        hits, fills = C.c_uint64(0), C.c_uint64(0)
        self._check(self._lib.blok_hip_beam_cache_counters(self._ctx, C.byref(hits), C.byref(fills)))
        return int(hits.value), int(fills.value)

    def beam_cache_last(self):
        action, n = C.c_int(0), C.c_uint32(0)
        self._check(self._lib.blok_hip_beam_cache_download(self._ctx, C.byref(action), C.byref(n), None, 0))
        if not action.value:
            return 0, None
        t0 = np.zeros(int(n.value), dtype=np.float32)
        self._check(self._lib.blok_hip_beam_cache_download(self._ctx, C.byref(action), C.byref(n), _ffi.ptr(t0), len(t0)))
        return int(action.value), t0

    def beam_cache_last_action(self) -> int:
        action = C.c_int(0)
        self._check(self._lib.blok_hip_beam_cache_download(self._ctx, C.byref(action), None, None, 0))
        return int(action.value)

    def set_beam_budget(self, max_node_visits: int):
        self._check(self._lib.blok_hip_set_beam_budget(self._ctx, max_node_visits))

    def set_voxel_size(self, voxel_size: float):
        self._check(self._lib.blok_hip_set_voxel_size(self._ctx, float(voxel_size)))

    def set_dense_dda(self, enabled: bool):
        self._check(self._lib.blok_hip_set_dense_dda(self._ctx, 1 if enabled else 0))

    def set_fused(self, enabled: bool):
        self._check(self._lib.blok_hip_set_fused(self._ctx, int(enabled)))

    def frame_queue_stalls(self) -> int:
        n = C.c_uint32(0)
        self._check(self._lib.blok_hip_frame_queue_stalls(self._ctx, C.byref(n)))
        return int(n.value)

    def reset_accum(self):
        self._check(self._lib.blok_hip_reset_accum(self._ctx))

    def _check(self, rc: int):
        if rc != 0:
            raise BlokError(rc, self._lib.blok_hip_last_error(self._ctx).decode())

    def add_world(self, world) -> WorldStats:
        nodes = np.ascontiguousarray(world.nodes, dtype=SVO_NODE)
        subs = np.ascontiguousarray(world.sub_chunks, dtype=SUB_CHUNK)
        mats = np.ascontiguousarray(world.materials, dtype=MATERIAL)
        self._check(self._lib.blok_hip_upload_world(self._ctx, _ffi.ptr(nodes), len(nodes), _ffi.ptr(subs), len(subs),
                                                    _ffi.ptr(mats), len(mats)))
        return self.world_stats()

    update_world = add_world

    def add_dense(self, material_ids: np.ndarray, origin=(0, 0, 0), materials: np.ndarray | None = None) -> WorldStats:
        ids = np.ascontiguousarray(material_ids, dtype=np.uint32)
        nz, ny, nx = ids.shape
# ... 450 lines not shown
```

include/blok_hip_debug.h:

```cpp
#ifndef BLOK_HIP_DEBUG_H
#define BLOK_HIP_DEBUG_H

#include "blok_hip.h"

#ifdef __cplusplus
extern "C" {
#endif

int blok_hip_set_host_build(blok_hip_ctx* ctx, int enabled);
int blok_hip_world_built_on_device(const blok_hip_ctx* ctx);
int blok_hip_download_tree(const blok_hip_ctx* ctx, void* nodes_out, size_t node_capacity,
                           uint32_t* materials_out, size_t material_capacity);

int blok_hip_set_volume_layout(blok_hip_ctx* ctx, int keyed);
int blok_hip_volume_refresh_counts(blok_hip_ctx* ctx, uint64_t out_counts[3]);
int blok_hip_volume_flood_counters(blok_hip_ctx* ctx, uint64_t out_counts[2]);

int blok_hip_set_ray_batching(blok_hip_ctx* ctx, int enabled);
int blok_hip_set_path_start(blok_hip_ctx* ctx, int resume_from_anchor, int wave_tile_beam);
int blok_hip_set_sun_map(blok_hip_ctx* ctx, int enabled);

int blok_hip_set_beam(blok_hip_ctx* ctx, uint32_t beam_tile_pixels);
int blok_hip_set_tile_ordering(blok_hip_ctx* ctx, int resort_every_n_frames);
int blok_hip_set_moving_order(blok_hip_ctx* ctx, int enabled);
int blok_hip_set_rank_tile_ordering(blok_hip_ctx* ctx, int enabled);
int blok_hip_debug_class_order(blok_hip_ctx* ctx, const uint32_t* cost_host, uint32_t tiles_x, uint32_t tiles_y, uint32_t radius, const float* beam_host, uint32_t n_beams,
                               uint32_t* out_order_host, uint32_t* out_rank_of_host, uint32_t* out_live, float* out_depth_sums3);
int64_t blok_hip_last_fallback_tiles(const blok_hip_ctx* ctx);
int blok_hip_debug_force_order_shift(blok_hip_ctx* ctx, int enabled, uint32_t shift_x, uint32_t shift_y);
int blok_hip_last_order_use(const blok_hip_ctx* ctx, int32_t* out_shift_x, int32_t* out_shift_y);
int blok_hip_set_joint_prefix_limit(blok_hip_ctx* ctx, uint32_t max_walk_waves);
int blok_hip_set_miss_writer(blok_hip_ctx* ctx, int in_walk);
int blok_hip_set_beam_cache(blok_hip_ctx* ctx, int mode);
int blok_hip_set_beam_list_after(blok_hip_ctx* ctx, uint32_t hits);
uint32_t blok_hip_pack_area(void);
int blok_hip_beam_cache_list_builds(const blok_hip_ctx* ctx, uint64_t* out_builds);
int blok_hip_beam_cache_download_list(blok_hip_ctx* ctx, int* out_state, uint32_t* out_n_areas, uint32_t* out_n_groups, uint32_t* out_list_host_or_null, size_t list_capacity,
                                      uint32_t* out_table_host_or_null, size_t table_capacity, uint8_t* out_trips_host_or_null, size_t trips_capacity);
int blok_hip_beam_cache_download_starts(blok_hip_ctx* ctx, int* out_state, float* out_starts_host_or_null, size_t starts_capacity, uint8_t* out_restarts_host_or_null,
                                        size_t restarts_capacity);
int blok_hip_beam_cache_start_counters(const blok_hip_ctx* ctx, uint64_t* out_from_starts, uint64_t* out_other_key);
int blok_hip_set_packed_fill(blok_hip_ctx* ctx, uint32_t units_per_wave);
int blok_hip_packed_fill_counters(const blok_hip_ctx* ctx, uint64_t* out_one_launch_frames, uint64_t* out_fill_only_workgroups);
int blok_hip_beam_cache_counters(const blok_hip_ctx* ctx, uint64_t* out_hits, uint64_t* out_fills);
int blok_hip_beam_cache_refines(const blok_hip_ctx* ctx, uint64_t* out_refines);
int blok_hip_set_beam_refine_after(blok_hip_ctx* ctx, uint32_t hits);
int blok_hip_beam_cache_download(blok_hip_ctx* ctx, int* out_action, uint32_t* out_n_beams, float* out_t0_host_or_null, size_t capacity);
int blok_hip_beam_cache_download_fine(blok_hip_ctx* ctx, int* out_state, uint32_t* out_n_tiles, float* out_t0_host_or_null, size_t capacity);
int blok_hip_set_beam_budget(blok_hip_ctx* ctx, uint32_t max_node_visits);
int blok_hip_set_fused(blok_hip_ctx* ctx, int enabled);
int blok_hip_frame_queue_stalls(blok_hip_ctx* ctx, uint32_t* out_stalled_waves);
int blok_hip_beam_prepass(blok_hip_ctx* ctx, const blok_camera* cam, uint32_t x0, uint32_t y0, uint32_t w, uint32_t h,
                          float* out_t0_host, uint32_t* out_visits_host_or_null, size_t capacity);
int blok_hip_trace_wave_tiles_device(blok_hip_ctx* ctx, const blok_camera* cam, uint32_t x0, uint32_t y0, uint32_t w, uint32_t h,
                                     const uint32_t* tiles_host, const float* t0_host_or_null, size_t n_tiles,
                                     void* out_hits_dev_or_null, void* out_rgba8_dev_or_null, void* hip_stream);
int blok_hip_set_debug_wave_clocks(blok_hip_ctx* ctx, void* clocks_dev_or_null);
typedef struct blok_sun_map_info {
    float    u[3], v[3], s[3];
    float    u0, v0, texel;
    uint32_t nu, nv;
    uint32_t has_map;
    uint32_t loose_edits;
    uint32_t tighten_pending;
    uint32_t pending_u0, pending_u1, pending_v0, pending_v1;
} blok_sun_map_info;
int blok_hip_sun_map_download(blok_hip_ctx* ctx, blok_sun_map_info* out_info, float* map_out_or_null, size_t capacity);
int blok_hip_last_launch_kind(const blok_hip_ctx* ctx);
int blok_hip_set_list_classes(blok_hip_ctx* ctx, int enabled);

int blok_hip_multi_debug_deny_peer_access(blok_hip_multi* m, int deny);

int blok_hip_debug_build_tlas(blok_hip_ctx* ctx, const blok_instance* instances_dev, uint32_t n_instances, void* out_nodes_host, size_t capacity,
                              uint32_t* out_count);

int blok_hip_debug_build_pose_tlas(blok_hip_ctx* ctx, const blok_camera* cam, const blok_pose* poses_dev, uint32_t n_poses, void* out_nodes_host,
                                   size_t capacity, uint32_t* out_count);
int blok_hip_set_pose_tlas(blok_hip_ctx* ctx, int enabled);

int blok_hip_debug_pose_motion_records(blok_hip_ctx* ctx, const blok_pose* cur_host, uint32_t n_cur, const blok_pose* prev_host, uint32_t n_prev,
                                       blok_pose_motion* out_records_host);

typedef struct blok_model_info {
    uint32_t levels;
    int32_t  origin[3];
    int32_t  lo[3], hi[3];
    uint64_t n_nodes, n_materials;
} blok_model_info;
int blok_hip_download_model(blok_hip_ctx* ctx, uint32_t model, void* nodes_out, size_t node_capacity, uint32_t* materials_out,
                            size_t material_capacity, blok_model_info* out_info);

#ifdef __cplusplus
}
#endif
#endif
```

Before: 193,900 Mrays/s.

## Cache per-ray restart node words so packed rays resume at the recorded node

Adds a beam-cache mode in which the counting trace records, for each ray, the index and level of the SVO node that contains its restart point. Pack build stores these node words next to each list entry, and a new packed-frame kernel enters the walk directly at that node instead of descending from the root. It is meant to remove the repeated top-down descent for cached rays. In exchange it adds per-pixel and per-entry node buffers, extra kernel work while building, and a whole-wave fallback to the full trace if any lane fails to settle.

```diff
diff --git a/blok_amd/_ffi.py b/blok_amd/_ffi.py
--- a/blok_amd/_ffi.py
+++ b/blok_amd/_ffi.py
@@ -343,6 +343,8 @@
     "blok_hip_beam_cache_counters": (C.c_int, [C.c_void_p, C.POINTER(C.c_uint64), C.POINTER(C.c_uint64)]),
     "blok_hip_beam_cache_download_starts": (C.c_int, [C.c_void_p, C.c_void_p, C.c_void_p, C.c_size_t, C.c_void_p, C.c_size_t]),
     "blok_hip_beam_cache_start_counters": (C.c_int, [C.c_void_p, C.POINTER(C.c_uint64), C.POINTER(C.c_uint64)]),
+    "blok_hip_beam_cache_download_nodes": (C.c_int, [C.c_void_p, C.c_void_p, C.c_void_p, C.c_size_t, C.c_void_p, C.c_size_t]),
+    "blok_hip_beam_cache_node_counters": (C.c_int, [C.c_void_p, C.POINTER(C.c_uint64)]),
     "blok_hip_set_packed_fill": (C.c_int, [C.c_void_p, C.c_uint32]),
     "blok_hip_packed_fill_counters": (C.c_int, [C.c_void_p, C.POINTER(C.c_uint64), C.POINTER(C.c_uint64)]),
     "blok_hip_beam_cache_refines": (C.c_int, [C.c_void_p, C.POINTER(C.c_uint64)]),
diff --git a/blok_amd/csrc/hip/api.hip b/blok_amd/csrc/hip/api.hip
--- a/blok_amd/csrc/hip/api.hip
+++ b/blok_amd/csrc/hip/api.hip
@@ -261,7 +261,7 @@
 
 extern "C" {
 
-uint32_t blok_hip_abi_version(void) { return (1u << 16) | 26u; }
+uint32_t blok_hip_abi_version(void) { return (1u << 16) | 27u; }
 
 const char* blok_hip_last_error(const blok_hip_ctx* ctx) { return ctx ? ctx->error.c_str() : g_create_error.c_str(); }
 
diff --git a/blok_amd/csrc/hip/api_debug.hip b/blok_amd/csrc/hip/api_debug.hip
--- a/blok_amd/csrc/hip/api_debug.hip
+++ b/blok_amd/csrc/hip/api_debug.hip
@@ -315,6 +315,7 @@
     ctx->beam_cache.refine = mode >= 2;
     ctx->beam_cache.packed = mode >= 3;
     ctx->beam_cache.policy.own_starts = mode >= 4;
+    ctx->beam_cache.policy.node_restart = mode >= 5;
     blok::beam_cache_clear(ctx->beam_cache.policy);
     if (!ctx->beam_cache.packed) return BLOK_OK;
     BLOK_HIP_TRY(ctx, hipSetDevice(ctx->device));
@@ -388,6 +389,32 @@
     return BLOK_OK;
 }
 
+int blok_hip_beam_cache_download_nodes(blok_hip_ctx* ctx, int* out_has_nodes, uint32_t* out_entry_words_host, size_t entry_capacity, uint32_t* out_pixel_words_host, size_t pixel_capacity) {
+    if (!ctx) return BLOK_ERR_INVALID_ARG;
+    const auto& B = ctx->beam_cache;
+    const bool has = B.last_list && B.last_slot >= 0 && static_cast<uint32_t>(B.last_slot) < blok::kBeamCacheSlots && B.policy.starts[B.last_slot] && B.policy.nodes[B.last_slot] &&
+                     B.slots[B.last_slot].d_node;
+    if (out_has_nodes) *out_has_nodes = has ? 1 : 0;
+    if (!out_entry_words_host && !out_pixel_words_host) return BLOK_OK;
+    if (!has) return set_error(ctx, BLOK_ERR_INVALID_ARG, "beam cache: the latest launch's slot has no list with node words");
+    const auto& sl = B.slots[B.last_slot];
+    const size_t entries = static_cast<size_t>(sl.n_words / blok::kPackGroups) * blok::kPackStretch, pixels = static_cast<size_t>(B.last_w) * B.last_h;
+    if (entries > sl.d_node.capacity() || pixels > B.d_ray_node.capacity()) return set_error(ctx, BLOK_ERR_INVALID_ARG, "beam cache: the node words' buffers are gone (a resize)");
+    if ((out_entry_words_host && entry_capacity < entries) || (out_pixel_words_host && pixel_capacity < pixels))
+        return set_error(ctx, BLOK_ERR_INVALID_ARG, "beam cache: output smaller than the list or the rectangle");
+    BLOK_HIP_TRY(ctx, hipSetDevice(ctx->device));
+    BLOK_HIP_TRY(ctx, hipDeviceSynchronize());
+    if (out_entry_words_host) BLOK_HIP_TRY(ctx, hipMemcpy(out_entry_words_host, sl.d_node, entries * sizeof(uint32_t), hipMemcpyDeviceToHost));
+    if (out_pixel_words_host) BLOK_HIP_TRY(ctx, hipMemcpy(out_pixel_words_host, B.d_ray_node, pixels * sizeof(uint32_t), hipMemcpyDeviceToHost));
+    return BLOK_OK;
+}
+
+int blok_hip_beam_cache_node_counters(const blok_hip_ctx* ctx, uint64_t* out_from_nodes) {
+    if (!ctx) return BLOK_ERR_INVALID_ARG;
+    if (out_from_nodes) *out_from_nodes = ctx->beam_cache.node_hits;
+    return BLOK_OK;
+}
+
 int blok_hip_set_packed_fill(blok_hip_ctx* ctx, uint32_t units_per_wave) {
     if (!ctx) return BLOK_ERR_INVALID_ARG;
     ctx->beam_cache.packed_fill = units_per_wave;
diff --git a/blok_amd/csrc/hip/api_internal.h b/blok_amd/csrc/hip/api_internal.h
--- a/blok_amd/csrc/hip/api_internal.h
+++ b/blok_amd/csrc/hip/api_internal.h
@@ -152,12 +152,15 @@
             bool used = false;
             blok::DeviceArray<uint32_t> d_list, d_table;
             blok::DeviceArray<float> d_start;
+            blok::DeviceArray<uint32_t> d_node;
             uint32_t n_words = 0, n_groups = 0;
         } slots[blok::kBeamCacheSlots];
         bool packed = true;
         blok::DeviceArray<uint8_t> d_trips;
         blok::DeviceArray<float> d_ray_start;
         blok::DeviceArray<uint8_t> d_restarts;
+        blok::DeviceArray<uint32_t> d_ray_node;
+        uint64_t node_hits = 0;
         blok::DeviceArray<uint32_t> d_words;
         blok::DeviceBytes d_sort_temp; size_t sort_temp_bytes = 0;
         blok::PinnedArray<uint32_t> h_groups;
diff --git a/blok_amd/csrc/hip/api_launch.hip b/blok_amd/csrc/hip/api_launch.hip
--- a/blok_amd/csrc/hip/api_launch.hip
+++ b/blok_amd/csrc/hip/api_launch.hip
@@ -333,9 +333,10 @@
     if (!B.packed) return BLOK_OK;
     const size_t areas = static_cast<size_t>((ctx->width + blok::kPackArea - 1u) / blok::kPackArea) * ((ctx->height + blok::kPackArea - 1u) / blok::kPackArea);
     const size_t entries = areas * blok::kPackStretch, words = areas * blok::kPackGroups, pixels = static_cast<size_t>(ctx->width) * ctx->height;
-    const bool own = B.policy.own_starts;
+    const bool own = B.policy.own_starts, nodes = own && B.policy.node_restart;
     if (B.list_capacity >= entries && B.words_capacity >= words && B.d_trips.capacity() >= pixels &&
-        (!own || (B.d_ray_start.capacity() >= pixels && B.d_restarts.capacity() >= pixels && B.slots[0].d_start.capacity() >= entries))) return BLOK_OK;
+        (!own || (B.d_ray_start.capacity() >= pixels && B.d_restarts.capacity() >= pixels && B.slots[0].d_start.capacity() >= entries)) &&
+        (!nodes || (B.d_ray_node.capacity() >= pixels && B.slots[0].d_node.capacity() >= entries))) return BLOK_OK;
     BLOK_HIP_TRY(ctx, hipDeviceSynchronize());
     B.list_capacity = 0; B.words_capacity = 0;
     blok::beam_cache_clear(B.policy);
@@ -345,10 +346,12 @@
         BLOK_HIP_TRY(ctx, sl.d_list.reserve(entries, waited));
         BLOK_HIP_TRY(ctx, sl.d_table.reserve(words, waited));
         if (own) BLOK_HIP_TRY(ctx, sl.d_start.reserve(entries, waited));
+        if (nodes) BLOK_HIP_TRY(ctx, sl.d_node.reserve(entries, waited));
         sl.n_groups = 0;
     }
     BLOK_HIP_TRY(ctx, B.d_trips.reserve(pixels, waited));
     if (own) { BLOK_HIP_TRY(ctx, B.d_ray_start.reserve(pixels, waited)); BLOK_HIP_TRY(ctx, B.d_restarts.reserve(pixels, waited)); }
+    if (nodes) BLOK_HIP_TRY(ctx, B.d_ray_node.reserve(pixels, waited));
     BLOK_HIP_TRY(ctx, B.d_words.reserve(words, waited));
     B.sort_temp_bytes = blok::pack_table_temp_bytes(static_cast<uint32_t>(words));
     BLOK_HIP_TRY(ctx, B.d_sort_temp.reserve(B.sort_temp_bytes ? B.sort_temp_bytes : 16, waited));
@@ -406,6 +409,8 @@
     std::memcpy(start_key.jitter_clip, args.jitter_clip, sizeof(start_key.jitter_clip));
     std::memcpy(&start_key.tmin, &args.tmin, sizeof(uint32_t)); std::memcpy(&start_key.tmax, &args.tmax, sizeof(uint32_t));
     *starts = blok::plan_beam_starts(B.policy, *plan, *listed, start_key);
+    if (blok::beam_nodes_count(B.policy, *plan, *starts) && (!blok::node_words_apply(ctx->stats.n_tree_nodes) || !B.d_ray_node || !B.slots[plan->slot].d_node))
+        blok::beam_nodes_decline(B.policy, plan->slot);
     if (plan->action == blok::BeamAction::Search) return BLOK_OK;
     auto& sl = B.slots[plan->slot];
     if (plan->action == blok::BeamAction::Hit) {
@@ -532,17 +537,22 @@
         const bool one_launch = listed.use_list && sl.n_groups > 0u && B.packed_fill > 0u;
         if (!one_launch) blok::launch_beam_fill(mode, fill, n_beams, sl.d_fine, stream);
         if (one_launch) {
-            const uint32_t tail = starts.use == blok::BeamStarts::Use ? blok::launch_packed_frame_own(fill, sl.d_start, sl.d_fine, sl.d_list, sl.d_table, sl.n_groups, B.packed_fill, stream)
-                                                                      : blok::launch_packed_frame(fill, sl.d_fine, sl.d_list, sl.d_table, sl.n_groups, B.packed_fill, stream);
+            const bool from_nodes = blok::beam_nodes_use(B.policy, cached, starts) && sl.d_node;
+            const uint32_t tail = from_nodes ? blok::launch_packed_frame_node(fill, sl.d_start, sl.d_node, sl.d_fine, sl.d_list, sl.d_table, sl.n_groups, B.packed_fill, stream)
+                                  : starts.use == blok::BeamStarts::Use ? blok::launch_packed_frame_own(fill, sl.d_start, sl.d_fine, sl.d_list, sl.d_table, sl.n_groups, B.packed_fill, stream)
+                                                                        : blok::launch_packed_frame(fill, sl.d_fine, sl.d_list, sl.d_table, sl.n_groups, B.packed_fill, stream);
             B.one_launch_frames += 1u; B.fill_only_workgroups += tail;
+            if (from_nodes) B.node_hits += 1u;
         } else if (listed.use_list && starts.use == blok::BeamStarts::Use) blok::launch_packed_walk_own(fill, sl.d_start, sl.d_list, sl.d_table, sl.n_groups, stream);
         else if (listed.use_list) blok::launch_packed_walk(fill, sl.d_fine, sl.d_list, sl.d_table, sl.n_groups, stream);
         else if (starts.count_own) {
             blok::TraceArgs walk = fill;
             walk.beam = sl.d_fine; walk.beam_tile = blok::kWaveW; walk.beam_bx = (args.w + blok::kWaveW - 1u) / blok::kWaveW;
-            blok::launch_trace_count_own(walk, blocks, B.d_trips, B.d_ray_start, B.d_restarts, stream);
+            const bool with_nodes = blok::beam_nodes_count(B.policy, cached, starts);
+            blok::launch_trace_count_own(walk, blocks, B.d_trips, B.d_ray_start, B.d_restarts, with_nodes ? B.d_ray_node.get() : nullptr, stream);
             sl.n_words = blok::pack_areas(args) * blok::kPackGroups; sl.n_groups = 0u;
-            blok::launch_pack_build_own(fill, sl.d_fine, B.d_restarts, B.d_ray_start, sl.d_list, B.d_words, sl.d_start, stream);
+            if (with_nodes) blok::launch_pack_build_node(fill, sl.d_fine, B.d_restarts, B.d_ray_start, B.d_ray_node, sl.d_list, B.d_words, sl.d_start, sl.d_node, stream);
+            else blok::launch_pack_build_own(fill, sl.d_fine, B.d_restarts, B.d_ray_start, sl.d_list, B.d_words, sl.d_start, stream);
         } else {
             blok::TraceArgs walk = fill;
             walk.beam = sl.d_fine; walk.beam_tile = blok::kWaveW; walk.beam_bx = (args.w + blok::kWaveW - 1u) / blok::kWaveW;
diff --git a/blok_amd/csrc/hip/beam_cache.h b/blok_amd/csrc/hip/beam_cache.h
--- a/blok_amd/csrc/hip/beam_cache.h
+++ b/blok_amd/csrc/hip/beam_cache.h
@@ -73,12 +73,14 @@
     bool own_starts = true;
     bool starts[kBeamCacheSlots];
     BeamStartKey start_key[kBeamCacheSlots];
+    bool node_restart = true;
+    bool nodes[kBeamCacheSlots];
     int building = -1;
     bool building_stale = false;
 };
 
 inline void beam_list_drop(BeamCachePolicy& s, int slot) {
-    s.list[slot] = BeamList::None; s.fine_hits[slot] = 0u; s.starts[slot] = false;
+    s.list[slot] = BeamList::None; s.fine_hits[slot] = 0u; s.starts[slot] = false; s.nodes[slot] = false;
     if (s.building == slot) s.building_stale = true;
 }
 
@@ -146,6 +148,7 @@
     if (p.action != BeamAction::Hit || p.slot < 0 || p.slot >= kBeamCacheSlots) return {false, BeamStarts::None};
     if (l.count_now) {
         s.starts[p.slot] = s.own_starts;
+        s.nodes[p.slot] = s.own_starts && s.node_restart;
         if (s.own_starts) s.start_key[p.slot] = k;
         return {s.own_starts, BeamStarts::None};
     }
@@ -157,7 +160,17 @@
     if (slot < 0 || slot >= kBeamCacheSlots || s.list[slot] != BeamList::Now) return;
     s.list[slot] = issued ? BeamList::Building : BeamList::None;
     if (issued) { s.building = slot; s.building_stale = false; }
-    else { s.fine_hits[slot] = 0u; s.starts[slot] = false; }
+    else { s.fine_hits[slot] = 0u; s.starts[slot] = false; s.nodes[slot] = false; }
+}
+
+inline void beam_nodes_decline(BeamCachePolicy& s, int slot) {
+    if (slot >= 0 && slot < kBeamCacheSlots) s.nodes[slot] = false;
+}
+inline bool beam_nodes_count(const BeamCachePolicy& s, const BeamCachePlan& p, const BeamStartsPlan& plan) {
+    return plan.count_own && p.slot >= 0 && p.slot < kBeamCacheSlots && s.nodes[p.slot];
+}
+inline bool beam_nodes_use(const BeamCachePolicy& s, const BeamCachePlan& p, const BeamStartsPlan& plan) {
+    return plan.use == BeamStarts::Use && p.slot >= 0 && p.slot < kBeamCacheSlots && s.node_restart && s.nodes[p.slot];
 }
 
 }
diff --git a/blok_amd/csrc/hip/trace_core.h b/blok_amd/csrc/hip/trace_core.h
--- a/blok_amd/csrc/hip/trace_core.h
+++ b/blok_amd/csrc/hip/trace_core.h
@@ -419,6 +419,84 @@
 }
 #endif
 
+constexpr uint32_t kNodeWordNone = 0xFFFFFFFFu;
+constexpr uint32_t kNodeWordLevelShift = 29u;
+constexpr uint32_t kNodeWordIndexMask = (1u << kNodeWordLevelShift) - 1u;
+
+BLOK_DEV bool start_axis(const Axis& a, bool neg, float point, float inv_vs, int origin, int W, float tS, float& f, float& t_far) {
+    const float w = floorf(point * inv_vs) - static_cast<float>(origin);
+    const float v = neg ? static_cast<float>(W - 1) - w : w;
+    if (!(v == v)) return false;
+    const float u = fminf(fmaxf(v, 0.0f), static_cast<float>(W - 1));
+    f = kCoordBias + u;
+    float t_lo = plane_t(a, f);
+    t_far = plane_t(a, f + 1.0f);
+    if (t_lo > tS) { f -= 1.0f; t_far = t_lo; t_lo = plane_t(a, f); }
+    else if (t_far <= tS) { f += 1.0f; t_lo = t_far; t_far = plane_t(a, f + 1.0f); }
+    return t_lo <= tS && tS < t_far && f >= kCoordBias && f <= kCoordBias + static_cast<float>(W - 1);
+}
+
+BLOK_DEV bool start_voxel(const TraceArgs& A, const RayIn& r, const WalkRay& R, float& fx, float& fy, float& fz, float& tFx, float& tFy, float& tFz) {
+    const int W = 1 << (2 * A.levels);
+    const float tS = r.tmin;
+    const bool negx = !(R.ax.inv > 0.0f), negy = !(R.ay.inv > 0.0f), negz = !(R.az.inv > 0.0f);
+    fx = fy = fz = kCoordBias; tFx = tFy = tFz = 0.0f;
+    bool ok = start_axis(R.ax, negx, __builtin_fmaf(r.dx, tS, r.ox), A.inv_voxel_size, A.origin[0], W, tS, fx, tFx);
+    ok = start_axis(R.ay, negy, __builtin_fmaf(r.dy, tS, r.oy), A.inv_voxel_size, A.origin[1], W, tS, fy, tFy) && ok;
+    ok = start_axis(R.az, negz, __builtin_fmaf(r.dz, tS, r.oz), A.inv_voxel_size, A.origin[2], W, tS, fz, tFz) && ok;
+    return ok && tS < r.tmax;
+}
+
+BLOK_DEV uint32_t restart_node_word(const TraceArgs& A, const RayIn& r, const WalkRay& R, const uint32_t level) {
+    if (level >= A.levels) return kNodeWordNone;
+    float fx, fy, fz, tFx, tFy, tFz;
+    if (!start_voxel(A, r, R, fx, fy, fz, tFx, tFy, tFz)) return kNodeWordNone;
+    uint32_t index = 0u;
+    for (uint32_t lvl = A.levels - 1u; lvl > level; --lvl) {
+        const uint4 c = A.nodes[index];
+        NodeRec node;
+        node.lo = c.x; node.hi = c.y; node.base = c.z;
+        const uint32_t shift = 2u * lvl;
+        const uint32_t bit = (digit2(__float_as_uint(fx), shift) | (digit2(__float_as_uint(fy), shift) << 2) | (digit2(__float_as_uint(fz), shift) << 4)) ^ R.mirror;
+        if (!mask_bit(node, bit)) return kNodeWordNone;
+        index = child_index(node, bit);
+    }
+    if (index > kNodeWordIndexMask) return kNodeWordNone;
+    return index | (level << kNodeWordLevelShift);
+}
+
+BLOK_DEV bool walk_enter_node(const TraceArgs& A, const RayIn& r, const WalkRay& R, const uint32_t word, const uint4 rec, WalkState& s) {
+    const uint32_t lvl = word >> kNodeWordLevelShift;
+    float fx, fy, fz, tFx, tFy, tFz;
+    const bool ok = start_voxel(A, r, R, fx, fy, fz, tFx, tFy, tFz) && word != kNodeWordNone && lvl < A.levels;
+    const uint32_t shift = 2u * lvl;
+    const float size = cell_size_of_shift(shift);
+    if (shift != 0u) {
+        const uint32_t keep = ~((1u << shift) - 1u);
+        fx = __uint_as_float(__float_as_uint(fx) & keep); fy = __uint_as_float(__float_as_uint(fy) & keep); fz = __uint_as_float(__float_as_uint(fz) & keep);
+        tFx = plane_t(R.ax, fx + size); tFy = plane_t(R.ay, fy + size); tFz = plane_t(R.az, fz + size);
+    }
+    const uint32_t bit = (digit2(__float_as_uint(fx), shift) | (digit2(__float_as_uint(fy), shift) << 2) | (digit2(__float_as_uint(fz), shift) << 4)) ^ R.mirror;
+    NodeRec node;
+    node.lo = rec.x; node.hi = rec.y; node.base = rec.z;
+    const bool occupied = mask_bit(node, bit);
+    const float tCur = r.tmin;
+    const float tExit = fminf(fminf(tFx, tFy), tFz);
+    const bool found = occupied && tCur < fminf(tExit, r.tmax);
+    const bool go = !found && tExit < r.tmax;
+    bool ends = !go;
+    if (go) {
+        const bool sx = tFx == tExit;
+        const bool sy = !sx && tFy == tExit;
+        const float stepped = (sx ? fx : (sy ? fy : fz)) + size;
+        const uint32_t up = static_cast<uint32_t>(__builtin_ctz(__float_as_uint(stepped))) & ~1u;
+        ends = up >= 2u * A.levels;
+    }
+    s.fx = fx; s.fy = fy; s.fz = fz; s.tFx = tFx; s.tFy = tFy; s.tFz = tFz; s.tCur = tCur; s.size = size;
+    s.lvl = lvl; s.bit = bit; s.node = node; s.walking = false; s.found = found;
+    return ok && !(occupied && shift != 0u) && (found || ends);
+}
+
 BLOK_DEV HitInfo walk(const TraceArgs& A, const RayIn& r, uint4* stk) {
     BLOK_STAT(4, 0);
     HitInfo out;
diff --git a/blok_amd/csrc/hip/trace_kernels.h b/blok_amd/csrc/hip/trace_kernels.h
--- a/blok_amd/csrc/hip/trace_kernels.h
+++ b/blok_amd/csrc/hip/trace_kernels.h
@@ -207,7 +207,7 @@
 void launch_trace_count(const TraceArgs& args, uint32_t n_blocks, uint8_t* trips, hipStream_t stream);
 void launch_pack_build(const TraceArgs& args, const float* fine, const uint8_t* trips, uint32_t* list, uint32_t* words, hipStream_t stream);
 void launch_packed_walk(const TraceArgs& args, const float* fine, const uint32_t* list, const uint32_t* table, uint32_t n_groups, hipStream_t stream);
-void launch_trace_count_own(const TraceArgs& args, uint32_t n_blocks, uint8_t* trips, float* starts, uint8_t* restarts, hipStream_t stream);
+void launch_trace_count_own(const TraceArgs& args, uint32_t n_blocks, uint8_t* trips, float* starts, uint8_t* restarts, uint32_t* node_words, hipStream_t stream);
 void launch_pack_build_own(const TraceArgs& args, const float* fine, const uint8_t* restarts, const float* starts, uint32_t* list, uint32_t* words, float* slot_start, hipStream_t stream);
 void launch_packed_walk_own(const TraceArgs& args, const float* slot_start, const uint32_t* list, const uint32_t* table, uint32_t n_groups, hipStream_t stream);
 #ifndef BLOK_PACKED_FILL
@@ -216,6 +216,11 @@
 uint32_t launch_packed_frame(const TraceArgs& args, const float* fine, const uint32_t* list, const uint32_t* table, uint32_t n_groups, uint32_t units_per_wave, hipStream_t stream);
 uint32_t launch_packed_frame_own(const TraceArgs& args, const float* slot_start, const float* fine, const uint32_t* list, const uint32_t* table, uint32_t n_groups, uint32_t units_per_wave,
                                  hipStream_t stream);
+bool node_words_apply(size_t n_tree_nodes);
+void launch_pack_build_node(const TraceArgs& args, const float* fine, const uint8_t* restarts, const float* starts, const uint32_t* node_words, uint32_t* list, uint32_t* words,
+                            float* slot_start, uint32_t* slot_node, hipStream_t stream);
+uint32_t launch_packed_frame_node(const TraceArgs& args, const float* slot_start, const uint32_t* slot_node, const float* fine, const uint32_t* list, const uint32_t* table,
+                                  uint32_t n_groups, uint32_t units_per_wave, hipStream_t stream);
 void launch_untile(const UntileArgs& args, uint32_t n_frames, hipStream_t stream);
 void launch_tile_frames(const TraceArgs& args, const TileFrames& frames, hipStream_t stream, uint32_t walk_blocks_per_frame = 0);
 void launch_beam_frames(const TraceArgs& args, const TileFrames& frames, hipStream_t stream);
diff --git a/blok_amd/csrc/hip/trace_kernels.hip b/blok_amd/csrc/hip/trace_kernels.hip
--- a/blok_amd/csrc/hip/trace_kernels.hip
+++ b/blok_amd/csrc/hip/trace_kernels.hip
@@ -166,7 +166,8 @@
 
 template <RayMode MODE, bool kListed = false, bool kCount = false, bool kOwn = false>
 __device__ __forceinline__ void trace_block(const TraceArgs& A, const uint32_t block, const uint32_t grid, uint4* lds_stack, const float listed_t0 = 0.0f,
-                                            [[maybe_unused]] uint8_t* trips = nullptr, [[maybe_unused]] float* starts = nullptr, [[maybe_unused]] uint8_t* restarts = nullptr) {
+                                            [[maybe_unused]] uint8_t* trips = nullptr, [[maybe_unused]] float* starts = nullptr, [[maybe_unused]] uint8_t* restarts = nullptr,
+                                            [[maybe_unused]] uint32_t* node_words = nullptr) {
     const uint32_t tid = threadIdx.x;
     uint4* stk = lds_stack + tid;
 
@@ -279,6 +280,13 @@
         else if constexpr (kCount) trace_one<true, true>(A, r, stk, sink, trips + out_index);
         else trace_one<BLOK_WAVE_START != 0>(A, r, stk, sink);
         if (cost_slot && tid == 0) *cost_slot = max(static_cast<uint32_t>(__builtin_amdgcn_s_memtime() - clock0), 256u);
+        if constexpr (kOwn) if (node_words) {
+            const uint32_t restarted = restarts[out_index];
+            RayIn from = r;
+            from.tmin = fmaxf(A.tmin, starts[out_index]);
+            const WalkRay R = walk_ray(A, r.ox, r.oy, r.oz, safe_inv(r.dx), safe_inv(r.dy), safe_inv(r.dz));
+            node_words[out_index] = restarted != 0u && restarted <= A.levels ? restart_node_word(A, from, R, A.levels - restarted) : kNodeWordNone;
+        }
     }
 }
 
@@ -293,9 +301,9 @@
     trace_block<RayMode::Rect, false, true>(A, blockIdx.x, gridDim.x, lds_stack, 0.0f, trips);
 }
 
-__global__ __launch_bounds__(kBlock) void trace_count_own_kernel(const TraceArgs A, uint8_t* trips, float* starts, uint8_t* restarts) {
-    extern __shared__ uint4 lds_stack[];
-    trace_block<RayMode::Rect, false, true, true>(A, blockIdx.x, gridDim.x, lds_stack, 0.0f, trips, starts, restarts);
+__global__ __launch_bounds__(kBlock) void trace_count_own_kernel(const TraceArgs A, uint8_t* trips, float* starts, uint8_t* restarts, uint32_t* node_words) {
+    extern __shared__ uint4 lds_stack[];
+    trace_block<RayMode::Rect, false, true, true>(A, blockIdx.x, gridDim.x, lds_stack, 0.0f, trips, starts, restarts, node_words);
 }
 
 __device__ __forceinline__ TraceArgs frame_args(const TraceArgs& A, const TileFrames& F, const uint32_t f) {
@@ -548,6 +556,16 @@
     slot_start[i] = starts[static_cast<size_t>(ry) * w + rx];
 }
 
+__global__ __launch_bounds__(256) void pack_starts_nodes_kernel(const uint32_t* list, const float* starts, const uint32_t* node_words, const uint32_t w, const uint32_t h,
+                                                                const uint32_t n_entries, float* slot_start, uint32_t* slot_node) {
+    const uint32_t i = blockIdx.x * 256u + threadIdx.x;
+    if (i >= n_entries) return;
+    const uint32_t entry = list[i], rx = entry & 0xFFFFu, ry = entry >> 16;
+    if (entry == kPackPad || rx >= w || ry >= h) return;
+    slot_start[i] = starts[static_cast<size_t>(ry) * w + rx];
+    slot_node[i] = node_words[static_cast<size_t>(ry) * w + rx];
+}
+
 __global__ __launch_bounds__(kBlock) void packed_walk_kernel(const TraceArgs A, const float* fine, const uint32_t* list, const uint32_t* table) {
     static_assert(kBlock == 64, "one wave per group");
     extern __shared__ uint4 lds_stack[];
@@ -649,6 +667,43 @@
             RayIn r = primary_ray(A, A.x0 + rx, A.y0 + ry);
             r.tmin = fmaxf(r.tmin, t0);
             trace_one<true>(A, r, lds_stack + lane, Sink{A.out ? A.out + at : nullptr, A.out_rgba ? A.out_rgba + at : nullptr});
+        }
+    }
+    if constexpr (BLOK_PACKED_FILL_FIRST == 0) fill_units_of_workgroup(A, fine, n_units, units_x);
+}
+
+__global__ __launch_bounds__(kBlock) void packed_frame_node_kernel(const TraceArgs A, const float* slot_start, const uint32_t* slot_node, const float* fine, const uint32_t* list,
+                                                                   const uint32_t* table, const uint32_t n_groups, const uint32_t n_units, const uint32_t units_x) {
+    static_assert(kBlock == 64, "one wave per group, one lane per pixel of a unit");
+    extern __shared__ uint4 lds_stack[];
+    const uint32_t lane = threadIdx.x;
+    if constexpr (BLOK_PACKED_FILL_FIRST != 0) fill_units_of_workgroup(A, fine, n_units, units_x);
+    if (blockIdx.x < n_groups) {
+        const uint32_t group = __builtin_amdgcn_readfirstlane(table[blockIdx.x]) & ((1u << kPackKeyShift) - 1u);
+        const uint32_t entry = list[static_cast<size_t>(group) * 64u + lane];
+        const float t0 = slot_start[static_cast<size_t>(group) * 64u + lane];
+        const uint32_t word = slot_node[static_cast<size_t>(group) * 64u + lane];
+        const uint32_t rx = entry & 0xFFFFu, ry = entry >> 16;
+        if (entry != kPackPad && rx < A.w && ry < A.h) {
+            const uint4 rec = A.nodes[word == kNodeWordNone ? 0u : (word & kNodeWordIndexMask)];
+            const size_t at = static_cast<size_t>(ry) * A.w + rx;
+            const Sink dst{A.out ? A.out + at : nullptr, A.out_rgba ? A.out_rgba + at : nullptr};
+            RayIn r = primary_ray(A, A.x0 + rx, A.y0 + ry);
+            r.tmin = fmaxf(r.tmin, t0);
+            const WalkRay R = walk_ray(A, r.ox, r.oy, r.oz, safe_inv(r.dx), safe_inv(r.dy), safe_inv(r.dz));
+            WalkState s;
+            const bool settled = walk_enter_node(A, r, R, word, rec, s);
+            if (__ballot(!settled) != 0ull) trace_one<true>(A, r, lds_stack + lane, dst);
+            else if (s.found) {
+                const HitInfo h = walk_hit(A, r, R, s);
+                uint4 out;
+                out.x = __float_as_uint(h.t);
+                out.y = h.material;
+                out.z = (static_cast<uint32_t>(h.vx) & 0xFFFFu) | (static_cast<uint32_t>(h.vy) << 16);
+                out.w = (static_cast<uint32_t>(h.vz) & 0xFFFFu) | (h.face << 16) | (1u << 24);
+                if (dst.hit) *reinterpret_cast<uint4*>(dst.hit) = out;
+                if (dst.rgba) *dst.rgba = shade_rgba(A.mat_table, A.n_materials, h.material, h.face);
+            } else write_miss(dst);
         }
     }
     if constexpr (BLOK_PACKED_FILL_FIRST == 0) fill_units_of_workgroup(A, fine, n_units, units_x);
@@ -1360,9 +1415,19 @@
     hipLaunchKernelGGL(pack_build_kernel, dim3(pack_areas(args)), dim3(kPackThreads), 0, stream, trips, fine, args.w, args.h, list, words);
 }
 
-void launch_trace_count_own(const TraceArgs& args, uint32_t n_blocks, uint8_t* trips, float* starts, uint8_t* restarts, hipStream_t stream) {
+void launch_trace_count_own(const TraceArgs& args, uint32_t n_blocks, uint8_t* trips, float* starts, uint8_t* restarts, uint32_t* node_words, hipStream_t stream) {
     if (n_blocks == 0 || !trips || !starts || !restarts) return;
-    hipLaunchKernelGGL(trace_count_own_kernel, dim3(n_blocks), dim3(kBlock), frame_lds_bytes(args), stream, args, trips, starts, restarts);
+    hipLaunchKernelGGL(trace_count_own_kernel, dim3(n_blocks), dim3(kBlock), frame_lds_bytes(args), stream, args, trips, starts, restarts, node_words);
+}
+
+bool node_words_apply(size_t n_tree_nodes) { return n_tree_nodes != 0 && n_tree_nodes <= static_cast<size_t>(kNodeWordIndexMask); }
+
+void launch_pack_build_node(const TraceArgs& args, const float* fine, const uint8_t* restarts, const float* starts, const uint32_t* node_words, uint32_t* list, uint32_t* words,
+                            float* slot_start, uint32_t* slot_node, hipStream_t stream) {
+    if (!pack_applies(args) || !fine || !restarts || !starts || !node_words || !list || !words || !slot_start || !slot_node) return;
+    hipLaunchKernelGGL(pack_build_kernel, dim3(pack_areas(args)), dim3(kPackThreads), 0, stream, restarts, fine, args.w, args.h, list, words);
+    const uint32_t n_entries = pack_areas(args) * kPackStretch;
+    hipLaunchKernelGGL(pack_starts_nodes_kernel, dim3((n_entries + 255u) / 256u), dim3(256), 0, stream, list, starts, node_words, args.w, args.h, n_entries, slot_start, slot_node);
 }
 
 void launch_pack_build_own(const TraceArgs& args, const float* fine, const uint8_t* restarts, const float* starts, uint32_t* list, uint32_t* words, float* slot_start, hipStream_t stream) {
@@ -1394,6 +1459,14 @@
     if (n_groups == 0 || units_per_wave == 0 || !pack_applies(args) || !slot_start || !fine || !list || !table) return 0u;
     const FillGrid g = fill_grid(args.w, args.h, n_groups, units_per_wave);
     hipLaunchKernelGGL(packed_frame_own_kernel, dim3(g.grid), dim3(kBlock), frame_lds_bytes(args), stream, args, slot_start, fine, list, table, n_groups, g.n_units, g.units_x);
+    return g.grid - n_groups;
+}
+
+uint32_t launch_packed_frame_node(const TraceArgs& args, const float* slot_start, const uint32_t* slot_node, const float* fine, const uint32_t* list, const uint32_t* table,
+                                  uint32_t n_groups, uint32_t units_per_wave, hipStream_t stream) {
+    if (n_groups == 0 || units_per_wave == 0 || !pack_applies(args) || !slot_start || !slot_node || !fine || !list || !table) return 0u;
+    const FillGrid g = fill_grid(args.w, args.h, n_groups, units_per_wave);
+    hipLaunchKernelGGL(packed_frame_node_kernel, dim3(g.grid), dim3(kBlock), frame_lds_bytes(args), stream, args, slot_start, slot_node, fine, list, table, n_groups, g.n_units, g.units_x);
     return g.grid - n_groups;
 }
 
diff --git a/blok_amd/tracer.py b/blok_amd/tracer.py
--- a/blok_amd/tracer.py
+++ b/blok_amd/tracer.py
@@ -505,7 +505,7 @@
         self._check(self._lib.blok_hip_set_miss_writer(self._ctx, 1 if in_walk else 0))
 
     def set_beam_cache(self, mode):
-        self._check(self._lib.blok_hip_set_beam_cache(self._ctx, (4 if mode else 0) if isinstance(mode, bool) else int(mode)))
+        self._check(self._lib.blok_hip_set_beam_cache(self._ctx, (5 if mode else 0) if isinstance(mode, bool) else int(mode)))
 
     def set_beam_refine_after(self, hits: int):
         self._check(self._lib.blok_hip_set_beam_refine_after(self._ctx, hits))
@@ -557,6 +557,24 @@
         self._check(self._lib.blok_hip_beam_cache_start_counters(self._ctx, C.byref(used), C.byref(other)))
         return int(used.value), int(other.value)
 
+    def beam_cache_has_nodes(self) -> bool:
+        has = C.c_int(0)
+        self._check(self._lib.blok_hip_beam_cache_download_nodes(self._ctx, C.byref(has), None, 0, None, 0))
+        return bool(has.value)
+
+    def beam_cache_nodes(self, w: int, h: int):
+        state, areas = C.c_int(0), C.c_uint32(0)
+        self._check(self._lib.blok_hip_beam_cache_download_list(self._ctx, C.byref(state), C.byref(areas), None, None, 0, None, 0, None, 0))
+        entry_words = np.zeros((int(areas.value), self.pack_area() ** 2), dtype=np.uint32)
+        pixel_words = np.zeros((h, w), dtype=np.uint32)
+        self._check(self._lib.blok_hip_beam_cache_download_nodes(self._ctx, None, _ffi.ptr(entry_words), entry_words.size, _ffi.ptr(pixel_words), pixel_words.size))
+        return entry_words, pixel_words
+
+    def beam_cache_node_counter(self) -> int:
+        n = C.c_uint64(0)
+        self._check(self._lib.blok_hip_beam_cache_node_counters(self._ctx, C.byref(n)))
+        return int(n.value)
+
     def set_packed_fill(self, units_per_wave: int):
         self._check(self._lib.blok_hip_set_packed_fill(self._ctx, int(units_per_wave)))
 
diff --git a/include/blok_hip_debug.h b/include/blok_hip_debug.h
--- a/include/blok_hip_debug.h
+++ b/include/blok_hip_debug.h
@@ -40,6 +40,9 @@
 int blok_hip_beam_cache_download_starts(blok_hip_ctx* ctx, int* out_state, float* out_starts_host_or_null, size_t starts_capacity, uint8_t* out_restarts_host_or_null,
                                         size_t restarts_capacity);
 int blok_hip_beam_cache_start_counters(const blok_hip_ctx* ctx, uint64_t* out_from_starts, uint64_t* out_other_key);
+int blok_hip_beam_cache_download_nodes(blok_hip_ctx* ctx, int* out_has_nodes, uint32_t* out_entry_words_host_or_null, size_t entry_capacity, uint32_t* out_pixel_words_host_or_null,
+                                       size_t pixel_capacity);
+int blok_hip_beam_cache_node_counters(const blok_hip_ctx* ctx, uint64_t* out_from_nodes);
 int blok_hip_set_packed_fill(blok_hip_ctx* ctx, uint32_t units_per_wave);
 int blok_hip_packed_fill_counters(const blok_hip_ctx* ctx, uint64_t* out_one_launch_frames, uint64_t* out_fill_only_workgroups);
 int blok_hip_beam_cache_counters(const blok_hip_ctx* ctx, uint64_t* out_hits, uint64_t* out_fills);
```

Measured after the change: 228,800 Mrays/s, median of 6. 18.0% higher.
